# 92MING/Stable-Renderer

Measured on AMD Instinct MI355X. Metric: frames/sec @512^2, SD1.5 20-step img2img, 8-view overlap, higher is better.
Workload: dtype f16

## Files before the change

include/sr_hip.h:

```cpp
#ifndef SR_HIP_H
#define SR_HIP_H
#include <stdint.h>
#ifdef __cplusplus
extern "C" {
#endif

typedef enum {
  SR_OK = 0,
  SR_ERR_INVALID = -1,
  SR_ERR_LAUNCH = -2,
  SR_ERR_UNSUPPORTED = -3
} sr_status;

typedef enum { SR_F16 = 0, SR_F32 = 1 } sr_dtype;

const char* sr_last_error(void);
int sr_version(void);
const char* sr_source_hash(void);
int sr_device_sync(void);

typedef struct {
  const void* a;
  const void* a2;
  const void* w;
  const float* bias;
  const float* rowvec;
  const void* residual;
  void* out;
  const void* zero_page;
  int32_t B, H, W;
  int32_t C1, C2;
  int32_t N;
  int32_t KH;
  int32_t stride;
  int32_t upsample;
  int32_t act;
  int32_t transpose_out;
  int32_t ldt;
  int32_t out_f32;
  int32_t dtype;
  float scale;
  int32_t rowvec_ld;
  void* workspace;
  int64_t workspace_bytes;
  const float* row_stats;
  const float* colsum;
  int32_t tile;
  int32_t split;
  int32_t pad_br;
  const void* prefetch;
  int64_t prefetch_bytes;
  int32_t up_h, up_w;
  int32_t* split_counters;
  int32_t group;
  int32_t ln_inline;
  float ln_eps;
  int32_t tile_order;
} sr_igemm_args;
#define SR_IGEMM_SPLIT_COUNTERS 4096
#define SR_IGEMM_GROUP_MAX 4
int sr_igemm(const sr_igemm_args* args, void* stream);
int sr_igemm_group(const sr_igemm_args* const* args, int32_t n, void* stream);

typedef struct {
  const void* x; const void* x2;
  const float* gamma; const float* beta;
  void* y;
  float* partials;
  int32_t B, HW, C1, C2, groups, silu, dtype;
  float eps;
} sr_groupnorm_args;
int sr_groupnorm(const sr_groupnorm_args* args, void* stream);
int64_t sr_groupnorm_scratch_floats(int32_t B, int32_t HW);

int sr_row_stats(const void* x, float* stats, int32_t rows, int32_t C, float eps, int32_t dtype, void* stream);
int sr_layernorm(const void* x, const float* gamma, const float* beta, void* y, int32_t rows, int32_t C,
                 float eps, int32_t dtype, void* stream);
int sr_layernorm_gather(const void* x, const int32_t* sel, int32_t nsel, int32_t frame_rows, int32_t n_frames, int32_t* err_flag,
                        const float* gamma, const float* beta, void* y, int32_t C, float eps, int32_t dtype, void* stream);

typedef struct {
  const void* q; const void* k; const void* vt; void* o;
  int32_t B, Bk, Tq, Tk, heads, d, ldt, dtype;
  int32_t q_stride, k_stride;
  float scale;
} sr_attention_args;
int sr_attention(const sr_attention_args* args, void* stream);

int sr_nchw_to_nhwc(const float* x, void* y, int32_t B, int32_t C, int32_t HW, int32_t Cpad, float scale_mul,
                    const float* per_batch_scale, int32_t dtype, void* stream);
int sr_nhwc_to_nchw(const void* x, float* y, int32_t B, int32_t C, int32_t HW, int32_t ldc, int32_t dtype,
                    void* stream);
int sr_timestep_embedding(const float* t, void* y, int32_t B, int32_t dim, int32_t dtype, void* stream);
int sr_silu(const void* x, void* y, int64_t n, int32_t dtype, void* stream);
int sr_cast(const void* x, int32_t src_dtype, void* y, int32_t dst_dtype, int64_t n, void* stream);
int sr_cache_touch(const void* p, int64_t bytes, void* stream);
int sr_softmax_rows(void* x, int32_t rows, int32_t cols, int32_t dtype, void* stream);
int sr_gather_rows(const void* x, const int32_t* sel, void* y, int32_t nsel, int32_t n_rows, int64_t row_bytes,
                   int32_t* err_flag, void* stream);
int sr_add_scaled(const void* a, const void* b, void* y, int64_t n, float s, int32_t dtype, void* stream);

typedef enum {
  SR_OP_IGEMM = 1, SR_OP_GROUPNORM = 2, SR_OP_LAYERNORM = 3, SR_OP_ATTENTION = 4, SR_OP_NCHW_TO_NHWC = 5,
  SR_OP_NHWC_TO_NCHW = 6, SR_OP_TIMESTEP_EMBED = 7, SR_OP_SILU = 8, SR_OP_SOFTMAX_ROWS = 9, SR_OP_GATHER_ROWS = 10, SR_OP_ADD_SCALED = 11,
  SR_OP_FORK = 12,
  SR_OP_JOIN = 13,
  SR_OP_ROW_STATS = 14,
  SR_OP_LAYERNORM_GATHER = 15
} sr_op_kind;
typedef struct {
  int32_t kind; int32_t lane;
  union {
    sr_igemm_args igemm;
    sr_groupnorm_args gn;
    sr_attention_args attn;
    struct { const void* x; const float* gamma; const float* beta; void* y; int32_t rows, C, dtype; float eps;
             const int32_t* sel; int32_t* err_flag; int32_t frame_rows, n_frames; } ln;
    struct { const void* x; void* y; const float* per_batch_scale; int32_t B, C, HW, Cpad, dtype, ldc; float scale; } cvt;
    struct { const float* t; void* y; int32_t B, dim, dtype; } temb;
    struct { const void* x; void* y; int64_t n; int32_t dtype; int32_t rows, cols; } ew;
    struct { const void* x; void* y; const int32_t* sel; int64_t row_bytes; int32_t nsel; int32_t n_rows; int32_t* err_flag; } gather;
    struct { const void* a; const void* b; void* y; int64_t n; float s; int32_t dtype; } add;
  } u;
} sr_op;
int sr_plan_run(const sr_op* host_ops, int32_t n_ops, void* stream);
int sr_plan_capture(const sr_op* host_ops, int32_t n_ops, void* stream, void** graph_exec);
int sr_graph_launch(void* graph_exec, void* stream);
int sr_graph_destroy(void* graph_exec);

typedef struct sr_model sr_model;
int sr_model_load(const char* path, sr_model** model);
int sr_model_free(sr_model* model);
int sr_model_io(sr_model* model, const char* name, void** dev_ptr, int64_t* nbytes);
int sr_model_run(sr_model* model, const char* plan, void* stream);
int sr_model_write(sr_model* model, const char* name, const void* src, void* stream);
int sr_model_read(sr_model* model, const char* name, void* dst, void* stream);
int sr_unet_forward(sr_model* unet, const float* x, const float* t, const void* ctx, float* out, void* stream);
int sr_vae_decode(sr_model* vae, const float* z, float* img, void* stream);

int sr_eps_scale_input(const float* x, float* xin, int64_t n_per_copy, int32_t copies, float sigma, void* stream);
int sr_cfg_denoise(const float* x, const float* eps, float* denoised, float* d, int64_t n, int32_t copies,
                   float sigma, float cfg, void* stream);
int sr_cond_crop_scale(const float* x, float* xin, int32_t N, int32_t C, int32_t h, int32_t w, int32_t ah, int32_t aw, int32_t y0,
                       int32_t x0, int32_t chunks, float sigma, void* stream);
int sr_cond_accumulate(const float* x, const float* eps, const float* mult, const int32_t* kinds, float* out_c, float* cnt_c,
                       float* out_u, float* cnt_u, int32_t N, int32_t C, int32_t h, int32_t w, int32_t ah, int32_t aw, int32_t y0,
                       int32_t x0, int32_t chunks, float sigma, void* stream);
int sr_cfg_combine(const float* x, const float* out_c, const float* cnt_c, const float* out_u, const float* cnt_u, float* denoised,
                   float* d, int64_t n, float sigma, float cfg, void* stream);
int sr_euler_step(float* x, const float* d, int64_t n, float dt, void* stream);
int sr_vae_sample(const float* moments, const float* noise, float* z, int32_t B, int32_t zc, int32_t HW, void* stream);
int sr_ddpm_step(float* x, const float* denoised, const float* noise, int64_t n, float sigma, float sigma_next,
                 void* stream);
int sr_lcm_step(float* x, const float* denoised, const float* noise, int64_t n, float sigma_next, void* stream);
int sr_axpby(float* y, const float* x, int64_t n, float a, float b, void* stream);

int sr_idmap_masks(const int32_t* ids, float* masks, int64_t n_pixels, void* stream);

int sr_overlap_build(const int32_t* ids, int32_t N, int32_t H, int32_t W, int32_t lh, int32_t lw,
                     int32_t* pix_cell, int32_t* cell_vid, int32_t* max_vid, void* stream);
int64_t sr_overlap_csr_scratch_ints(int32_t vid_capacity);
int sr_overlap_csr(const int32_t* ids, const int32_t* pix_cell, int32_t N, int32_t H, int32_t W, int32_t vid_capacity,
                   int32_t* vid_off, int32_t* entries, int32_t* scratch, void* stream);
int sr_overlap_step(float* x, const int32_t* cell_vid, const int32_t* vid_off, const int32_t* entries, int32_t N, int32_t C,
                    int32_t lh, int32_t lw, int32_t vid_capacity, float ratio, float* blended, void* stream);

int sr_adain(const float* content, int64_t c_ps, int64_t c_cs, int64_t c_ns, int32_t HWc,
             const void* style, int32_t style_dtype, int64_t s_ps, int64_t s_cs, int64_t s_ns, int32_t HWs,
             float* out, int32_t N, int32_t C, float eps, float* stats, void* stream);

int sr_noise_pool(const void* noise_f16, const void* alpha_f16, const float* bg, float* pooled, float* out,
                  int32_t H, int32_t W, float* stats, void* stream);
int sr_noise_pool_strips(const void* noise_f16, const void* alpha_f16, const float* bg, float* pooled, float* out,
                         int32_t H, int32_t W, int32_t strip, float* stats, void* stream);

int sr_corrmap_update(const float* frame, int32_t Cf, const int32_t* ids, const float* mask,
                      const int32_t* src_index, int32_t n_pixels, int32_t sprite, int32_t material,
                      int32_t check_sprite, int32_t check_material, int32_t mode_first, void* values,
                      uint8_t* writtens, int32_t kk, int32_t V, int32_t* winner, int32_t* err_flag, void* stream);

int sr_legacy_overlap(const float* x, float* y, const int32_t* pix_vert, const int32_t* offsets, const int32_t* tr_f,
                      const int32_t* tr_y, const int32_t* tr_x, const float* view_normal, int32_t T, int32_t C, int32_t h,
                      int32_t w, int32_t H, int32_t W, float alpha, int32_t radius, int32_t algo, int32_t keep_nonzero,
                      void* stream);

int sr_legacy_levels(const int32_t* offsets, const int32_t* tr_f, const int32_t* tr_y, const int32_t* tr_x, const int32_t* order,
                     int32_t n_vertices, int32_t T, int32_t H, int32_t W, int32_t radius, int32_t* level_of, int32_t* n_levels);
int sr_legacy_overlap_seq(float* U, float* newval, const int32_t* lvl_vert, const int32_t* lvl_off_host, int32_t n_levels, int32_t max_len,
                          const int32_t* offsets, const int32_t* tr_f, const int32_t* tr_y, const int32_t* tr_x, const float* view_normal,
                          int32_t C, int32_t H, int32_t W, float alpha, int32_t radius, int32_t algo, void* stream);
int sr_nearest_resize(const float* src, float* dst, int64_t planes, int32_t Hi, int32_t Wi, int32_t Ho, int32_t Wo,
                      const float* keep_if_zero, void* stream);

typedef struct {
  const float* pos; const float* normal; const float* uv;
  const float* color;
  const int32_t* vertex_id;
  const int32_t* tris;
  int32_t nv, nt;
  float MV[16], MV_IT[16], P[16];
  int32_t sprite_id, material_id, corrmap_k, use_texcoord_id, render_mode;
  int32_t has_vertex_color, depth_test, cull_back;
  int32_t id_w, id_h;
  const void* noise_tex; int32_t noise_w, noise_h;
  const void* diffuse_tex; int32_t diffuse_w, diffuse_h;
  const void* corrmap_tex; int32_t corr_w, corr_h;
  const float* tangent; const float* bitangent;
  const void* normal_tex; int32_t normal_w, normal_h;
  int32_t diffuse_levels;
} sr_draw;
typedef struct {
  void* color;
  int32_t* id;
  float* pos;
  void* normal_depth;
  void* noise;
  float* canny;
  float* zbuf;
  int32_t W, H;
} sr_gbuffer;
int sr_gbuffer_clear(const sr_gbuffer* g, void* stream);
int sr_gbuffer_depth_merge(const sr_gbuffer* acc, const sr_gbuffer* src, void* stream);
int sr_defer_post(const void* color_rgba16f, const int32_t* ids, float* out_rgba, int32_t W, int32_t H, int32_t is_baking,
                  int32_t enable_gamma, int32_t enable_hdr, float gamma, float exposure, float saturation, float brightness,
                  float contrast, void* stream);
// ... 8 lines not shown
```

stable-renderer_amd/_lib.py:

```python
import ctypes as C
import os

_HERE = os.path.dirname(os.path.abspath(__file__))
LIB_PATH = os.path.join(_HERE, "csrc", "libsr_hip.so")
_DEV_LIB = os.environ.get("SR_DEV_LIB")

SR_F16, SR_F32 = 0, 1
(OP_IGEMM, OP_GROUPNORM, OP_LAYERNORM, OP_ATTENTION, OP_NCHW_TO_NHWC, OP_NHWC_TO_NCHW, OP_TIMESTEP_EMBED, OP_SILU,
 OP_SOFTMAX_ROWS, OP_GATHER_ROWS, OP_ADD_SCALED, OP_FORK, OP_JOIN, OP_ROW_STATS, OP_LAYERNORM_GATHER) = range(1, 16)

vp = C.c_void_p
i32 = C.c_int32
i64 = C.c_int64
f32 = C.c_float


class IgemmArgs(C.Structure):
    _fields_ = [("a", vp), ("a2", vp), ("w", vp), ("bias", vp), ("rowvec", vp), ("residual", vp), ("out", vp),
                ("zero_page", vp), ("B", i32), ("H", i32), ("W", i32), ("C1", i32), ("C2", i32), ("N", i32),
                ("KH", i32), ("stride", i32), ("upsample", i32), ("act", i32), ("transpose_out", i32), ("ldt", i32),
                ("out_f32", i32), ("dtype", i32), ("scale", f32), ("rowvec_ld", i32), ("workspace", vp),
                ("workspace_bytes", C.c_int64), ("row_stats", vp), ("colsum", vp), ("tile", i32), ("split", i32), ("pad_br", i32),
                ("prefetch", vp), ("prefetch_bytes", C.c_int64), ("up_h", i32), ("up_w", i32), ("split_counters", vp), ("group", i32), ("ln_inline", i32), ("ln_eps", f32), ("tile_order", i32)]


class GroupNormArgs(C.Structure):
    _fields_ = [("x", vp), ("x2", vp), ("gamma", vp), ("beta", vp), ("y", vp), ("partials", vp), ("B", i32),
                ("HW", i32), ("C1", i32), ("C2", i32), ("groups", i32), ("silu", i32), ("dtype", i32), ("eps", f32)]


class AttentionArgs(C.Structure):
    _fields_ = [("q", vp), ("k", vp), ("vt", vp), ("o", vp), ("B", i32), ("Bk", i32), ("Tq", i32), ("Tk", i32),
                ("heads", i32), ("d", i32), ("ldt", i32), ("dtype", i32), ("q_stride", i32), ("k_stride", i32),
                ("scale", f32)]


class _Ln(C.Structure):
    _fields_ = [("x", vp), ("gamma", vp), ("beta", vp), ("y", vp), ("rows", i32), ("C", i32), ("dtype", i32), ("eps", f32),
                ("sel", vp), ("err_flag", vp), ("frame_rows", i32), ("n_frames", i32)]


class _Cvt(C.Structure):
    _fields_ = [("x", vp), ("y", vp), ("per_batch_scale", vp), ("B", i32), ("C", i32), ("HW", i32), ("Cpad", i32),
                ("dtype", i32), ("ldc", i32), ("scale", f32)]


class _Temb(C.Structure):
    _fields_ = [("t", vp), ("y", vp), ("B", i32), ("dim", i32), ("dtype", i32)]


class _Ew(C.Structure):
    _fields_ = [("x", vp), ("y", vp), ("n", i64), ("dtype", i32), ("rows", i32), ("cols", i32)]


class _Gather(C.Structure):
    _fields_ = [("x", vp), ("y", vp), ("sel", vp), ("row_bytes", i64), ("nsel", i32), ("n_rows", i32), ("err_flag", vp)]


class _Add(C.Structure):
    _fields_ = [("a", vp), ("b", vp), ("y", vp), ("n", i64), ("s", f32), ("dtype", i32)]


class _OpU(C.Union):
    _fields_ = [("igemm", IgemmArgs), ("gn", GroupNormArgs), ("attn", AttentionArgs), ("ln", _Ln), ("cvt", _Cvt),
                ("temb", _Temb), ("ew", _Ew), ("gather", _Gather), ("add", _Add)]


class Op(C.Structure):
    _fields_ = [("kind", i32), ("lane", i32), ("u", _OpU)]


class Draw(C.Structure):
    _fields_ = [("pos", vp), ("normal", vp), ("uv", vp), ("color", vp), ("vertex_id", vp), ("tris", vp), ("nv", i32),
                ("nt", i32), ("MV", f32 * 16), ("MV_IT", f32 * 16), ("P", f32 * 16), ("sprite_id", i32),
                ("material_id", i32), ("corrmap_k", i32), ("use_texcoord_id", i32), ("render_mode", i32),
                ("has_vertex_color", i32), ("depth_test", i32), ("cull_back", i32), ("id_w", i32), ("id_h", i32),
                ("noise_tex", vp), ("noise_w", i32), ("noise_h", i32), ("diffuse_tex", vp), ("diffuse_w", i32),
                ("diffuse_h", i32), ("corrmap_tex", vp), ("corr_w", i32), ("corr_h", i32),
                ("tangent", vp), ("bitangent", vp), ("normal_tex", vp), ("normal_w", i32), ("normal_h", i32), ("diffuse_levels", i32)]


class GBuffer(C.Structure):
    _fields_ = [("color", vp), ("id", vp), ("pos", vp), ("normal_depth", vp), ("noise", vp), ("canny", vp), ("zbuf", vp),
                ("W", i32), ("H", i32)]


P = C.POINTER
SYMBOLS = {
    "sr_last_error": (C.c_char_p, []),
    "sr_version": (C.c_int, []),
    "sr_source_hash": (C.c_char_p, []),
    "sr_device_sync": (C.c_int, []),
    "sr_model_load": (C.c_int, [C.c_char_p, P(vp)]),
    "sr_model_free": (C.c_int, [vp]),
    "sr_model_io": (C.c_int, [vp, C.c_char_p, P(vp), P(i64)]),
    "sr_model_run": (C.c_int, [vp, C.c_char_p, vp]),
    "sr_model_write": (C.c_int, [vp, C.c_char_p, vp, vp]),
    "sr_model_read": (C.c_int, [vp, C.c_char_p, vp, vp]),
    "sr_unet_forward": (C.c_int, [vp, vp, vp, vp, vp, vp]),
    "sr_vae_decode": (C.c_int, [vp, vp, vp, vp]),
    "sr_layernorm_gather": (C.c_int, [vp, vp, i32, i32, i32, vp, vp, vp, vp, i32, f32, i32, vp]),
    "sr_igemm": (C.c_int, [P(IgemmArgs), vp]),
    "sr_igemm_group": (C.c_int, [P(P(IgemmArgs)), i32, vp]),
    "sr_groupnorm": (C.c_int, [P(GroupNormArgs), vp]),
    "sr_groupnorm_scratch_floats": (i64, [i32, i32]),
    "sr_layernorm": (C.c_int, [vp, vp, vp, vp, i32, i32, f32, i32, vp]),
    "sr_row_stats": (C.c_int, [vp, vp, i32, i32, f32, i32, vp]),
    "sr_attention": (C.c_int, [P(AttentionArgs), vp]),
    "sr_nchw_to_nhwc": (C.c_int, [vp, vp, i32, i32, i32, i32, f32, vp, i32, vp]),
    "sr_nhwc_to_nchw": (C.c_int, [vp, vp, i32, i32, i32, i32, i32, vp]),
    "sr_timestep_embedding": (C.c_int, [vp, vp, i32, i32, i32, vp]),
    "sr_silu": (C.c_int, [vp, vp, i64, i32, vp]),
    "sr_cast": (C.c_int, [vp, i32, vp, i32, i64, vp]),
    "sr_cache_touch": (C.c_int, [vp, i64, vp]),
    "sr_softmax_rows": (C.c_int, [vp, i32, i32, i32, vp]),
    "sr_gather_rows": (C.c_int, [vp, vp, vp, i32, i32, i64, vp, vp]),
    "sr_add_scaled": (C.c_int, [vp, vp, vp, i64, f32, i32, vp]),
    "sr_plan_run": (C.c_int, [P(Op), i32, vp]),
    "sr_plan_capture": (C.c_int, [P(Op), i32, vp, P(vp)]),
    "sr_graph_launch": (C.c_int, [vp, vp]),
    "sr_graph_destroy": (C.c_int, [vp]),
    "sr_eps_scale_input": (C.c_int, [vp, vp, i64, i32, f32, vp]),
    "sr_cfg_denoise": (C.c_int, [vp, vp, vp, vp, i64, i32, f32, f32, vp]),
    "sr_cond_crop_scale": (C.c_int, [vp, vp, i32, i32, i32, i32, i32, i32, i32, i32, i32, f32, vp]),
    "sr_cond_accumulate": (C.c_int, [vp, vp, vp, vp, vp, vp, vp, vp, i32, i32, i32, i32, i32, i32, i32, i32, i32, f32, vp]),
    "sr_cfg_combine": (C.c_int, [vp, vp, vp, vp, vp, vp, vp, i64, f32, f32, vp]),
    "sr_euler_step": (C.c_int, [vp, vp, i64, f32, vp]),
    "sr_vae_sample": (C.c_int, [vp, vp, vp, i32, i32, i32, vp]),
    "sr_ddpm_step": (C.c_int, [vp, vp, vp, i64, f32, f32, vp]),
    "sr_lcm_step": (C.c_int, [vp, vp, vp, i64, f32, vp]),
    "sr_axpby": (C.c_int, [vp, vp, i64, f32, f32, vp]),
    "sr_idmap_masks": (C.c_int, [vp, vp, i64, vp]),
    "sr_overlap_build": (C.c_int, [vp, i32, i32, i32, i32, i32, vp, vp, vp, vp]),
    "sr_overlap_csr_scratch_ints": (i64, [i32]),
    "sr_overlap_csr": (C.c_int, [vp, vp, i32, i32, i32, i32, vp, vp, vp, vp]),
    "sr_overlap_step": (C.c_int, [vp, vp, vp, vp, i32, i32, i32, i32, i32, f32, vp, vp]),
    "sr_legacy_overlap": (C.c_int, [vp, vp, vp, vp, vp, vp, vp, vp, i32, i32, i32, i32, i32, i32, f32, i32, i32, i32, vp]),
    "sr_legacy_levels": (C.c_int, [vp, vp, vp, vp, vp, i32, i32, i32, i32, i32, vp, vp]),
    "sr_legacy_overlap_seq": (C.c_int, [vp, vp, vp, vp, i32, i32, vp, vp, vp, vp, vp, i32, i32, i32, f32, i32, i32, vp]),
    "sr_nearest_resize": (C.c_int, [vp, vp, i64, i32, i32, i32, i32, vp, vp]),
    "sr_adain": (C.c_int, [vp, i64, i64, i64, i32, vp, i32, i64, i64, i64, i32, vp, i32, i32, f32, vp, vp]),
    "sr_noise_pool": (C.c_int, [vp, vp, vp, vp, vp, i32, i32, vp, vp]),
    "sr_noise_pool_strips": (C.c_int, [vp, vp, vp, vp, vp, i32, i32, i32, vp, vp]),
    "sr_corrmap_update": (C.c_int, [vp, i32, vp, vp, vp, i32, i32, i32, i32, i32, i32, vp, vp, i32, i32, vp, vp, vp]),
    "sr_gbuffer_clear": (C.c_int, [P(GBuffer), vp]),
    "sr_gbuffer_depth_merge": (C.c_int, [P(GBuffer), P(GBuffer), vp]),
    "sr_defer_post": (C.c_int, [vp, vp, vp, i32, i32, i32, i32, i32, f32, f32, f32, f32, f32, vp]),
    "sr_raster_draw": (C.c_int, [P(Draw), P(GBuffer), vp, i64, vp]),
    "sr_raster_scratch_bytes": (i64, [i32, i32, i32]),
}

_lib = None


class SrHipError(RuntimeError):
    pass


def _build_module():
    import importlib.util
    spec = importlib.util.spec_from_file_location("sr_build", os.path.join(_HERE, "csrc", "build.py"))
    mod = importlib.util.module_from_spec(spec)
    spec.loader.exec_module(mod)
    return mod


def _load():
    L = C.CDLL(LIB_PATH)
    for name, (res, args) in SYMBOLS.items():
        fn = getattr(L, name)
        fn.restype = res
        fn.argtypes = args
    return L


def lib():
    global _lib
    if _lib is None and _DEV_LIB:
        L = C.CDLL(_DEV_LIB)
        for name, (res, args) in SYMBOLS.items():
            fn = getattr(L, name)
            fn.restype = res
            fn.argtypes = args
        _lib = L
    if _lib is None:
        bm = _build_module()
        want = bm.source_hash()
        L = None
        if os.path.exists(LIB_PATH) and bm.built_hash() in (None, want):
            try:
                with open(LIB_PATH, "rb") as f:
                    current = want.encode() in f.read()
                if current:
                    L = _load()
            except (OSError, AttributeError):
                L = None
        if L is None:
            import fcntl
            try:
                os.makedirs(os.path.join(_HERE, "csrc", "_obj"), exist_ok=True)
                lock = open(os.path.join(_HERE, "csrc", "_obj", ".build.lock"), "w")
            except OSError as e:
                raise SrHipError(f"libsr_hip.so is stale or missing (sources are {want}) and {os.path.join(_HERE, 'csrc')} is not "
                                 f"writable for a rebuild: {e}; there is no CPU fallback for the product path") from e
            with lock:
                fcntl.flock(lock, fcntl.LOCK_EX)
                try:
                    have = bm.built_hash()
                    if have != want:
                        if os.environ.get("SR_NO_REBUILD") == "1":
                            raise SrHipError(f"libsr_hip.so is stale or missing (built from {have}, sources are {want}) and SR_NO_REBUILD=1; "
                                             "there is no CPU fallback for the product path")
                        try:
                            bm.build()
                        except Exception as e:
                            raise SrHipError(f"libsr_hip.so is stale or missing (built from {have}, sources are {want}) and the rebuild "
                                             f"failed: {e}\nrun `python stable-renderer_amd/csrc/build.py`; there is no CPU fallback for the "
                                             "product path") from e
                    if not os.path.exists(LIB_PATH):
                        raise SrHipError(f"{LIB_PATH} not built; there is no CPU fallback for the product path")
                    L = _load()
                finally:
                    fcntl.flock(lock, fcntl.LOCK_UN)
        if L.sr_source_hash().decode() != want:
            raise SrHipError(f"libsr_hip.so (built from {L.sr_source_hash().decode()}) does not match its sources ({want}): "
                             "remove stable-renderer_amd/csrc/_obj and rebuild")
        _lib = L
    return _lib


def check(rc):
    if rc != 0:
        raise SrHipError("libsr_hip: %s (code %d)" % (lib().sr_last_error().decode(errors="replace"), rc))
```

stable-renderer_amd/csrc/igemm.hip:

```cpp
#include "sr_common.h"
#ifndef SR_IGEMM_TRACE
#define SR_IGEMM_TRACE 0
#endif
#if SR_IGEMM_TRACE
#define SR_TS(k) do { if (threadIdx.x == 0) ts_[k] = wall_clock64(); } while (0)
#else
#define SR_TS(k) do { } while (0)
#endif
#include <stdlib.h>
#include <type_traits>

namespace {

#define SR_FOLD(p) ((p).row_stats != nullptr || (p).ln_inline != 0)
__device__ __forceinline__ float2 sr_fold_stat(const sr_igemm_args& p, const int m, const int m0) {
  extern __shared__ __attribute__((aligned(16))) char sr_lds_front[];
  if (p.ln_inline) return *(const float2*)(sr_lds_front + 8 * (m - m0));
  return *(const float2*)(p.row_stats + 2 * (int64_t)m);
}

template <typename T, int BM, int BN, int WAVES_M, int WAVES_N, int LDS_AVAIL, bool GEGLU, int VCAP, bool VECPRE>
__device__ __forceinline__ void epilogue_rows_h(const sr_igemm_args& p, f32x4 (&acc)[BN / WAVES_N / 16][BM / WAVES_M / 16], char* smem, const int M,
                                                const int rpb, const int m0, const int n0, const int pm0, const int qn0, const int wv,
                                                const int lane) {
  constexpr int NW = WAVES_M * WAVES_N, TM = BM / WAVES_M / 16, TN = BN / WAVES_N / 16;
  constexpr int WCOLS = BN / WAVES_N, OCOLS = GEGLU ? WCOLS / 2 : WCOLS;
  constexpr int ROWB = OCOLS * 2 + 16;
  constexpr int CPR = OCOLS * 2 / 16, RPI = 64 / CPR;
  constexpr int VEC_B = 2 * BN * 4;
  constexpr int LDS_ROWS = VECPRE ? LDS_AVAIL : LDS_AVAIL - VEC_B;
  constexpr int ACC = TM * TN * 4;
  constexpr auto iters = [](int tmp) { return (tmp * 16 + RPI - 1) / RPI; };
  constexpr auto fits = [](int tmp) { return tmp >= 1 && TM % tmp == 0 && NW * tmp * 16 * ROWB <= LDS_ROWS; };
  constexpr auto pre_ok = [](int tmp) { return ACC + (TM / tmp) * ((tmp * 16 + RPI - 1) / RPI) * 4 + 48 <= VCAP; };
  constexpr auto roll_ok = [](int tmp) { return TM / tmp > 1 && ACC + 2 * ((tmp * 16 + RPI - 1) / RPI) * 4 + 40 <= VCAP; };
  constexpr int T_LDS = fits(TM) ? TM : (fits(TM / 2) ? TM / 2 : 1);
  constexpr int TMP = pre_ok(T_LDS) ? T_LDS : (roll_ok(T_LDS) ? T_LDS : ((T_LDS > 1 && roll_ok(T_LDS / 2) && fits(T_LDS / 2)) ? T_LDS / 2 : ((T_LDS > 1 && roll_ok(1)) ? 1 : T_LDS)));
  constexpr int ROWS = TMP * 16, ITER = iters(TMP), NPASS = TM / TMP;
  constexpr bool PRE = pre_ok(TMP);
  constexpr bool ROLL = !PRE && roll_ok(TMP);
  static_assert(OCOLS % 8 == 0 && NW * 16 * ROWB <= LDS_ROWS, "epilogue staging");
  const int c16 = lane & 15, g4 = lane >> 4;
  const float scale = p.scale;
  const int N = p.N;
  const int ldr = p.rowvec_ld ? p.rowvec_ld : N;
  const int ldo = GEGLU ? (N >> 1) : N;
  float* lvec = (float*)(VECPRE ? smem - VEC_B : smem);
  char* wl = smem + (VECPRE ? 0 : VEC_B) + wv * (ROWS * ROWB);
  const int lr = lane / CPR, lc = lane - lr * CPR;
  const int ncol = (GEGLU ? ((n0 + qn0) >> 1) : (n0 + qn0)) + lc * 8;
  const bool lane_on = lr < RPI && ncol < ldo;
  const int tid = wv * 64 + lane;

  float4 vb = make_float4(0.f, 0.f, 0.f, 0.f), vc = make_float4(0.f, 0.f, 0.f, 0.f);
  if constexpr (!VECPRE) {
    const bool vec_lane = tid < BN / 4 && n0 + tid * 4 < N;
    if (vec_lane) {
      if (p.bias) vb = *(const float4*)(p.bias + n0 + tid * 4);
      if (SR_FOLD(p)) vc = *(const float4*)(p.colsum + n0 + tid * 4);
    }
  }
  uint4 resid[PRE ? NPASS * ITER : 1];
  if constexpr (PRE) {
    if (p.residual) {
#pragma unroll
      for (int ps = 0; ps < NPASS; ++ps)
#pragma unroll
        for (int it = 0; it < ITER; ++it) {
          const int row = it * RPI + lr, m = m0 + pm0 + ps * ROWS + row;
          resid[ps * ITER + it] = make_uint4(0, 0, 0, 0);
          if (lane_on && row < ROWS && m < M) resid[ps * ITER + it] = *(const uint4*)((const _Float16*)p.residual + (int64_t)m * ldo + ncol);
        }
    }
  }
  uint4 rcur[ROLL ? ITER : 1], rnext[ROLL ? ITER : 1];
  auto roll_load = [&](uint4 (&dst)[ROLL ? ITER : 1], int ps) {
#pragma unroll
    for (int it = 0; it < (ROLL ? ITER : 1); ++it) {
      const int row = it * RPI + lr, m = m0 + pm0 + ps * ROWS + row;
      dst[it] = make_uint4(0, 0, 0, 0);
      if (lane_on && row < ROWS && m < M) dst[it] = *(const uint4*)((const _Float16*)p.residual + (int64_t)m * ldo + ncol);
    }
  };
  if constexpr (ROLL) { if (p.residual) roll_load(rcur, 0); }
  __syncthreads();
  if constexpr (!VECPRE) {
    if (tid < BN / 4) { *(float4*)(lvec + tid * 4) = vb; *(float4*)(lvec + BN + tid * 4) = vc; }
    __syncthreads();
  }
#pragma unroll
  for (int ps = 0; ps < NPASS; ++ps) {
#pragma unroll
    for (int t = 0; t < TMP; ++t) {
      const int tm = ps * TMP + t;
      const int m = m0 + pm0 + tm * 16 + c16;
      const int b = (p.rowvec && m < M) ? m / rpb : 0;
      float2 rs = make_float2(1.f, 0.f);
      if (SR_FOLD(p) && m < M) rs = sr_fold_stat(p, m, m0);
#pragma unroll
      for (int tn = 0; tn < TN; ++tn) {
        const int nl = qn0 + tn * 16 + 4 * g4, n = n0 + nl;
        float v[4] = {acc[tn][tm][0] * scale, acc[tn][tm][1] * scale, acc[tn][tm][2] * scale, acc[tn][tm][3] * scale};
        if (n < N) {
          if (SR_FOLD(p)) {
            const float4 cs = *(const float4*)(lvec + BN + nl);
            v[0] = fmaf(rs.x, v[0], rs.y * cs.x); v[1] = fmaf(rs.x, v[1], rs.y * cs.y);
            v[2] = fmaf(rs.x, v[2], rs.y * cs.z); v[3] = fmaf(rs.x, v[3], rs.y * cs.w);
          }
          if (p.bias) { const float4 bv = *(const float4*)(lvec + nl); v[0] += bv.x; v[1] += bv.y; v[2] += bv.z; v[3] += bv.w; }
          if (p.rowvec) { const float4 rv = *(const float4*)(p.rowvec + (int64_t)b * ldr + n); v[0] += rv.x; v[1] += rv.y; v[2] += rv.z; v[3] += rv.w; }
        }
        if (p.act == 1) { for (int r = 0; r < 4; ++r) v[r] = sr_silu_f(v[r]); }
        else if (p.act == 3) { for (int r = 0; r < 4; ++r) v[r] = sr_gelu_f(v[r]); }
        else if (p.act == 4) { for (int r = 0; r < 4; ++r) v[r] = fminf(fmaxf((v[r] + 1.0f) * 0.5f, 0.0f), 1.0f); }
        char* dst = wl + (t * 16 + c16) * ROWB;
        if constexpr (GEGLU) {
          const float o0 = v[0] * sr_gelu_f(v[1]), o1 = v[2] * sr_gelu_f(v[3]);
          h16x2 hv = {(_Float16)o0, (_Float16)o1};
          *(h16x2*)(dst + (tn * 8 + 2 * g4) * 2) = hv;
        } else {
          h16x4 hv = {(_Float16)v[0], (_Float16)v[1], (_Float16)v[2], (_Float16)v[3]};
          *(h16x4*)(dst + (tn * 16 + 4 * g4) * 2) = hv;
        }
      }
    }
    __builtin_amdgcn_s_waitcnt(0xC07F);
    __builtin_amdgcn_wave_barrier();
    if constexpr (ROLL) { if (p.residual && ps + 1 < NPASS) roll_load(rnext, ps + 1); }
#pragma unroll
    for (int it = 0; it < ITER; ++it) {
      const int row = it * RPI + lr, m = m0 + pm0 + ps * ROWS + row;
      if (!(lane_on && row < ROWS && m < M)) continue;
      uint4 raw = *(const uint4*)(wl + row * ROWB + lc * 16);
      const int64_t oi = (int64_t)m * ldo + ncol;
      if (p.residual) {
        const h16x8 rr = PRE ? __builtin_bit_cast(h16x8, resid[PRE ? ps * ITER + it : 0])
                       : ROLL ? __builtin_bit_cast(h16x8, rcur[ROLL ? it : 0]) : *(const h16x8*)((const _Float16*)p.residual + oi);
        h16x8 hv = __builtin_bit_cast(h16x8, raw);
#pragma unroll
        for (int e = 0; e < 8; ++e) hv[e] = (_Float16)((float)hv[e] + (float)rr[e]);
        raw = __builtin_bit_cast(uint4, hv);
      }
      *(uint4*)((_Float16*)p.out + oi) = raw;
    }
    if constexpr (ROLL) {
#pragma unroll
      for (int it = 0; it < ITER; ++it) rcur[it] = rnext[it];
    }
    __builtin_amdgcn_wave_barrier();
  }
}

template <typename T, int BM, int BN, int WAVES_M, int WAVES_N, int LDS_AVAIL, bool BLOCK_SYNC = true, int VCAP = 256, bool VECPRE = false>
__device__ __forceinline__ void epilogue_rows(const sr_igemm_args& p, f32x4 (&acc)[BN / WAVES_N / 16][BM / WAVES_M / 16], char* smem, const int M,
                                              const int rpb, const int m0, const int n0, const int pm0, const int qn0, const int wv,
                                              const int lane) {
  constexpr int NW = WAVES_M * WAVES_N, TM = BM / WAVES_M / 16, TN = BN / WAVES_N / 16;
  const int c16 = lane & 15, g4 = lane >> 4;
  const float scale = p.scale;
  const int N = p.N;
  const int ldr = p.rowvec_ld ? p.rowvec_ld : N;
  {
    const int ldo = (p.act == 2) ? (N >> 1) : N;
    const bool o32 = p.out_f32 || sizeof(T) == 4;
    const int oes = o32 ? 4 : 2;
    if constexpr (sizeof(T) == 2) {
      if (!o32 && (ldo * 2) % 16 == 0) {
        static_assert(BLOCK_SYNC, "the fp16 epilogue synchronises the workgroup itself");
        if (p.act == 2) epilogue_rows_h<T, BM, BN, WAVES_M, WAVES_N, LDS_AVAIL, true, VCAP, VECPRE>(p, acc, smem, M, rpb, m0, n0, pm0, qn0, wv, lane);
        else            epilogue_rows_h<T, BM, BN, WAVES_M, WAVES_N, LDS_AVAIL, false, VCAP, VECPRE>(p, acc, smem, M, rpb, m0, n0, pm0, qn0, wv, lane);
        return;
      }
    }
    if ((ldo * oes) % 16 == 0) {
      constexpr int WCOLS = BN / WAVES_N;
      constexpr int TMP = (NW * (BM / WAVES_M) * (WCOLS * 4 + 16) <= LDS_AVAIL) ? TM : 1;
      const int ocols = (p.act == 2) ? WCOLS / 2 : WCOLS;
      const int rowb = ocols * oes + 16;
      if constexpr (BLOCK_SYNC) __syncthreads();
      char* wl = smem + wv * ((TMP * 16) * rowb);
      const int cpr = ocols * oes / 16;
      const int rpi = 64 / cpr;
      const int lr = lane / cpr, lc = lane - lr * cpr;
      const int ncol0 = (p.act == 2) ? ((n0 + qn0) >> 1) : (n0 + qn0);
      const int epc_o = 16 / oes;
#pragma unroll
     for (int tm0 = 0; tm0 < TM; tm0 += TMP) {
#pragma unroll
      for (int tm = tm0; tm < tm0 + TMP; ++tm) {
        const int m = m0 + pm0 + tm * 16 + c16;
        const int b = (m < M) ? m / rpb : 0;
        float2 rs = make_float2(1.f, 0.f);
        if (SR_FOLD(p) && m < M) rs = sr_fold_stat(p, m, m0);
#pragma unroll
        for (int tn = 0; tn < TN; ++tn) {
          const int n = n0 + qn0 + tn * 16 + 4 * g4;
          float v[4] = {acc[tn][tm][0] * scale, acc[tn][tm][1] * scale, acc[tn][tm][2] * scale, acc[tn][tm][3] * scale};
          if (n < N) {
            if (SR_FOLD(p)) {
              const float4 cs = *(const float4*)(p.colsum + n);
              v[0] = fmaf(rs.x, v[0], rs.y * cs.x); v[1] = fmaf(rs.x, v[1], rs.y * cs.y);
              v[2] = fmaf(rs.x, v[2], rs.y * cs.z); v[3] = fmaf(rs.x, v[3], rs.y * cs.w);
            }
            if (p.bias) { const float4 bv = *(const float4*)(p.bias + n); v[0] += bv.x; v[1] += bv.y; v[2] += bv.z; v[3] += bv.w; }
            if (p.rowvec) { const float4 rv = *(const float4*)(p.rowvec + (int64_t)b * ldr + n); v[0] += rv.x; v[1] += rv.y; v[2] += rv.z; v[3] += rv.w; }
          }
          if (p.act == 1) { for (int r = 0; r < 4; ++r) v[r] = sr_silu_f(v[r]); }
          else if (p.act == 3) { for (int r = 0; r < 4; ++r) v[r] = sr_gelu_f(v[r]); }
          else if (p.act == 4) { for (int r = 0; r < 4; ++r) v[r] = fminf(fmaxf((v[r] + 1.0f) * 0.5f, 0.0f), 1.0f); }
          char* dst = wl + ((tm - tm0) * 16 + c16) * rowb;
          if (p.act == 2) {
            const float o0 = v[0] * sr_gelu_f(v[1]), o1 = v[2] * sr_gelu_f(v[3]);
            const int col = tn * 8 + 2 * g4;
            if (o32) *(float2*)(dst + col * 4) = make_float2(o0, o1);
            else { h16x2 hv = {(_Float16)o0, (_Float16)o1}; *(h16x2*)(dst + col * 2) = hv; }
          } else {
            const int col = tn * 16 + 4 * g4;
            if (o32) *(float4*)(dst + col * 4) = make_float4(v[0], v[1], v[2], v[3]);
            else { h16x4 hv = {(_Float16)v[0], (_Float16)v[1], (_Float16)v[2], (_Float16)v[3]}; *(h16x4*)(dst + col * 2) = hv; }
          }
        }
      }
      __builtin_amdgcn_s_waitcnt(0xC07F);
      __builtin_amdgcn_wave_barrier();
      for (int r0 = 0; r0 < TMP * 16; r0 += rpi) {
        const int row = r0 + lr;
        if (lr >= rpi || row >= TMP * 16) continue;
        const int m = m0 + pm0 + tm0 * 16 + row, ncol = ncol0 + lc * epc_o;
        if (m >= M || ncol >= ldo) continue;
        uint4 raw = *(const uint4*)(wl + row * rowb + lc * 16);
        const int64_t oi = (int64_t)m * ldo + ncol;
        if (p.residual) {
          if constexpr (sizeof(T) == 2) {
            if (o32) {
              float4 f = __builtin_bit_cast(float4, raw);
              const h16x4 r4 = *(const h16x4*)((const _Float16*)p.residual + oi);
              f.x += (float)r4[0]; f.y += (float)r4[1]; f.z += (float)r4[2]; f.w += (float)r4[3];
              raw = __builtin_bit_cast(uint4, f);
            } else {
              const h16x8 rr = *(const h16x8*)((const _Float16*)p.residual + oi);
              h16x8 hv = __builtin_bit_cast(h16x8, raw);
#pragma unroll
              for (int e = 0; e < 8; ++e) hv[e] = (_Float16)((float)hv[e] + (float)rr[e]);
              raw = __builtin_bit_cast(uint4, hv);
            }
          } else {
            float4 f = __builtin_bit_cast(float4, raw);
            const float4 rr = *(const float4*)((const float*)p.residual + oi);
            f.x += rr.x; f.y += rr.y; f.z += rr.z; f.w += rr.w;
            raw = __builtin_bit_cast(uint4, f);
          }
        }
        *(uint4*)((char*)p.out + oi * oes) = raw;
      }
      __builtin_amdgcn_wave_barrier();
     }
      return;
    }
#pragma unroll
    for (int tm = 0; tm < TM; ++tm) {
      const int m = m0 + pm0 + tm * 16 + c16;
      if (m >= M) continue;
      const int b = m / rpb;
#pragma unroll
      for (int tn = 0; tn < TN; ++tn) {
        const int n = n0 + qn0 + tn * 16 + 4 * g4;
        if (n >= N) continue;
        float v[4] = {acc[tn][tm][0] * scale, acc[tn][tm][1] * scale, acc[tn][tm][2] * scale, acc[tn][tm][3] * scale};
        const int nv = (N - n) < 4 ? (N - n) : 4;
        if (SR_FOLD(p)) {
          const float2 rs = sr_fold_stat(p, m, m0);
          for (int r = 0; r < nv; ++r) v[r] = fmaf(rs.x, v[r], rs.y * p.colsum[n + r]);
        }
        if (p.bias) { for (int r = 0; r < nv; ++r) v[r] += p.bias[n + r]; }
        if (p.rowvec) { for (int r = 0; r < nv; ++r) v[r] += p.rowvec[(int64_t)b * ldr + n + r]; }
        if (p.act == 1) { for (int r = 0; r < 4; ++r) v[r] = sr_silu_f(v[r]); }
        else if (p.act == 3) { for (int r = 0; r < 4; ++r) v[r] = sr_gelu_f(v[r]); }
        else if (p.act == 4) { for (int r = 0; r < 4; ++r) v[r] = fminf(fmaxf((v[r] + 1.0f) * 0.5f, 0.0f), 1.0f); }
        if (p.act == 2) {
          float o0 = v[0] * sr_gelu_f(v[1]), o1 = v[2] * sr_gelu_f(v[3]);
          const int64_t oi = (int64_t)m * ldo + (n >> 1);
          if (p.residual) { o0 += sr_load_f((const T*)p.residual + oi); o1 += sr_load_f((const T*)p.residual + oi + 1); }
          if (p.out_f32) { float* o = (float*)p.out + oi; o[0] = o0; o[1] = o1; }
          else { T* o = (T*)p.out + oi; sr_store_f(o, o0); sr_store_f(o + 1, o1); }
          continue;
        }
        const int64_t oi = (int64_t)m * ldo + n;
        if (nv == 4) {
          if (p.residual) {
            if constexpr (sizeof(T) == 2) {
              const h16x4 rr = *(const h16x4*)((const T*)p.residual + oi);
              v[0] += (float)rr[0]; v[1] += (float)rr[1]; v[2] += (float)rr[2]; v[3] += (float)rr[3];
            } else {
              const float4 rr = *(const float4*)((const float*)p.residual + oi);
              v[0] += rr.x; v[1] += rr.y; v[2] += rr.z; v[3] += rr.w;
            }
          }
          if (p.out_f32 || sizeof(T) == 4) {
            *(float4*)((float*)p.out + oi) = make_float4(v[0], v[1], v[2], v[3]);
          } else {
            h16x4 hv = {(_Float16)v[0], (_Float16)v[1], (_Float16)v[2], (_Float16)v[3]};
            *(h16x4*)((_Float16*)p.out + oi) = hv;
          }
        } else {
          for (int r = 0; r < nv; ++r) {
            float o = v[r];
            if (p.residual) o += sr_load_f((const T*)p.residual + oi + r);
            if (p.out_f32) ((float*)p.out)[oi + r] = o; else sr_store_f((T*)p.out + oi + r, o);
          }
        }
      }
    }
  }
}

template <int PS, int D>
__device__ __forceinline__ void wait_leaving(int y) {
#define SR_WL(k) if constexpr (D - 1 > k) { if (y == k) { asm volatile("s_waitcnt vmcnt(%0)" ::"n"(PS * k) : "memory"); return; } }
  SR_WL(1) SR_WL(2) SR_WL(3) SR_WL(4) SR_WL(5) SR_WL(6)
#undef SR_WL
  asm volatile("s_waitcnt vmcnt(0)" ::: "memory");
}

template <typename T, int BM, int BN, int WAVES_M, int WAVES_N, int STAGES, bool TRANS, bool SPLIT = false, int BKB = 128, int SPREAD = 0, int MINB = 1, bool LNI = false>
__device__ __forceinline__ void igemm_body(const sr_igemm_args& p, const int M, const int Ho, const int Wo,
                                           const int NT, const int nwg, const int tile0, const int bid, const int nblk) {
  extern __shared__ __attribute__((aligned(16))) char smem_all[];
  constexpr int PF_B = WAVES_M * WAVES_N * 256;
  char* const smem_raw = smem_all + PF_B;
  constexpr bool VECPRE = sizeof(T) == 2 && !SPLIT;
  constexpr int VEC_B = VECPRE ? 2 * BN * 4 : 0;
  char* const smem = smem_raw + VEC_B;
  constexpr int KE = BKB / (int)sizeof(T);
  constexpr int NW = WAVES_M * WAVES_N;
  constexpr int RPI = 1024 / BKB;
  constexpr int GP = BM / RPI, GQ = BN / RPI;
  constexpr int NIP = (GP + NW - 1) / NW, NIQ = (GQ + NW - 1) / NW;
  constexpr int TM = BM / WAVES_M / 16, TN = BN / WAVES_N / 16;
  constexpr int STAGE_BYTES = (BM + BN) * BKB;
  constexpr int FBLK = 16 * BKB;
  static_assert(NW == 4 || NW == 8, "4 or 8 waves");
  static_assert(BKB == 128 || BKB == 64, "K bytes per stage");
  static_assert(BM % RPI == 0 && BN % RPI == 0, "tile rows must be whole LDS-DMA groups");

  const int tid = threadIdx.x, lane = tid & 63;
  const int wv = __builtin_amdgcn_readfirstlane(tid >> 6);
#if SR_IGEMM_TRACE
  unsigned long long ts_[6] = {0, 0, 0, 0, 0, 0};
#endif
  SR_TS(0);
  if (p.prefetch) {
    const int64_t nthr = (int64_t)nblk * gridDim.y * (NW * 64);
    sr_prefetch_touch(p.prefetch, p.prefetch_bytes, ((int64_t)blockIdx.y * nblk + bid) * (NW * 64) + tid, nthr,
                      __builtin_amdgcn_readfirstlane(sr_lds_addr(smem_all) + wv * 256));
  }
  const int wg = tile0 + sr_xcd_remap(bid, nwg);
  int mt, nt;
  sr_tile_of(wg, NT, (M + BM - 1) / BM, p.tile_order, mt, nt);
  const int m0 = mt * BM, n0 = nt * BN;
  if constexpr (VECPRE) {
    constexpr int CH = BN / 2;
    const int c = wv * 64 + lane;
    if (wv * 64 < CH) {
      const bool second = c >= BN / 4;
      const int n = n0 + 4 * (second ? c - BN / 4 : c);
      const float* base = second ? (SR_FOLD(p) ? p.colsum : nullptr) : p.bias;
      const char* src = (base && n < p.N) ? (const char*)(base + n) : (const char*)p.zero_page;
      if (c < CH) sr_glds16_asm(src, __builtin_amdgcn_readfirstlane(sr_lds_addr(smem_raw) + wv * 1024));
    }
  }
  const int lrow = BKB == 128 ? lane >> 3 : lane >> 2;
  int lchunk;
  if constexpr (BKB == 128) lchunk = (lane & 7) ^ lrow;
  else { const int q = (lane & 3) ^ ((lrow >> 2) & 3); lchunk = (0x1320 >> (4 * q)) & 3; }

  const int C1 = p.C1, C2 = p.C2, Ctot = C1 + C2;
  const int K1 = C1 / KE, KPT = Ctot / KE;
  const int ntaps = p.KH * p.KH;
  const int KT = ntaps * KPT;
  const int H = p.H, W = p.W, pad = p.pad_br ? 0 : (p.KH >> 1);
  const int rpb = Ho * Wo;

  int pb[NIP], py[NIP], px[NIP];
#pragma unroll
  for (int i = 0; i < NIP; ++i) {
    const int gi = (i * NW + wv) < GP ? (i * NW + wv) : GP - 1;
    const int m = m0 + gi * RPI + lrow;
    if (m < M) {
      if (rpb == 1) { pb[i] = m; py[i] = -pad; px[i] = -pad; }
      else {
        const int b = m / rpb, rem = m - b * rpb, oy = rem / Wo;
        pb[i] = b; py[i] = oy * p.stride - pad; px[i] = (rem - oy * Wo) * p.stride - pad;
      }
    } else { pb[i] = -1; py[i] = 0; px[i] = 0; }
  }
  const char* zp = (const char*)p.zero_page + lchunk * 16;
  const char* rowA[NIP];
  const char* rowB[NIP];
  auto set_tap = [&](int tap) {
    const int ky = tap / p.KH, kx = tap - ky * p.KH;
#pragma unroll
    for (int i = 0; i < NIP; ++i) {
      int iy = py[i] + ky, ix = px[i] + kx;
      bool ok = pb[i] >= 0;
      if (p.upsample) {
        if (p.up_h > 0) {
          ok = ok && iy >= 0 && ix >= 0 && iy < p.up_h && ix < p.up_w;
          iy = min((int)floorf((float)iy * ((float)H / (float)p.up_h)), H - 1);
          ix = min((int)floorf((float)ix * ((float)W / (float)p.up_w)), W - 1);
          if (!ok) { iy = 0; ix = 0; }
        } else { ok = ok && iy >= 0 && ix >= 0 && iy < 2 * H && ix < 2 * W; iy >>= 1; ix >>= 1; }
      }
      else            { ok = ok && iy >= 0 && ix >= 0 && iy < H && ix < W; }
      const int64_t pix = ((int64_t)pb[i] * H + iy) * W + ix;
      rowA[i] = ok ? (const char*)p.a + (pix * C1) * (int64_t)sizeof(T) + lchunk * 16 : zp;
      rowB[i] = (ok && C2 > 0) ? (const char*)p.a2 + (pix * C2) * (int64_t)sizeof(T) + lchunk * 16 : zp;
    }
  };
  const char* wrow[NIQ];
#pragma unroll
  for (int i = 0; i < NIQ; ++i) {
    const int gi = (i * NW + wv) < GQ ? (i * NW + wv) : GQ - 1;
    const int n = n0 + gi * RPI + lrow;
    wrow[i] = (const char*)p.w + ((int64_t)n * KT * KE) * (int64_t)sizeof(T) + lchunk * 16;
  }

  int kt0 = 0, kt1 = KT;
  if constexpr (SPLIT) {
    kt0 = (int)((int64_t)KT * blockIdx.y / gridDim.y);
    kt1 = (int)((int64_t)KT * (blockIdx.y + 1) / gridDim.y);
#pragma unroll
    for (int i = 0; i < NIQ; ++i) wrow[i] += (int64_t)kt0 * BKB;
  }
  int s_tap = kt0 / KPT, s_kk = kt0 - s_tap * KPT;
  auto advance = [&]() { if (++s_kk == KPT) { s_kk = 0; if (++s_tap < ntaps) set_tap(s_tap); } };
  set_tap(s_tap);
  auto stage = [&](int buf) {
    char* tP = smem + buf * STAGE_BYTES;
    char* tQ = tP + BM * BKB;
    const bool fromA = s_kk < K1;
    const int off = (fromA ? s_kk : s_kk - K1) * BKB;
    auto gp = [&](int i) { return ((i * NW + wv) < GP ? (i * NW + wv) : GP - 1) * 1024; };
    auto gq = [&](int i) { return ((i * NW + wv) < GQ ? (i * NW + wv) : GQ - 1) * 1024; };
    {
      const unsigned lP = __builtin_amdgcn_readfirstlane(sr_lds_addr(tP)), lQ = __builtin_amdgcn_readfirstlane(sr_lds_addr(tQ));
      const unsigned m0 = sr_m0_save();
#pragma unroll
      for (int i = 0; i < NIP; ++i) sr_glds16_asm_nosave((fromA ? rowA[i] : rowB[i]) + off, lP + gp(i));
#pragma unroll
      for (int i = 0; i < NIQ; ++i) { sr_glds16_asm_nosave(wrow[i], lQ + gq(i)); wrow[i] += BKB; }
      sr_m0_restore(m0);
    }
    advance();
  };

  const int c16 = lane & 15, g4 = lane >> 4;
  const int wm = wv / WAVES_N, wn = wv - wm * WAVES_N;
  const int pm0 = wm * (BM / WAVES_M), qn0 = wn * (BN / WAVES_N);
  int foff[2];
  if constexpr (BKB == 128) {
    foff[0] = c16 * 128 + (((0 + g4) ^ (c16 & 7)) << 4);
    foff[1] = c16 * 128 + (((4 + g4) ^ (c16 & 7)) << 4);
  } else {
    foff[0] = foff[1] = c16 * 64 + ((((c16 >> 2) & 3) ^ ((0x2130 >> (4 * g4)) & 3)) << 4);
  }

  constexpr int TA = TRANS ? TM : TN, TB = TRANS ? TN : TM;
  f32x4 acc[TA][TB];
#pragma unroll
  for (int a = 0; a < TA; ++a)
#pragma unroll
    for (int b = 0; b < TB; ++b) acc[a][b] = f32x4{0.f, 0.f, 0.f, 0.f};

  constexpr int TMS = LNI ? TM / WAVES_N : 1;
  static_assert(!LNI || (TM % WAVES_N == 0 && !SPLIT), "in-launch LayerNorm statistics: fragments split evenly over the waves of a row block");
  float lsum[TMS], lsq[TMS], lpiv[TMS];
#pragma unroll
// ... 28 lines not shown

  auto compute = [&](int buf, int j0 = 0, int j1 = BKB / 64) {
    const char* tP = smem + buf * STAGE_BYTES + pm0 * BKB;
    const char* tQ = smem + buf * STAGE_BYTES + BM * BKB + qn0 * BKB;
#pragma unroll
    for (int j = j0; j < j1; ++j) {
      uint4 xf[TM], wf[TN];
#pragma unroll
      for (int t = 0; t < TM; ++t) xf[t] = *(const uint4*)(tP + t * FBLK + foff[j]);
#pragma unroll
      for (int t = 0; t < TN; ++t) wf[t] = *(const uint4*)(tQ + t * FBLK + foff[j]);
      if constexpr (LNI) ln_acc(tP, foff[j]);
#pragma unroll
      for (int tn = 0; tn < TN; ++tn)
#pragma unroll
        for (int tm = 0; tm < TM; ++tm) {
          if constexpr (TRANS) sr_mma(acc[tm][tn], xf[tm], wf[tn], T());
          else                 sr_mma(acc[tn][tm], wf[tn], xf[tm], T());
        }
    }
  };
  auto compute_staging = [&](int buf, int nbuf) {
    const char* tP = smem + buf * STAGE_BYTES + pm0 * BKB;
    const char* tQ = smem + buf * STAGE_BYTES + BM * BKB + qn0 * BKB;
    char* nP = smem + nbuf * STAGE_BYTES;
    const unsigned lP = __builtin_amdgcn_readfirstlane(sr_lds_addr(nP)), lQ = __builtin_amdgcn_readfirstlane(sr_lds_addr(nP + BM * BKB));
    const bool fromA = s_kk < K1;
    const int off = (fromA ? s_kk : s_kk - K1) * BKB;
    constexpr int PIECES = NIP + NIQ, PPS = (PIECES + TN - 1) / TN;
    auto piece = [&](int i) {
      if (i < NIP) {
        const int g = ((i * NW + wv) < GP ? (i * NW + wv) : GP - 1) * 1024;
        sr_glds16_asm_nosave((fromA ? rowA[i] : rowB[i]) + off, lP + g);
      } else if (i < PIECES) {
        const int q = i - NIP;
        const int g = ((q * NW + wv) < GQ ? (q * NW + wv) : GQ - 1) * 1024;
        sr_glds16_asm_nosave(wrow[q], lQ + g);
        wrow[q] += BKB;
      }
    };
    const unsigned m0_keep = sr_m0_save();
#pragma unroll
    for (int j = 0; j < BKB / 64; ++j) {
      uint4 xf[TM], wf[TN];
#pragma unroll
      for (int t = 0; t < TM; ++t) xf[t] = *(const uint4*)(tP + t * FBLK + foff[j]);
#pragma unroll
      for (int t = 0; t < TN; ++t) wf[t] = *(const uint4*)(tQ + t * FBLK + foff[j]);
      if constexpr (LNI) ln_acc(tP, foff[j]);
#pragma unroll
      for (int tn = 0; tn < TN; ++tn) {
#pragma unroll
        for (int tm = 0; tm < TM; ++tm) {
          if constexpr (TRANS) sr_mma(acc[tm][tn], xf[tm], wf[tn], T());
          else                 sr_mma(acc[tn][tm], wf[tn], xf[tm], T());
        }
        if (j == 0) {
#pragma unroll
          for (int q = 0; q < PPS; ++q) piece(tn * PPS + q);
        }
      }
    }
    sr_m0_restore(m0_keep);
    advance();
  };
  {
    constexpr int PER_STAGE = NIP + NIQ;
    constexpr int D = STAGES - 1;
    static_assert(STAGES >= 2 && STAGES <= 8, "ring depth");
    static_assert(PER_STAGE * (D - 1) < 64, "vmcnt immediate");
    const int nk = kt1 - kt0;
    SR_TS(1);
#pragma unroll
    for (int i = 0; i < D; ++i) if (i < nk) stage(i);
    int cur = 0;
    for (int kt = 0; kt < nk; ++kt) {
      const int younger = nk - 1 - kt;
      if (younger >= D - 1) asm volatile("s_waitcnt vmcnt(%0)" ::"n"(PER_STAGE * (D - 1)) : "memory");
      else                  wait_leaving<PER_STAGE, D>(younger);
      __builtin_amdgcn_s_barrier();
      if (kt == 0) SR_TS(2);
      if constexpr (SPREAD == 1) {
        if (kt + D < nk) { int nb = cur + D; if (nb >= STAGES) nb -= STAGES; compute_staging(cur, nb); }
        else compute(cur);
      } else if constexpr (SPREAD == 2 && BKB == 128) {
        compute(cur, 0, 1);
        if (kt + D < nk) { int nb = cur + D; if (nb >= STAGES) nb -= STAGES; stage(nb); }
        compute(cur, 1, 2);
      } else {
        if (kt + D < nk) { int nb = cur + D; if (nb >= STAGES) nb -= STAGES; stage(nb); }
        compute(cur);
      }
      if (++cur == STAGES) cur = 0;
    }
  }

  SR_TS(3);
  if constexpr (LNI) {
    const float invk = 1.0f / (float)p.C1;
#pragma unroll
    for (int i = 0; i < TMS; ++i) {
      float su = lsum[i], sq = lsq[i];
      su += __shfl_xor(su, 16); sq += __shfl_xor(sq, 16);
      su += __shfl_xor(su, 32); sq += __shfl_xor(sq, 32);
      const int tm = wn + i * WAVES_N;
      if (g4 == 0) {
        const float dm = su * invk, var = fmaxf(fmaf(-dm, dm, sq * invk), 0.f);
        const float mean = sizeof(T) == 4 ? lpiv[i] + dm : dm;
        const float rstd = rsqrtf(var + p.ln_eps);
        *(float2*)(smem_all + 8 * (pm0 + tm * 16 + c16)) = make_float2(rstd, -rstd * mean);
      }
    }
    __syncthreads();
  }
  const float scale = p.scale;
  const int N = p.N;
  const int ldr = p.rowvec_ld ? p.rowvec_ld : N;
  if constexpr (SPLIT) {
    f32x4* ws = (f32x4*)p.workspace + (((int64_t)blockIdx.y * nwg + (wg - tile0)) * NW + wv) * (TN * TM * 64) + lane;
#pragma unroll
    for (int tn = 0; tn < TN; ++tn)
#pragma unroll
      for (int tm = 0; tm < TM; ++tm) ws[(tn * TM + tm) * 64] = acc[tn][tm];
    if (p.split_counters == nullptr) return;
    __threadfence();
    __syncthreads();
    int* const flag = (int*)smem_all;
    if (tid == 0) {
      const int prev = __hip_atomic_fetch_add(p.split_counters + (wg - tile0), 1, __ATOMIC_RELAXED, __HIP_MEMORY_SCOPE_AGENT);
      *flag = prev == (int)gridDim.y - 1;
    }
    __syncthreads();
    if (!*flag) return;
    __threadfence();
    {
      const f32x4* wr = (const f32x4*)p.workspace + ((int64_t)(wg - tile0) * NW + wv) * (TN * TM * 64) + lane;
      const int64_t zs = (int64_t)nwg * NW * (TN * TM * 64);
      const int S = gridDim.y;
#pragma unroll
      for (int tn = 0; tn < TN; ++tn)
#pragma unroll
        for (int tm = 0; tm < TM; ++tm) acc[tn][tm] = wr[(tn * TM + tm) * 64];
      for (int z = 1; z < S; ++z) {
#pragma unroll
        for (int tn = 0; tn < TN; ++tn)
#pragma unroll
          for (int tm = 0; tm < TM; ++tm) acc[tn][tm] += wr[z * zs + (tn * TM + tm) * 64];
      }
      if (tid == 0) p.split_counters[wg - tile0] = 0;
    }
    epilogue_rows<T, BM, BN, WAVES_M, WAVES_N, STAGES * STAGE_BYTES, true, (MINB >= 4 ? 128 : 256), VECPRE>(p, acc, smem, M, rpb, m0, n0, pm0, qn0, wv, lane);
    return;
  } else if constexpr (!TRANS) {
    epilogue_rows<T, BM, BN, WAVES_M, WAVES_N, STAGES * STAGE_BYTES, true, (MINB >= 4 ? 128 : 256), VECPRE>(p, acc, smem, M, rpb, m0, n0, pm0, qn0, wv, lane);
#if SR_IGEMM_TRACE
    SR_TS(4);
    asm volatile("s_waitcnt vmcnt(0)" ::: "memory");
    SR_TS(5);
    if (threadIdx.x == 0 && p.workspace && !SPLIT) { unsigned long long* w_ = (unsigned long long*)p.workspace + (size_t)bid * 8; for (int k_ = 0; k_ < 6; ++k_) w_[k_] = ts_[k_]; w_[6] = __smid(); }
#endif
  } else {
    const bool vec = (rpb % 4 == 0) && (p.ldt % 4 == 0);
#pragma unroll
    for (int tm = 0; tm < TM; ++tm) {
      const int m = m0 + pm0 + tm * 16 + 4 * g4;
      if (m >= M) continue;
#pragma unroll
      for (int tn = 0; tn < TN; ++tn) {
        const int n = n0 + qn0 + tn * 16 + c16;
        if (n >= N) continue;
        const float bz = p.bias ? p.bias[n] : 0.f;
        float v[4] = {acc[tm][tn][0] * scale, acc[tm][tn][1] * scale, acc[tm][tn][2] * scale, acc[tm][tn][3] * scale};
        if (SR_FOLD(p)) {
          const float cs = p.colsum[n];
          for (int r = 0; r < 4; ++r)
            if (m + r < M) { const float2 rs = sr_fold_stat(p, m + r, m0); v[r] = fmaf(rs.x, v[r], rs.y * cs); }
        }
        for (int r = 0; r < 4; ++r) v[r] += bz;
        if (vec) {
          const int b = m / rpb, t = m - b * rpb;
          const int64_t oi = ((int64_t)b * N + n) * p.ldt + t;
          if (p.out_f32 || sizeof(T) == 4) *(float4*)((float*)p.out + oi) = make_float4(v[0], v[1], v[2], v[3]);
          else { h16x4 hv = {(_Float16)v[0], (_Float16)v[1], (_Float16)v[2], (_Float16)v[3]}; *(h16x4*)((_Float16*)p.out + oi) = hv; }
        } else {
          for (int r = 0; r < 4; ++r) {
            const int mm = m + r;
            if (mm >= M) break;
            const int b = mm / rpb, t = mm - b * rpb;
            const int64_t oi = ((int64_t)b * N + n) * p.ldt + t;
            if (p.out_f32) ((float*)p.out)[oi] = v[r]; else sr_store_f((T*)p.out + oi, v[r]);
          }
        }
      }
    }
  }
}

template <typename T, int BM, int BN, int WAVES_M, int WAVES_N, int STAGES, bool TRANS, bool SPLIT = false, int BKB = 128, int SPREAD = 0, int MINB = 1, bool LNI = false>
__global__ __launch_bounds__(WAVES_M * WAVES_N * 64, MINB) void igemm_kernel(const sr_igemm_args p, const int M, const int Ho, const int Wo,
                                                                        const int NT, const int nwg, const int tile0) {
  igemm_body<T, BM, BN, WAVES_M, WAVES_N, STAGES, TRANS, SPLIT, BKB, SPREAD, MINB, LNI>(p, M, Ho, Wo, NT, nwg, tile0, blockIdx.x, gridDim.x);
}

struct igemm_group_k {
  sr_igemm_args p[SR_IGEMM_GROUP_MAX];
  int M[SR_IGEMM_GROUP_MAX], Ho[SR_IGEMM_GROUP_MAX], Wo[SR_IGEMM_GROUP_MAX], NT[SR_IGEMM_GROUP_MAX], nwg[SR_IGEMM_GROUP_MAX];
  int start[SR_IGEMM_GROUP_MAX + 1];
  int n;
};
template <typename T, int BM, int BN, int WAVES_M, int WAVES_N, int STAGES, int BKB = 128, int SPREAD = 0, int MINB = 1, bool LNI = false>
__global__ __launch_bounds__(WAVES_M * WAVES_N * 64, MINB) void igemm_group_kernel(const igemm_group_k g) {
  int i = 0;
#pragma unroll
  for (int j = 1; j < SR_IGEMM_GROUP_MAX; ++j) if (j < g.n && (int)blockIdx.x >= g.start[j]) i = j;
  igemm_body<T, BM, BN, WAVES_M, WAVES_N, STAGES, false, false, BKB, SPREAD, MINB, LNI>(g.p[i], g.M[i], g.Ho[i], g.Wo[i], g.NT[i], g.nwg[i], 0,
                                                                                          (int)blockIdx.x - g.start[i], g.nwg[i]);
}

template <typename T, int BM, int BN, int WAVES_M, int WAVES_N, int STAGES, int BKB = 128, int SPREAD = 0, int MINB = 1, bool LNI = false>
int launch_group_impl(const sr_igemm_args* const* as, const int* Ms, const int* Hos, const int* Wos, int n, hipStream_t st) {
  igemm_group_k g;
  g.n = n;
  int tot = 0;
  for (int i = 0; i < SR_IGEMM_GROUP_MAX; ++i) {
    const int k = i < n ? i : n - 1;
    g.p[i] = *as[k];
    g.p[i].prefetch = nullptr;
    g.M[i] = Ms[k]; g.Ho[i] = Hos[k]; g.Wo[i] = Wos[k];
    g.NT[i] = (as[k]->N + BN - 1) / BN;
    g.nwg[i] = ((Ms[k] + BM - 1) / BM) * g.NT[i];
    g.start[i] = tot;
    if (i < n) tot += g.nwg[i];
  }
  g.start[SR_IGEMM_GROUP_MAX] = tot;
  constexpr int lds_stage = STAGES * (BM + BN) * BKB;
  constexpr int lds_epi_all = WAVES_M * WAVES_N * (BM / WAVES_M) * ((BN / WAVES_N) * 4 + 16);
  constexpr int lds_epi = lds_epi_all <= lds_stage ? lds_epi_all : WAVES_M * WAVES_N * 16 * ((BN / WAVES_N) * 4 + 16);
  constexpr int lds = (lds_stage > lds_epi ? lds_stage : lds_epi) + (sizeof(T) == 2 ? 2 * BN * 4 : 0) + WAVES_M * WAVES_N * 256;
  auto k = igemm_group_kernel<T, BM, BN, WAVES_M, WAVES_N, STAGES, BKB, SPREAD, MINB, LNI>;
  static bool attr_set = false;
  if (!attr_set) { (void)hipFuncSetAttribute((const void*)k, hipFuncAttributeMaxDynamicSharedMemorySize, lds); attr_set = true; }
  hipLaunchKernelGGL(k, dim3(tot), dim3(WAVES_M * WAVES_N * 64), lds, st, g);
  SR_CHECK_LAUNCH("sr_igemm_group");
  return SR_OK;
}
template <typename T, int BM, int BN, int WAVES_M, int WAVES_N, int STAGES, int BKB = 128, int SPREAD = 0, int MINB = 1>
int launch_group(const sr_igemm_args* const* as, const int* Ms, const int* Hos, const int* Wos, int n, hipStream_t st) {
  bool lni = false;
  for (int i = 0; i < n; ++i) lni = lni || as[i]->ln_inline;
  if (lni) return launch_group_impl<T, BM, BN, WAVES_M, WAVES_N, STAGES, BKB, SPREAD, MINB, true>(as, Ms, Hos, Wos, n, st);
  return launch_group_impl<T, BM, BN, WAVES_M, WAVES_N, STAGES, BKB, SPREAD, MINB, false>(as, Ms, Hos, Wos, n, st);
}

template <typename T, int BM, int BN, int WAVES_M, int WAVES_N, int STAGES, bool TRANS, int BKB, int SPREAD, int MINB, bool LNI>
int launch_impl(const sr_igemm_args& a, int M, int Ho, int Wo, hipStream_t st) {
  const int Npad = (a.N + 127) / 128 * 128;
  const int MT = (M + BM - 1) / BM, NT = Npad / BN;
  const int NTv = (a.N + BN - 1) / BN;
  const int nwg = MT * NTv;
  constexpr int lds_stage = STAGES * (BM + BN) * BKB;
  constexpr int lds_epi_all = WAVES_M * WAVES_N * (BM / WAVES_M) * ((BN / WAVES_N) * 4 + 16);
  constexpr int lds_epi = lds_epi_all <= lds_stage ? lds_epi_all : WAVES_M * WAVES_N * 16 * ((BN / WAVES_N) * 4 + 16);
  constexpr int lds = (lds_stage > lds_epi ? lds_stage : lds_epi) + (sizeof(T) == 2 ? 2 * BN * 4 : 0)
                      + WAVES_M * WAVES_N * 256;
  auto k = igemm_kernel<T, BM, BN, WAVES_M, WAVES_N, STAGES, TRANS, false, BKB, SPREAD, MINB, LNI>;
  static bool attr_set = false;
  if (!attr_set) { (void)hipFuncSetAttribute((const void*)k, hipFuncAttributeMaxDynamicSharedMemorySize, lds); attr_set = true; }
  (void)NT;
  hipLaunchKernelGGL(k, dim3(nwg), dim3(WAVES_M * WAVES_N * 64), lds, st, a, M, Ho, Wo, NTv, nwg, 0);
  SR_CHECK_LAUNCH("sr_igemm");
  return SR_OK;
}
template <typename T, int BM, int BN, int WAVES_M, int WAVES_N, int STAGES, bool TRANS, int BKB = 128, int SPREAD = 0, int MINB = 1>
int launch(const sr_igemm_args& a, int M, int Ho, int Wo, hipStream_t st) {
  if (a.ln_inline) SR_FAIL(SR_ERR_INVALID, "sr_igemm: ln_inline is not built for this tile (%d x %d, %d stages)", BM, BN, STAGES);
  return launch_impl<T, BM, BN, WAVES_M, WAVES_N, STAGES, TRANS, BKB, SPREAD, MINB, false>(a, M, Ho, Wo, st);
}
template <typename T, int BM, int BN, int WAVES_M, int WAVES_N, int STAGES, bool TRANS, int BKB = 128, int SPREAD = 0, int MINB = 1>
int launch_ln(const sr_igemm_args& a, int M, int Ho, int Wo, hipStream_t st) {
  if (a.ln_inline) return launch_impl<T, BM, BN, WAVES_M, WAVES_N, STAGES, TRANS, BKB, SPREAD, MINB, true>(a, M, Ho, Wo, st);
  return launch_impl<T, BM, BN, WAVES_M, WAVES_N, STAGES, TRANS, BKB, SPREAD, MINB, false>(a, M, Ho, Wo, st);
}

template <typename T, int BM, int BN>
__global__ __launch_bounds__(256) void splitk_reduce_kernel(const sr_igemm_args p, const int M, const int rpb, const int S,
                                                            const int NT, const int nwg, const int tile0) {
  constexpr int TM = BM / 2 / 16, TN = BN / 2 / 16, FR = TN * TM;
  const int tile_l = blockIdx.x / FR, fr = blockIdx.x - tile_l * FR;
  const int tn = fr / TM, tm = fr - tn * TM;
  const int wv = threadIdx.x >> 6, lane = threadIdx.x & 63, c16 = lane & 15, g4 = lane >> 4;
  const int wg = tile0 + tile_l;
  int mt, nt;
  sr_tile_of(wg, NT, (M + BM - 1) / BM, p.tile_order, mt, nt);
  const int m = mt * BM + (wv >> 1) * (BM / 2) + tm * 16 + c16;
  const int n = nt * BN + (wv & 1) * (BN / 2) + tn * 16 + 4 * g4;
  const int N = p.N;
  if (m >= M || n >= N) return;
  const f32x4* ws = (const f32x4*)p.workspace + ((int64_t)tile_l * 4 + wv) * (FR * 64) + fr * 64 + lane;
  const int64_t zs = (int64_t)nwg * 4 * FR * 64;
  f32x4 acc = ws[0];
  for (int z = 1; z < S; ++z) acc += ws[z * zs];
  float v[4] = {acc[0] * p.scale, acc[1] * p.scale, acc[2] * p.scale, acc[3] * p.scale};
  if (p.row_stats) {
    const float2 rs = *(const float2*)(p.row_stats + 2 * (int64_t)m);
    const float4 cs = *(const float4*)(p.colsum + n);
    v[0] = fmaf(rs.x, v[0], rs.y * cs.x); v[1] = fmaf(rs.x, v[1], rs.y * cs.y);
    v[2] = fmaf(rs.x, v[2], rs.y * cs.z); v[3] = fmaf(rs.x, v[3], rs.y * cs.w);
  }
  if (p.bias) { const float4 bv = *(const float4*)(p.bias + n); v[0] += bv.x; v[1] += bv.y; v[2] += bv.z; v[3] += bv.w; }
  if (p.rowvec) {
    const int ldr = p.rowvec_ld ? p.rowvec_ld : N;
    const float4 rv = *(const float4*)(p.rowvec + (int64_t)(m / rpb) * ldr + n);
    v[0] += rv.x; v[1] += rv.y; v[2] += rv.z; v[3] += rv.w;
  }
  if (p.act == 1) { for (int r = 0; r < 4; ++r) v[r] = sr_silu_f(v[r]); }
  else if (p.act == 3) { for (int r = 0; r < 4; ++r) v[r] = sr_gelu_f(v[r]); }
  else if (p.act == 4) { for (int r = 0; r < 4; ++r) v[r] = fminf(fmaxf((v[r] + 1.0f) * 0.5f, 0.0f), 1.0f); }
  const int64_t oi = (int64_t)m * N + n;
  if (p.residual) {
    if constexpr (sizeof(T) == 2) {
      const h16x4 rr = *(const h16x4*)((const _Float16*)p.residual + oi);
      v[0] += (float)rr[0]; v[1] += (float)rr[1]; v[2] += (float)rr[2]; v[3] += (float)rr[3];
    } else {
      const float4 rr = *(const float4*)((const float*)p.residual + oi);
      v[0] += rr.x; v[1] += rr.y; v[2] += rr.z; v[3] += rr.w;
    }
  }
  if (p.out_f32 || sizeof(T) == 4) *(float4*)((float*)p.out + oi) = make_float4(v[0], v[1], v[2], v[3]);
  else { h16x4 hv = {(_Float16)v[0], (_Float16)v[1], (_Float16)v[2], (_Float16)v[3]}; *(h16x4*)((_Float16*)p.out + oi) = hv; }
}

template <typename T, int BM, int BN, int STAGES = 2>
int launch_split(const sr_igemm_args& a, int M, int Ho, int Wo, int tile0, int S, hipStream_t st) {
  const int MT = (M + BM - 1) / BM, NTv = (a.N + BN - 1) / BN, ntiles = MT * NTv, ntail = ntiles - tile0;
  constexpr int lds_stage = STAGES * (BM + BN) * 128;
  constexpr int lds_epi = 4 * (BM / 2) * ((BN / 2) * 4 + 16);
  constexpr int lds = (lds_stage > lds_epi ? lds_stage : lds_epi) + (sizeof(T) == 2 ? 2 * BN * 4 : 0) + 4 * 256;
  auto kf = igemm_kernel<T, BM, BN, 2, 2, STAGES, false, false>;
  auto ks = igemm_kernel<T, BM, BN, 2, 2, STAGES, false, true>;
  static bool attr_set = false;
  if (!attr_set) {
    (void)hipFuncSetAttribute((const void*)kf, hipFuncAttributeMaxDynamicSharedMemorySize, lds);
    (void)hipFuncSetAttribute((const void*)ks, hipFuncAttributeMaxDynamicSharedMemorySize, lds);
    attr_set = true;
  }
  if (tile0 > 0) hipLaunchKernelGGL(kf, dim3(tile0), dim3(256), lds, st, a, M, Ho, Wo, NTv, tile0, 0);
  sr_igemm_args as = a;
  if (ntail > SR_IGEMM_SPLIT_COUNTERS) as.split_counters = nullptr;
  hipLaunchKernelGGL(ks, dim3(ntail, S), dim3(256), lds, st, as, M, Ho, Wo, NTv, ntail, tile0);
  if (!as.split_counters) {
    constexpr int FR = (BM / 32) * (BN / 32);
    hipLaunchKernelGGL((splitk_reduce_kernel<T, BM, BN>), dim3(ntail * FR), dim3(256), 0, st, a, M, Ho * Wo, S, NTv, ntail, tile0);
  }
  SR_CHECK_LAUNCH("sr_igemm(split-K)");
  return SR_OK;
}

__global__ __launch_bounds__(512, 1) void conv3p_kernel(const sr_igemm_args p, const int M, const int NT, const int nwg) {
  using T = _Float16;
  extern __shared__ __attribute__((aligned(16))) char smem_all[];
  char* const smem = smem_all + 8 * 256;
  constexpr int BM = 256, BN = 320, WAVES_M = 4, WAVES_N = 2, TM = 4, TN = 10;
  constexpr int APITCH = 80, ABYTES = 32768, BBYTES = BN * 64, BOFF = 2 * ABYTES, LDS_TOTAL = BOFF + 4 * BBYTES;
  const int tid = threadIdx.x, lane = tid & 63;
  const int wv = __builtin_amdgcn_readfirstlane(tid >> 6);
  if (p.prefetch)
    sr_prefetch_touch(p.prefetch, p.prefetch_bytes, (int64_t)blockIdx.x * 512 + tid, (int64_t)gridDim.x * 512,
                      __builtin_amdgcn_readfirstlane(sr_lds_addr(smem_all) + wv * 256));
  const int wg = sr_xcd_remap(blockIdx.x, nwg);
  const int mt = wg / NT, nt = wg - mt * NT;
  const int m0 = mt * BM, n0 = nt * BN;
  const int H = p.H, W = p.W, C1 = p.C1, rpb = H * W;
  const int ipt = rpb >= 256 ? 1 : 256 / rpb;
  const int Ri = rpb >= 256 ? 256 / W : H;
  const int PW = W + 2, HPI = (Ri + 2) * PW, HR = ipt * HPI;
  const int b0 = m0 / rpb, y0 = (m0 - b0 * rpb) / W;

  unsigned aoffg[4];
#pragma unroll
  for (int i = 0; i < 4; ++i) {
    const int u = (wv * 4 + i) * 64 + lane;
    const int hrow = u / 5, ch = u - hrow * 5;
    const int img = hrow / HPI, rem = hrow - img * HPI, hr = rem / PW, hc = rem - hr * PW;
    const int y = y0 + hr - 1, x = hc - 1, b = b0 + img;
    const bool ok = ch < 4 && hrow < HR && y >= 0 && y < H && x >= 0 && x < W && b < p.B;
    aoffg[i] = ok ? (unsigned)(((((int64_t)b * H + y) * W + x) * C1) * 2 + ch * 16) : 0xFFFFFFFFu;
    if (!ok) {
      *(uint4*)(smem + (wv * 4 + i) * 1024 + lane * 16) = make_uint4(0, 0, 0, 0);
      *(uint4*)(smem + ABYTES + (wv * 4 + i) * 1024 + lane * 16) = make_uint4(0, 0, 0, 0);
    }
  }
  asm volatile("s_waitcnt lgkmcnt(0)" ::: "memory");
  const int lrow = lane >> 2;
  const int lchunk = (0x1320 >> (4 * ((lane & 3) ^ ((lrow >> 2) & 3)))) & 3;
  const unsigned wlane = (unsigned)(lrow * 9 * C1 * 2 + lchunk * 16);
  const unsigned ldsA = __builtin_amdgcn_readfirstlane(sr_lds_addr(smem)), ldsB = ldsA + BOFF;
  int ac = 0;
  auto issueA = [&](int buf, int i) {
    if (aoffg[i] != 0xFFFFFFFFu) sr_glds16_asm_saddr(aoffg[i], (const char*)p.a + (int64_t)ac * 64, ldsA + buf * ABYTES + (wv * 4 + i) * 1024);
  };
  int lc = 0, lt = 0;
  auto issueB = [&](int slot) {
    const char* wb = (const char*)p.w + ((int64_t)n0 * 9 * C1 + lt * C1 + lc * 32) * 2;
#pragma unroll
    for (int i = 0; i < 3; ++i) {
      const int gi = (i * 8 + wv) < 20 ? (i * 8 + wv) : 19;
      sr_glds16_asm_saddr(wlane, wb + (int64_t)gi * 16 * 9 * C1 * 2, ldsB + slot * BBYTES + gi * 1024);
    }
    if (++lt == 9) { lt = 0; ++lc; }
  };

  const int c16 = lane & 15, g4 = lane >> 4;
  const int wm = wv >> 1, wn = wv & 1;
  const int pm0 = wm * 64, qn0 = wn * 160;
  int aoff0, adel[TM];
  {
    const int riw = Ri * W;
    auto hrow_of = [&](int pi) { const int img = pi / riw, q = pi - img * riw, r = q / W, cx = q - r * W; return img * HPI + r * PW + cx; };
    aoff0 = hrow_of(pm0 + c16) * APITCH + g4 * 16;
#pragma unroll
    for (int j = 0; j < TM; ++j) adel[j] = __builtin_amdgcn_readfirstlane((hrow_of(pm0 + j * 16) - hrow_of(pm0)) * APITCH);
  }
  const int foffB = qn0 * 64 + c16 * 64 + ((((c16 >> 2) & 3) ^ ((0x2130 >> (4 * g4)) & 3)) << 4);
  const int pw80 = PW * APITCH;

  f32x4 acc[TN][TM];
#pragma unroll
  for (int a = 0; a < TN; ++a)
#pragma unroll
    for (int b = 0; b < TM; ++b) acc[a][b] = f32x4{0.f, 0.f, 0.f, 0.f};

  const int NC = C1 / 32;
  {
    const unsigned m0k = sr_m0_save();
#pragma unroll
    for (int i = 0; i < 4; ++i) issueA(0, i);
    ac = 1;
    issueB(0); issueB(1); issueB(2);
    sr_m0_restore(m0k);
  }
  int s = 0;
  auto chunk = [&](auto lastc, const int c) {
    constexpr bool LASTC = decltype(lastc)::value;
    auto step = [&](auto tc) {
      constexpr int t = decltype(tc)::value;
      constexpr int nx = LASTC ? (t <= 6 ? 6 : (t == 7 ? 3 : 0))
                               : 6 + (t >= 1 && t <= 4) + (t >= 2 && t <= 5) + (t >= 3 && t <= 6);
      asm volatile("s_waitcnt vmcnt(%0)" ::"n"(nx) : "memory");
      __builtin_amdgcn_s_barrier();
      const char* Bq = smem + BOFF + (s & 3) * BBYTES + foffB;
      int to = (t / 3) * pw80 + (t % 3) * APITCH + (c & 1) * ABYTES;
      asm volatile("" : "+s"(to));
      uint4 xf[TM], wf[TN];
#pragma unroll
      for (int j = 0; j < TM; ++j) xf[j] = *(const uint4*)(smem + aoff0 + (adel[j] + to));
#pragma unroll
      for (int tn = 0; tn < TN; ++tn) wf[tn] = *(const uint4*)(Bq + tn * 1024);
      if (!LASTC || t < 6) {
        const unsigned m0k = sr_m0_save();
        issueB((s + 3) & 3);
        if constexpr (!LASTC) { if (t < 4) issueA((c + 1) & 1, t); if (t == 3) ++ac; }
        sr_m0_restore(m0k);
      }
#pragma unroll
      for (int tn = 0; tn < TN; ++tn)
#pragma unroll
        for (int tm = 0; tm < TM; ++tm) sr_mma(acc[tn][tm], wf[tn], xf[tm], T());
      ++s;
    };
    step(std::integral_constant<int, 0>{}); step(std::integral_constant<int, 1>{}); step(std::integral_constant<int, 2>{});
    step(std::integral_constant<int, 3>{}); step(std::integral_constant<int, 4>{}); step(std::integral_constant<int, 5>{});
    step(std::integral_constant<int, 6>{}); step(std::integral_constant<int, 7>{}); step(std::integral_constant<int, 8>{});
  };
  for (int c = 0; c < NC - 1; ++c) chunk(std::false_type{}, c);
  chunk(std::true_type{}, NC - 1);

  epilogue_rows<T, BM, BN, WAVES_M, WAVES_N, LDS_TOTAL>(p, acc, smem, M, rpb, m0, n0, pm0, qn0, wv, lane);
}

static bool conv3p_ok(const sr_igemm_args& a, int M) {
  if (a.dtype != SR_F16 || a.KH != 3 || a.stride != 1 || a.upsample || a.C2 || a.transpose_out || a.row_stats || a.ln_inline || a.pad_br) return false;
  if (a.C1 % 64 || a.N % 320 || M % 256 || a.act == 2) return false;
  const int rpb = a.H * a.W;
  if (a.W < 8 || 256 % a.W) { if (!(rpb < 256 && 256 % rpb == 0)) return false; }
  if (rpb >= 256 ? (rpb % 256 != 0 || 256 % a.W != 0) : (256 % rpb != 0)) return false;
  const int ipt = rpb >= 256 ? 1 : 256 / rpb, Ri = rpb >= 256 ? 256 / a.W : a.H;
  if ((int64_t)a.B * rpb * a.C1 * 2 >= 0xFFFFFFFFLL) return false;
  return ipt * (Ri + 2) * (a.W + 2) * 80 <= 32768;
}

static int launch_conv3p(const sr_igemm_args& a, int M, hipStream_t st) {
  constexpr int lds = 2 * 32768 + 4 * 320 * 64 + 8 * 256;
  const int NT = a.N / 320, nwg = (M / 256) * NT;
  static bool attr_set = false;
  if (!attr_set) { (void)hipFuncSetAttribute((const void*)conv3p_kernel, hipFuncAttributeMaxDynamicSharedMemorySize, lds); attr_set = true; }
  hipLaunchKernelGGL(conv3p_kernel, dim3(nwg), dim3(512), lds, st, a, M, NT, nwg);
  SR_CHECK_LAUNCH("sr_igemm(conv3p)");
  return SR_OK;
}

static inline int plan_split(int64_t tiles, int KT, int slots, double t_k, int64_t tile_ws_bytes, int64_t ws_bytes, int* tile0, int forceS = 0) {
  const int64_t full = tiles / slots, tail = tiles - full * slots;
  *tile0 = (int)(full * slots);
  if (tail == 0) return 1;
  if (forceS > 0)
    return (KT / forceS >= 4 && (int64_t)forceS * tail * tile_ws_bytes <= ws_bytes) ? forceS : -1;
  if (const char* fs = getenv("SR_SPLIT_S")) {
    const int S = atoi(fs);
    if (S >= 1 && KT / S >= 4 && (int64_t)S * tail * tile_ws_bytes <= ws_bytes) return S;
  }
  double best = (double)KT * t_k;
  int bestS = 1;
  for (int S = 2; S <= 16; ++S) {
    if (KT / S < 8 || (int64_t)S * tail * tile_ws_bytes > ws_bytes) break;
    const int64_t rounds = (tail * S + slots - 1) / slots;
    const double t = (double)rounds * ((KT + S - 1) / S) * t_k + (double)(2 * S * tail * tile_ws_bytes) / 4.0e6 + 14.0;
    if (t < best * 0.9) { best = t; bestS = S; }
  }
  return bestS;
}

template <typename T, bool TRANS>
int dispatch(const sr_igemm_args& a, int M, int Ho, int Wo, hipStream_t st) {
  const int n128 = (a.N + 127) / 128, n64 = (a.N + 63) / 64;
  const int64_t wg_128x128 = (int64_t)((M + 127) / 128) * n128;
  const bool waste128 = (n128 * 128 - a.N) * 8 > a.N;
  const char* fenv = getenv("SR_IGEMM_TILE");
  const int force = fenv ? atoi(fenv) : a.tile;
  static const bool split_off = getenv("SR_SPLITK") && atoi(getenv("SR_SPLITK")) == 0;
  const int KT = a.KH * a.KH * ((a.C1 + a.C2) / (int)(128 / sizeof(T)));
  const int forceS = a.split > 1 ? a.split : 0;
  const bool can_split = !TRANS && !split_off && a.split >= 0 && a.workspace && a.act != 2 && a.N % 4 == 0 && !a.ln_inline;
  const bool may_split = can_split && KT >= 32;
  const bool deep_split = can_split && KT >= 8 && (force == 14 || force == 15);
  if (forceS && !((may_split && (force == 2 || force == 3)) || deep_split))
    SR_FAIL(SR_ERR_INVALID, "sr_igemm: split = %d needs tile 2 / 3 (K >= 32 steps) or 14 / 15 (K >= 8 steps), a workspace, no GEGLU / transposed output", a.split);
  if constexpr (!TRANS) {
    if (deep_split && forceS) {
      int tile0 = 0;
      const int64_t tiles = force == 15 ? wg_128x128 : (int64_t)((M + 127) / 128) * n64;
      const int S = plan_split(tiles, KT, 256, 1.0, 128 * (force == 15 ? 128 : 64) * 4, a.workspace_bytes, &tile0, forceS);
      if (S < 0) SR_FAIL(SR_ERR_INVALID, "sr_igemm: split = %d does not fit this shape (K steps %d, workspace %lld B)", a.split, KT, (long long)a.workspace_bytes);
      if (S > 1) return force == 15 ? launch_split<T, 128, 128, 4>(a, M, Ho, Wo, tile0, S, st) : launch_split<T, 128, 64, 6>(a, M, Ho, Wo, tile0, S, st);
      SR_FAIL(SR_ERR_INVALID, "sr_igemm: split = %d: nothing to split (whole rounds of workgroups only)", a.split);
    }
    if (may_split && (force == 2 || force == 3)) {
      int tile0 = 0;
      if (force == 2) {
        const int S = plan_split(wg_128x128, KT, 512, 1.2, 128 * 128 * 4, a.workspace_bytes, &tile0, forceS);
        if (S < 0) SR_FAIL(SR_ERR_INVALID, "sr_igemm: split = %d does not fit this shape (K steps %d, workspace %lld B)", a.split, KT, (long long)a.workspace_bytes);
        if (S > 1) return launch_split<T, 128, 128>(a, M, Ho, Wo, tile0, S, st);
      } else {
        const int S = plan_split((int64_t)((M + 127) / 128) * n64, KT, 768, 0.93, 128 * 64 * 4, a.workspace_bytes, &tile0, forceS);
        if (S < 0) SR_FAIL(SR_ERR_INVALID, "sr_igemm: split = %d does not fit this shape (K steps %d, workspace %lld B)", a.split, KT, (long long)a.workspace_bytes);
        if (S > 1) return launch_split<T, 128, 64>(a, M, Ho, Wo, tile0, S, st);
      }
      if (forceS) SR_FAIL(SR_ERR_INVALID, "sr_igemm: split = %d: nothing to split (whole rounds of workgroups only)", a.split);
    }
  }
  if (force == 2) return launch_ln<T, 128, 128, 2, 2, 2, TRANS>(a, M, Ho, Wo, st);
  if (force == 3) return launch_ln<T, 128, 64, 2, 2, 2, TRANS>(a, M, Ho, Wo, st);
  if (force == 4) return launch_ln<T, 64, 64, 2, 2, 2, TRANS>(a, M, Ho, Wo, st);
  if (force == 13) return launch_ln<T, 64, 64, 2, 2, 8, TRANS>(a, M, Ho, Wo, st);
  if (force == 14) return launch_ln<T, 128, 64, 2, 2, 6, TRANS>(a, M, Ho, Wo, st);
  if (force == 15) return launch_ln<T, 128, 128, 2, 2, 4, TRANS>(a, M, Ho, Wo, st);
  if (force == 8) {
    if constexpr (!TRANS && sizeof(T) == 2) { if (conv3p_ok(a, M)) return launch_conv3p(a, M, st); }
    SR_FAIL(SR_ERR_INVALID, "sr_igemm: tile 8 (patch-stationary 3x3) needs fp16, KH=3, stride 1, one source, N %% 320 == 0, "
                            "256-pixel tiles of whole rows / images (H=%d W=%d M=%d N=%d)", a.H, a.W, M, a.N);
  }
  if constexpr (!TRANS && sizeof(T) == 2) {
    if ((force >= 5 && force <= 7) && a.N % 320) SR_FAIL(SR_ERR_INVALID, "sr_igemm: tile %d (256x320) needs N %% 320 == 0, N=%d", force, a.N);
    if (force == 6) return launch<T, 256, 320, 4, 2, 4, TRANS, 64>(a, M, Ho, Wo, st);
    if (force == 9) {
      if (a.N % 160) SR_FAIL(SR_ERR_INVALID, "sr_igemm: tile 9 (128x160) needs N %% 160 == 0, N=%d", a.N);
      return launch_ln<T, 128, 160, 4, 2, 2, TRANS, 128, 0, 4>(a, M, Ho, Wo, st);
    }
    if (force == 10) {
      if (a.N % 320) SR_FAIL(SR_ERR_INVALID, "sr_igemm: tile 10 (128x320) needs N %% 320 == 0, N=%d", a.N);
      return launch_ln<T, 128, 320, 2, 4, 2, TRANS, 64, 0, 4>(a, M, Ho, Wo, st);
    }
    if (force == 11) return launch_ln<T, 128, 128, 4, 2, 2, TRANS, 128, 0, 4>(a, M, Ho, Wo, st);
    if (force == 12) return launch_ln<T, 256, 128, 4, 2, 2, TRANS, 64, 0, 4>(a, M, Ho, Wo, st);
    if (force == 7 || (force == 0 && a.N % 320 == 0 && (int64_t)((M + 255) / 256) * (a.N / 320) < 256 &&
                       (int64_t)((M + 127) / 128) * (a.N / 320) >= 256))
      return launch_ln<T, 128, 320, 2, 4, 2, TRANS>(a, M, Ho, Wo, st);

    if (force == 5 || (force == 0 && a.N % 320 == 0 && (int64_t)((M + 255) / 256) * (a.N / 320) >= 256))
      return launch_ln<T, 256, 320, 4, 2, 2, TRANS, 128, 2>(a, M, Ho, Wo, st);
  } else {
    if (force >= 5 && force <= 12) SR_FAIL(SR_ERR_INVALID, "sr_igemm: tile %d is fp16, non-transposed only", force);
  }
  const int64_t wg_256x128 = (int64_t)((M + 255) / 256) * n128;
  const bool big = !waste128 && wg_256x128 >= 512;
  if constexpr (!TRANS) {
    if (force == 0 && may_split && !big) {
      int tile0 = 0;
      if (!waste128) {
        const int S = plan_split(wg_128x128, KT, 512, 1.2, 128 * 128 * 4, a.workspace_bytes, &tile0);
        if (S > 1) return launch_split<T, 128, 128>(a, M, Ho, Wo, tile0, S, st);
      } else {
        const int S = plan_split((int64_t)((M + 127) / 128) * n64, KT, 768, 0.93, 128 * 64 * 4, a.workspace_bytes, &tile0);
        if (S > 1) return launch_split<T, 128, 64>(a, M, Ho, Wo, tile0, S, st);
      }
    }
  }
  if (force == 1 || (force == 0 && big && !a.ln_inline))
    return launch<T, 256, 128, 4, 2, 3, TRANS, 128, 1>(a, M, Ho, Wo, st);
  if (!waste128 && wg_128x128 >= 192 && !(a.KH == 1 && wg_128x128 <= 768)) return launch_ln<T, 128, 128, 2, 2, 2, TRANS>(a, M, Ho, Wo, st);
  const int64_t wg_128x64 = (int64_t)((M + 127) / 128) * n64;
  if (wg_128x64 >= 192) return launch_ln<T, 128, 64, 2, 2, 2, TRANS>(a, M, Ho, Wo, st);
  if ((int64_t)((M + 63) / 64) * n64 <= 256 && KT >= 4) return launch_ln<T, 64, 64, 2, 2, 8, TRANS>(a, M, Ho, Wo, st);
  return launch_ln<T, 64, 64, 2, 2, 2, TRANS>(a, M, Ho, Wo, st);
}

}

static int igemm_check(const sr_igemm_args* a, int* M_, int* Ho_, int* Wo_) {
  if (!a || !a->a || !a->w || !a->out || !a->zero_page) SR_FAIL(SR_ERR_INVALID, "sr_igemm: null pointer");
  const int ke = a->dtype == SR_F16 ? 64 : 32;
  if (a->dtype != SR_F16 && a->dtype != SR_F32) SR_FAIL(SR_ERR_INVALID, "sr_igemm: bad dtype %d", a->dtype);
  if (a->C1 <= 0 || a->C1 % ke || a->C2 % ke || a->C2 < 0) SR_FAIL(SR_ERR_INVALID, "sr_igemm: C1=%d C2=%d must be multiples of %d", a->C1, a->C2, ke);
  if (a->C2 > 0 && !a->a2) SR_FAIL(SR_ERR_INVALID, "sr_igemm: C2>0 without a2");
  if (a->KH != 1 && a->KH != 3) SR_FAIL(SR_ERR_INVALID, "sr_igemm: KH=%d", a->KH);
  if (a->stride != 1 && a->stride != 2) SR_FAIL(SR_ERR_INVALID, "sr_igemm: stride=%d", a->stride);
  if (a->upsample && a->stride != 1) SR_FAIL(SR_ERR_INVALID, "sr_igemm: upsample with stride");
  if (a->pad_br && (a->KH != 3 || a->upsample)) SR_FAIL(SR_ERR_INVALID, "sr_igemm: pad_br is for 3x3 convs without upsample");
  if (a->N <= 0 || a->B <= 0 || a->H <= 0 || a->W <= 0) SR_FAIL(SR_ERR_INVALID, "sr_igemm: bad sizes");
  if (a->act == 2 && (a->N % 4 || a->transpose_out)) SR_FAIL(SR_ERR_INVALID, "sr_igemm: GEGLU needs N%%4==0");
  if (a->row_stats && !a->colsum) SR_FAIL(SR_ERR_INVALID, "sr_igemm: row_stats without colsum");
  if (a->ln_inline && (a->row_stats || !a->colsum)) SR_FAIL(SR_ERR_INVALID, "sr_igemm: ln_inline takes colsum and no row_stats");
  if ((a->row_stats || a->ln_inline) && (a->KH != 1 || a->stride != 1 || a->upsample || a->C2)) SR_FAIL(SR_ERR_INVALID, "sr_igemm: folded LayerNorm is for 1x1 single-source layers");
  if (a->tile < 0 || a->tile > 15 || a->split < -1 || a->split == 1 || a->split > 16) SR_FAIL(SR_ERR_INVALID, "sr_igemm: tile=%d split=%d", a->tile, a->split);
  if (a->tile_order != 0 && a->tile_order != 1) SR_FAIL(SR_ERR_INVALID, "sr_igemm: tile_order=%d (0 rows first, 1 columns first)", a->tile_order);
  int Ho, Wo;
  if (a->upsample && ((a->up_h > 0) != (a->up_w > 0))) SR_FAIL(SR_ERR_INVALID, "sr_igemm: up_h / up_w go together");
  if (!a->upsample && (a->up_h || a->up_w)) SR_FAIL(SR_ERR_INVALID, "sr_igemm: up_h / up_w without upsample");
  if (a->upsample) { Ho = a->up_h > 0 ? a->up_h : 2 * a->H; Wo = a->up_w > 0 ? a->up_w : 2 * a->W; }
  else if (a->stride == 2) {
    const int ptot = a->pad_br ? a->KH / 2 : 2 * (a->KH / 2);
    Ho = (a->H + ptot - a->KH) / 2 + 1; Wo = (a->W + ptot - a->KH) / 2 + 1;
  }
  else { Ho = a->H; Wo = a->W; }
  const int64_t M64 = (int64_t)a->B * Ho * Wo;
  if (M64 > 0x7fffffffLL / 2) SR_FAIL(SR_ERR_INVALID, "sr_igemm: M too large");
  if (a->transpose_out && a->ldt < Ho * Wo) SR_FAIL(SR_ERR_INVALID, "sr_igemm: ldt < pixels per batch");
  *M_ = (int)M64; *Ho_ = Ho; *Wo_ = Wo;
  return SR_OK;
}

extern "C" int sr_igemm(const sr_igemm_args* a, void* stream) {
  int M, Ho, Wo;
  const int rc = igemm_check(a, &M, &Ho, &Wo);
  if (rc != SR_OK) return rc;
  hipStream_t st = sr_stream(stream);
  if (a->dtype == SR_F16) {
    return a->transpose_out ? dispatch<_Float16, true>(*a, M, Ho, Wo, st) : dispatch<_Float16, false>(*a, M, Ho, Wo, st);
  }
  return a->transpose_out ? dispatch<float, true>(*a, M, Ho, Wo, st) : dispatch<float, false>(*a, M, Ho, Wo, st);
}

template <typename T>
static int group_launch(int tile, const sr_igemm_args* const* as, const int* Ms, const int* Hos, const int* Wos, int n, hipStream_t st) {
  switch (tile) {
    case 2: return launch_group<T, 128, 128, 2, 2, 2>(as, Ms, Hos, Wos, n, st);
    case 3: return launch_group<T, 128, 64, 2, 2, 2>(as, Ms, Hos, Wos, n, st);
    case 4: return launch_group<T, 64, 64, 2, 2, 2>(as, Ms, Hos, Wos, n, st);
    case 13: return launch_group<T, 64, 64, 2, 2, 8>(as, Ms, Hos, Wos, n, st);
    case 14: return launch_group<T, 128, 64, 2, 2, 6>(as, Ms, Hos, Wos, n, st);
    case 15: return launch_group<T, 128, 128, 2, 2, 4>(as, Ms, Hos, Wos, n, st);
    default: break;
  }
  if constexpr (sizeof(T) == 2) {
    if (tile == 9) return launch_group<T, 128, 160, 4, 2, 2, 128, 0, 4>(as, Ms, Hos, Wos, n, st);
    if (tile == 10) return launch_group<T, 128, 320, 2, 4, 2, 64, 0, 4>(as, Ms, Hos, Wos, n, st);
  }
  return -100;
}

extern "C" int sr_igemm_group(const sr_igemm_args* const* args, int32_t n, void* stream) {
  if (!args || n < 1 || n > SR_IGEMM_GROUP_MAX) SR_FAIL(SR_ERR_INVALID, "sr_igemm_group: 1..%d problems", SR_IGEMM_GROUP_MAX);
  int M[SR_IGEMM_GROUP_MAX], Ho[SR_IGEMM_GROUP_MAX], Wo[SR_IGEMM_GROUP_MAX];
  bool one = n > 1;
  for (int i = 0; i < n; ++i) {
    const int rc = igemm_check(args[i], &M[i], &Ho[i], &Wo[i]);
    if (rc != SR_OK) return rc;
    const sr_igemm_args* a = args[i];
    one = one && a->dtype == args[0]->dtype && a->tile == args[0]->tile && a->tile != 0 && !a->transpose_out && a->split == -1;
    if (a->tile == 9) one = one && a->N % 160 == 0;
    if (a->tile == 10) one = one && a->N % 320 == 0;
  }
  hipStream_t st = sr_stream(stream);
  if (one) {
    const int rc = args[0]->dtype == SR_F16 ? group_launch<_Float16>(args[0]->tile, args, M, Ho, Wo, n, st)
                                            : group_launch<float>(args[0]->tile, args, M, Ho, Wo, n, st);
    if (rc != -100) return rc;
  }
  for (int i = 0; i < n; ++i) {
    const int rc = sr_igemm(args[i], stream);
    if (rc != SR_OK) return rc;
  }
  return SR_OK;
}
```

stable-renderer_amd/csrc/norm.hip:

```cpp
#include "sr_common.h"
#include <stdlib.h>
#include <type_traits>

namespace {

__host__ __device__ inline int gn_ppc(int HW, int B) {
  const int chunks = B >= 8 ? 64 : B >= 4 ? 128 : 256;
  const int p = (HW + chunks - 1) / chunks;
  return p < 64 ? 64 : p;
}

template <typename T>
__device__ __forceinline__ void load_chunk(const T* p, float (&v)[sr_traits<T>::EPC]) {
  if constexpr (sizeof(T) == 2) {
    const h16x8 h = *(const h16x8*)p;
#pragma unroll
    for (int e = 0; e < 8; ++e) v[e] = (float)h[e];
  } else {
    const float4 f = *(const float4*)p;
    v[0] = f.x; v[1] = f.y; v[2] = f.z; v[3] = f.w;
  }
}
template <typename T>
__device__ __forceinline__ void store_chunk(T* p, const float (&v)[sr_traits<T>::EPC]) {
  if constexpr (sizeof(T) == 2) {
    h16x8 h;
#pragma unroll
    for (int e = 0; e < 8; ++e) h[e] = (_Float16)v[e];
    *(h16x8*)p = h;
  } else {
    *(float4*)p = make_float4(v[0], v[1], v[2], v[3]);
  }
}

template <typename T>
__device__ __forceinline__ float gn_pivot(const T* x1, const T* x2, int b, int HW, int C1, int C2, int c0) {
  return c0 < C1 ? (float)x1[(int64_t)b * HW * C1 + c0] : (float)x2[(int64_t)b * HW * C2 + (c0 - C1)];
}

template <typename T>
__global__ __launch_bounds__(256) void gn_stats_kernel(const T* __restrict__ x1, const T* __restrict__ x2, float* __restrict__ partials,
                                                       int HW, int C1, int C2, int groups, int nchunk) {
  constexpr int EPC = sr_traits<T>::EPC;
  extern __shared__ __attribute__((aligned(16))) char smem_raw[];
  const int C = C1 + C2, cpt = C / EPC, cpg = C / groups;
  const int b = blockIdx.y, chunk = blockIdx.x, tid = threadIdx.x;
  const int pp_ = 256 / cpt;
  const int nps = pp_ >= 1 ? pp_ : 1;
  float* chs = (float*)smem_raw;
  float* chq = chs + nps * C;
  const int ppc = gn_ppc(HW, gridDim.y);
  const int p0 = chunk * ppc;
  const int p1 = min(HW, p0 + ppc);
  const int pp = 256 / cpt;
  if (pp >= 1) {
    const int cc = tid % cpt, ps = tid / cpt;
    if (ps < pp) {
      float s[EPC], q[EPC];
#pragma unroll
      for (int e = 0; e < EPC; ++e) { s[e] = 0.f; q[e] = 0.f; }
      const int c0 = cc * EPC;
      const T* src = c0 < C1 ? x1 + (int64_t)b * HW * C1 + c0 : x2 + (int64_t)b * HW * C2 + (c0 - C1);
      const int cs = c0 < C1 ? C1 : C2;
      float piv[EPC];
#pragma unroll
      for (int e = 0; e < EPC; ++e) piv[e] = gn_pivot<T>(x1, x2, b, HW, C1, C2, (c0 + e) / cpg * cpg);
      int p = p0 + ps;
      for (; p + 3 * pp < p1; p += 4 * pp) {
        float v0[EPC], v1[EPC], v2[EPC], v3[EPC];
        load_chunk<T>(src + (int64_t)p * cs, v0);
        load_chunk<T>(src + (int64_t)(p + pp) * cs, v1);
        load_chunk<T>(src + (int64_t)(p + 2 * pp) * cs, v2);
        load_chunk<T>(src + (int64_t)(p + 3 * pp) * cs, v3);
#pragma unroll
        for (int e = 0; e < EPC; ++e) {
          const float d0 = v0[e] - piv[e], d1 = v1[e] - piv[e], d2 = v2[e] - piv[e], d3 = v3[e] - piv[e];
          s[e] += d0; q[e] += d0 * d0;
          s[e] += d1; q[e] += d1 * d1;
          s[e] += d2; q[e] += d2 * d2;
          s[e] += d3; q[e] += d3 * d3;
        }
      }
      for (; p < p1; p += pp) {
        float v[EPC];
        load_chunk<T>(src + (int64_t)p * cs, v);
#pragma unroll
        for (int e = 0; e < EPC; ++e) { const float d = v[e] - piv[e]; s[e] += d; q[e] += d * d; }
      }
#pragma unroll
      for (int e = 0; e < EPC; ++e) { chs[ps * C + c0 + e] = s[e]; chq[ps * C + c0 + e] = q[e]; }
    }
  } else {
    for (int cc = tid; cc < cpt; cc += 256) {
      float s[EPC], q[EPC];
#pragma unroll
      for (int e = 0; e < EPC; ++e) { s[e] = 0.f; q[e] = 0.f; }
      const int c0 = cc * EPC;
      const T* src = c0 < C1 ? x1 + (int64_t)b * HW * C1 + c0 : x2 + (int64_t)b * HW * C2 + (c0 - C1);
      const int cs = c0 < C1 ? C1 : C2;
      float piv[EPC];
#pragma unroll
      for (int e = 0; e < EPC; ++e) piv[e] = gn_pivot<T>(x1, x2, b, HW, C1, C2, (c0 + e) / cpg * cpg);
      for (int p = p0; p < p1; ++p) {
        float v[EPC];
        load_chunk<T>(src + (int64_t)p * cs, v);
#pragma unroll
        for (int e = 0; e < EPC; ++e) { const float d = v[e] - piv[e]; s[e] += d; q[e] += d * d; }
      }
#pragma unroll
      for (int e = 0; e < EPC; ++e) { chs[c0 + e] = s[e]; chq[c0 + e] = q[e]; }
    }
  }
  __syncthreads();
  if (tid < groups) {
    float gs = 0.f, gq = 0.f;
    for (int ps = 0; ps < nps; ++ps)
      for (int c = tid * cpg; c < (tid + 1) * cpg; ++c) { gs += chs[ps * C + c]; gq += chq[ps * C + c]; }
    float* o = partials + (((int64_t)b * nchunk + chunk) * groups + tid) * 2;
    o[0] = gs; o[1] = gq;
  }
}

template <typename T>
__global__ __launch_bounds__(256) void gn_apply_kernel(const T* __restrict__ x1, const T* __restrict__ x2, const float* __restrict__ partials,
                                                       const float* __restrict__ gamma, const float* __restrict__ beta, T* __restrict__ y,
                                                       int HW, int C1, int C2, int groups, int nchunk, float eps, int silu) {
  constexpr int EPC = sr_traits<T>::EPC;
  extern __shared__ __attribute__((aligned(16))) char smem_raw[];
  float* sc = (float*)smem_raw;
  const int C = C1 + C2, cpt = C / EPC, cpg = C / groups;
  float* sh = sc + C;
  float* gm = sh + C;
  const int b = blockIdx.y, chunk = blockIdx.x, tid = threadIdx.x;
  const int ppc = gn_ppc(HW, gridDim.y);
  const int p0 = chunk * ppc;
  const int p1 = min(HW, p0 + ppc);
  const int total = (p1 - p0) * cpt;
  auto src_of = [&](int idx, int& c0, int& p) -> const T* {
    p = p0 + idx / cpt;
    c0 = (idx - (idx / cpt) * cpt) * EPC;
    return c0 < C1 ? x1 + ((int64_t)b * HW + p) * C1 + c0 : x2 + ((int64_t)b * HW + p) * C2 + (c0 - C1);
  };
  auto finish = [&](float (&v)[EPC], int c0, int p) {
#pragma unroll
    for (int e = 0; e < EPC; ++e) {
      float t = v[e] * sc[c0 + e] + sh[c0 + e];
      v[e] = silu ? sr_silu_f(t) : t;
    }
    store_chunk<T>(y + ((int64_t)b * HW + p) * C + c0, v);
  };
  using VEC = typename std::conditional<sizeof(T) == 2, h16x8, f32x4>::type;
  VEC pr[4];
  int pc0[4], pq0[4];
  int pre_n = 0;
#pragma unroll
  for (int i = 0; i < 4; ++i) {
    pr[i] = VEC{};
    if (tid + i * 256 < total) { pr[i] = *(const VEC*)src_of(tid + i * 256, pc0[i], pq0[i]); pre_n = i + 1; }
  }
  {
    float* red = gm + 2 * groups;
    const int g = tid & 31, part = tid >> 5;
    if (g < groups) {
      float s = 0.f, q = 0.f;
      const float* pp = partials + ((int64_t)b * nchunk * groups + g) * 2;
      for (int i = part; i < nchunk; i += 8) { s += pp[(int64_t)i * groups * 2]; q += pp[(int64_t)i * groups * 2 + 1]; }
      red[(part * groups + g) * 2] = s; red[(part * groups + g) * 2 + 1] = q;
    }
    __syncthreads();
    if (tid < groups) {
      double s = 0.0, q = 0.0;
      for (int p8 = 0; p8 < 8; ++p8) { s += red[(p8 * groups + tid) * 2]; q += red[(p8 * groups + tid) * 2 + 1]; }
      const double cnt = (double)HW * cpg;
      const double dm = s / cnt;
      double var = q / cnt - dm * dm;
      if (var < 0.0) var = 0.0;
      gm[tid] = (float)((double)gn_pivot<T>(x1, x2, b, HW, C1, C2, tid * cpg) + dm);
      gm[groups + tid] = (float)(1.0 / sqrt(var + (double)eps));
    }
  }
  __syncthreads();
  for (int c = tid; c < C; c += 256) {
    const int g = c / cpg;
    const float a = gm[groups + g] * gamma[c];
    sc[c] = a; sh[c] = beta[c] - gm[g] * a;
  }
  __syncthreads();
  int idx = tid;
#pragma unroll
  for (int i = 0; i < 4; ++i) {
    VEC r = pr[i];
    asm volatile("" : "+v"(r));
    if (i < pre_n) {
      float v[EPC];
      load_chunk<T>((const T*)&r, v);
      finish(v, pc0[i], pq0[i]);
    }
  }
  idx += pre_n * 256;
  for (; idx + 3 * 256 < total; idx += 4 * 256) {
    int c0[4], pq[4];
    float v0[EPC], v1[EPC], v2[EPC], v3[EPC];
    load_chunk<T>(src_of(idx, c0[0], pq[0]), v0);
    load_chunk<T>(src_of(idx + 256, c0[1], pq[1]), v1);
    load_chunk<T>(src_of(idx + 512, c0[2], pq[2]), v2);
    load_chunk<T>(src_of(idx + 768, c0[3], pq[3]), v3);
    finish(v0, c0[0], pq[0]); finish(v1, c0[1], pq[1]); finish(v2, c0[2], pq[2]); finish(v3, c0[3], pq[3]);
  }
  for (; idx < total; idx += 256) {
    int c0, pq;
    float v[EPC];
    load_chunk<T>(src_of(idx, c0, pq), v);
    finish(v, c0, pq);
  }
}

template <typename T, int NV, int BLOCK>
__global__ __launch_bounds__(BLOCK) void gn_fused_kernel(const T* __restrict__ x1, const T* __restrict__ x2, const float* __restrict__ gamma,
                                                         const float* __restrict__ beta, T* __restrict__ y, int HW, int C1, int C2,
                                                         int groups, int GB, float eps, int silu) {
  constexpr int EPC = sr_traits<T>::EPC;
  using VEC = typename std::conditional<sizeof(T) == 2, h16x8, f32x4>::type;
  extern __shared__ __attribute__((aligned(16))) char smem_raw[];
  const int C = C1 + C2, cpg = C / groups, span = GB * cpg, vpp = span / EPC, pp = BLOCK / vpp;
  float* chs = (float*)smem_raw;
  float* chsum = chs + pp * span;
  float* gstat = chsum + span;
  float* strip = gstat + GB;
  const int NS = BLOCK / span;
  const int nb = groups / GB, wg = sr_xcd_remap(blockIdx.x, gridDim.x);
  const int b = wg / nb, bundle = wg - b * nb, tid = threadIdx.x;
  const int cc = tid % vpp, ps = tid / vpp;
  const bool active = ps < pp;
  const int cl = cc * EPC, c0 = bundle * span + cl;
  const T* src = c0 < C1 ? x1 + (int64_t)b * HW * C1 + c0 : x2 + (int64_t)b * HW * C2 + (c0 - C1);
  const int cs = c0 < C1 ? C1 : C2;
  VEC raw[NV];
  float acc[EPC], piv[EPC];
#pragma unroll
  for (int e = 0; e < EPC; ++e) { acc[e] = 0.f; piv[e] = gn_pivot<T>(x1, x2, b, HW, C1, C2, (c0 + e) / cpg * cpg); }
#pragma unroll
  for (int i = 0; i < NV; ++i) {
    const int p = ps + i * pp;
    if (active && p < HW) {
      raw[i] = *(const VEC*)(src + (int64_t)p * cs);
      float v[EPC];
      load_chunk<T>((const T*)&raw[i], v);
#pragma unroll
      for (int e = 0; e < EPC; ++e) acc[e] += v[e] - piv[e];
    }
  }
  const float inv_cnt = 1.0f / ((float)HW * (float)cpg);
  float mean_e[EPC], rstd_e[EPC];
  for (int round = 0; round < 2; ++round) {
    if (active) {
#pragma unroll
      for (int e = 0; e < EPC; ++e) chs[ps * span + cl + e] = acc[e];
    }
    __syncthreads();
    if (tid < NS * span) {
      const int c = tid % span, s0 = tid / span;
      float t = 0.f;
      for (int q = s0; q < pp; q += NS) t += chs[q * span + c];
      strip[s0 * span + c] = t;
    }
    __syncthreads();
    if (tid < span) {
      float t = 0.f;
      for (int q = 0; q < NS; ++q) t += strip[q * span + tid];
      chsum[tid] = t;
    }
    __syncthreads();
    if (tid < GB) {
      float t = 0.f;
      for (int c = tid * cpg; c < (tid + 1) * cpg; ++c) t += chsum[c];
      gstat[tid] = round == 0 ? t * inv_cnt : rsqrtf(t * inv_cnt + eps);
    }
    __syncthreads();
    if (round == 0) {
#pragma unroll
      for (int e = 0; e < EPC; ++e) { mean_e[e] = gstat[(cl + e) / cpg]; acc[e] = 0.f; }
#pragma unroll
      for (int i = 0; i < NV; ++i) {
        const int p = ps + i * pp;
        if (active && p < HW) {
          float v[EPC];
          VEC r = raw[i];
          asm volatile("" : "+v"(r));
          load_chunk<T>((const T*)&r, v);
#pragma unroll
          for (int e = 0; e < EPC; ++e) { const float d = (v[e] - piv[e]) - mean_e[e]; acc[e] += d * d; }
        }
      }
      __syncthreads();
    } else {
#pragma unroll
      for (int e = 0; e < EPC; ++e) rstd_e[e] = gstat[(cl + e) / cpg];
    }
  }
  if (!active) return;
  float sc[EPC], sh[EPC];
#pragma unroll
  for (int e = 0; e < EPC; ++e) {
    sc[e] = rstd_e[e] * gamma[c0 + e];
    sh[e] = beta[c0 + e] - mean_e[e] * sc[e];
  }
  T* dst = y + (int64_t)b * HW * C + c0;
#pragma unroll
  for (int i = 0; i < NV; ++i) {
    const int p = ps + i * pp;
    if (p < HW) {
      float v[EPC];
      VEC r = raw[i];
// ... 295 lines not shown
  for (int i = 0; i < MAXC; ++i) {
    const int cc = lane + i * 64;
    if (cc < cpt) {
      load_chunk<T>(x + (int64_t)row * C + cc * EPC, v[i]);
#pragma unroll
      for (int e = 0; e < EPC; ++e) s += v[i][e];
    }
  }
#pragma unroll
  for (int o = 32; o > 0; o >>= 1) s += __shfl_xor(s, o);
  const float mean = s / (float)C;
  float q = 0.f;
#pragma unroll
  for (int i = 0; i < MAXC; ++i) {
    const int cc = lane + i * 64;
    if (cc < cpt) {
#pragma unroll
      for (int e = 0; e < EPC; ++e) { const float d = v[i][e] - mean; q += d * d; }
    }
  }
#pragma unroll
  for (int o = 32; o > 0; o >>= 1) q += __shfl_xor(q, o);
  if (lane == 0) {
    const float rstd = rsqrtf(q / (float)C + eps);
    *(float2*)(stats + 2 * (int64_t)row) = make_float2(rstd, -rstd * mean);
  }
}

}

extern "C" int sr_row_stats(const void* x, float* stats, int32_t rows, int32_t C, float eps, int32_t dtype, void* stream) {
  if (!x || !stats) SR_FAIL(SR_ERR_INVALID, "sr_row_stats: null pointer");
  const int epc = dtype == SR_F16 ? 8 : 4;
  if (C % epc || C / epc > 64 * 5) SR_FAIL(SR_ERR_INVALID, "sr_row_stats: C=%d unsupported", C);
  hipStream_t st = sr_stream(stream);
  dim3 grid(sr_cdiv(rows, 4));
  if (dtype == SR_F16) hipLaunchKernelGGL(row_stats_kernel<_Float16>, grid, dim3(256), 0, st, (const _Float16*)x, stats, rows, C, eps);
  else if (dtype == SR_F32) hipLaunchKernelGGL(row_stats_kernel<float>, grid, dim3(256), 0, st, (const float*)x, stats, rows, C, eps);
  else SR_FAIL(SR_ERR_INVALID, "sr_row_stats: dtype");
  SR_CHECK_LAUNCH("sr_row_stats");
  return SR_OK;
}

extern "C" int64_t sr_groupnorm_scratch_floats(int32_t B, int32_t HW) {
  int64_t need = 0;
  for (int b = 1; b <= B; ++b) {
    const int64_t n = (int64_t)b * sr_cdiv(HW, gn_ppc(HW, b)) * 64 * 2;
    need = n > need ? n : need;
  }
  return need;
}

extern "C" int sr_groupnorm(const sr_groupnorm_args* a, void* stream) {
  if (!a || !a->x || !a->y || !a->gamma || !a->beta || !a->partials) SR_FAIL(SR_ERR_INVALID, "sr_groupnorm: null pointer");
  const int epc = a->dtype == SR_F16 ? 8 : 4;
  const int C = a->C1 + a->C2;
  if (a->groups <= 0 || a->groups > 64 || C % a->groups) SR_FAIL(SR_ERR_INVALID, "sr_groupnorm: C=%d groups=%d", C, a->groups);
  if (a->C1 % epc || a->C2 % epc) SR_FAIL(SR_ERR_INVALID, "sr_groupnorm: channels must be multiples of %d", epc);
  if (a->C2 > 0 && !a->x2) SR_FAIL(SR_ERR_INVALID, "sr_groupnorm: C2>0 without x2");
  const int nchunk = sr_cdiv(a->HW, gn_ppc(a->HW, a->B));
  if (a->groups > 32) SR_FAIL(SR_ERR_INVALID, "sr_groupnorm: at most 32 groups");
  const size_t lds = (size_t)(2 * C + 2 * a->groups + 16 * a->groups) * sizeof(float);
  if (lds > 64 * 1024) SR_FAIL(SR_ERR_INVALID, "sr_groupnorm: C too large");
  hipStream_t st = sr_stream(stream);
  static const bool no_fused = getenv("SR_GN_TWO_PASS") != nullptr;
  if (!no_fused && (a->dtype == SR_F16 ? try_gn_wave<_Float16>(a, st) : a->dtype == SR_F32 ? try_gn_wave<float>(a, st) : false)) {
    SR_CHECK_LAUNCH("sr_groupnorm");
    return SR_OK;
  }
  if (!no_fused && (a->dtype == SR_F16 ? try_gn_fused<_Float16>(a, st) : a->dtype == SR_F32 ? try_gn_fused<float>(a, st) : false)) {
    SR_CHECK_LAUNCH("sr_groupnorm");
    return SR_OK;
  }
  dim3 grid(nchunk, a->B);
  const int cpt = C / epc, nps = 256 / cpt >= 1 ? 256 / cpt : 1;
  const size_t lds_stats = (size_t)2 * nps * C * sizeof(float);
  if (a->dtype == SR_F16) {
    hipLaunchKernelGGL(gn_stats_kernel<_Float16>, grid, dim3(256), lds_stats, st, (const _Float16*)a->x, (const _Float16*)a->x2, a->partials, a->HW, a->C1, a->C2, a->groups, nchunk);
    hipLaunchKernelGGL(gn_apply_kernel<_Float16>, grid, dim3(256), lds, st, (const _Float16*)a->x, (const _Float16*)a->x2, a->partials, a->gamma, a->beta,
                       (_Float16*)a->y, a->HW, a->C1, a->C2, a->groups, nchunk, a->eps, a->silu);
  } else if (a->dtype == SR_F32) {
    hipLaunchKernelGGL(gn_stats_kernel<float>, grid, dim3(256), lds_stats, st, (const float*)a->x, (const float*)a->x2, a->partials, a->HW, a->C1, a->C2, a->groups, nchunk);
    hipLaunchKernelGGL(gn_apply_kernel<float>, grid, dim3(256), lds, st, (const float*)a->x, (const float*)a->x2, a->partials, a->gamma, a->beta,
                       (float*)a->y, a->HW, a->C1, a->C2, a->groups, nchunk, a->eps, a->silu);
  } else SR_FAIL(SR_ERR_INVALID, "sr_groupnorm: dtype");
  SR_CHECK_LAUNCH("sr_groupnorm");
  return SR_OK;
}

static int layernorm_impl(const void* x, const float* gamma, const float* beta, void* y, int32_t rows, int32_t C,
                          float eps, int32_t dtype, void* stream, const ln_gather g) {
  if (!x || !y || !gamma || !beta) SR_FAIL(SR_ERR_INVALID, "sr_layernorm: null pointer");
  const int epc = dtype == SR_F16 ? 8 : 4;
  if (C % epc || C / epc > 64 * 5) SR_FAIL(SR_ERR_INVALID, "sr_layernorm: C=%d unsupported", C);
  hipStream_t st = sr_stream(stream);
  const int cpt = C / epc;
  auto go = [&](auto t, auto maxc, auto nrows) {
    using T = decltype(t);
    constexpr int MAXC = decltype(maxc)::value, ROWS = decltype(nrows)::value;
    hipLaunchKernelGGL((layernorm_kernel<T, MAXC, ROWS>), dim3(sr_cdiv(rows, 4 * ROWS)), dim3(256), 0, st, (const T*)x, gamma, beta, (T*)y, rows, C, eps, g);
  };
  using I1 = std::integral_constant<int, 1>; using I2 = std::integral_constant<int, 2>; using I3 = std::integral_constant<int, 3>;
  using I4 = std::integral_constant<int, 4>; using I5 = std::integral_constant<int, 5>;
  static const bool no_sub = getenv("SR_LN_WAVE_ROWS") != nullptr;
  auto sub = [&](auto t) -> bool {
    using T = decltype(t);
    if (no_sub) return false;
    for (int nch = 5; nch >= 1; --nch) {
      if (cpt % nch) continue;
      const int lpr = cpt / nch;
      if (lpr > 32 || (lpr & (lpr - 1))) continue;
      const dim3 grid(sr_cdiv(rows, 4 * (64 / lpr)));
#define SR_LN_SUB(L, N) hipLaunchKernelGGL((layernorm_sub_kernel<T, L, N>), grid, dim3(256), 0, st, (const T*)x, gamma, beta, (T*)y, rows, C, eps, g); return true
#define SR_LN_SUBN(L) switch (nch) { case 1: SR_LN_SUB(L, 1); case 2: SR_LN_SUB(L, 2); case 3: SR_LN_SUB(L, 3); case 4: SR_LN_SUB(L, 4); default: SR_LN_SUB(L, 5); }
      switch (lpr) {
        case 1: SR_LN_SUBN(1)
        case 2: SR_LN_SUBN(2)
        case 4: SR_LN_SUBN(4)
        case 8: SR_LN_SUBN(8)
        case 16: SR_LN_SUBN(16)
        default: SR_LN_SUBN(32)
      }
#undef SR_LN_SUBN
#undef SR_LN_SUB
    }
    return false;
  };
  if ((dtype == SR_F16 && sub(_Float16())) || (dtype == SR_F32 && sub(float()))) {
    SR_CHECK_LAUNCH("sr_layernorm");
    return SR_OK;
  }
  if (dtype == SR_F16) {
    if (cpt <= 64) go(_Float16(), I1{}, I4{}); else if (cpt <= 128) go(_Float16(), I2{}, I2{});
    else if (cpt <= 192) go(_Float16(), I3{}, I2{}); else go(_Float16(), I5{}, I1{});
  } else if (dtype == SR_F32) {
    if (cpt <= 64) go(float(), I1{}, I4{}); else if (cpt <= 128) go(float(), I2{}, I2{});
    else if (cpt <= 192) go(float(), I3{}, I2{}); else go(float(), I5{}, I1{});
  }
  else SR_FAIL(SR_ERR_INVALID, "sr_layernorm: dtype");
  SR_CHECK_LAUNCH("sr_layernorm");
  return SR_OK;
}

extern "C" int sr_layernorm(const void* x, const float* gamma, const float* beta, void* y, int32_t rows, int32_t C,
                            float eps, int32_t dtype, void* stream) {
  return layernorm_impl(x, gamma, beta, y, rows, C, eps, dtype, stream, ln_gather{nullptr, nullptr, 1, 0});
}

extern "C" int sr_layernorm_gather(const void* x, const int32_t* sel, int32_t nsel, int32_t frame_rows, int32_t n_frames, int32_t* err_flag,
                                   const float* gamma, const float* beta, void* y, int32_t C, float eps, int32_t dtype, void* stream) {
  if (!sel || nsel < 1 || frame_rows < 1 || n_frames < 1) SR_FAIL(SR_ERR_INVALID, "sr_layernorm_gather: bad selection");
  return layernorm_impl(x, gamma, beta, y, nsel * frame_rows, C, eps, dtype, stream, ln_gather{sel, err_flag, frame_rows, n_frames});
}
```

stable-renderer_amd/csrc/plan.hip:

```cpp
#include "sr_common.h"

static int run_op(const sr_op& op, void* stream) {
  switch (op.kind) {
    case SR_OP_IGEMM: return sr_igemm(&op.u.igemm, stream);
    case SR_OP_GROUPNORM: return sr_groupnorm(&op.u.gn, stream);
    case SR_OP_ATTENTION: return sr_attention(&op.u.attn, stream);
    case SR_OP_LAYERNORM:
      return sr_layernorm(op.u.ln.x, op.u.ln.gamma, op.u.ln.beta, op.u.ln.y, op.u.ln.rows, op.u.ln.C, op.u.ln.eps, op.u.ln.dtype, stream);
    case SR_OP_LAYERNORM_GATHER:
      if (op.u.ln.frame_rows < 1 || op.u.ln.rows % op.u.ln.frame_rows) { sr_set_error("sr_plan_run: layernorm_gather: rows %% frame_rows"); return SR_ERR_INVALID; }
      return sr_layernorm_gather(op.u.ln.x, op.u.ln.sel, op.u.ln.rows / op.u.ln.frame_rows, op.u.ln.frame_rows, op.u.ln.n_frames, op.u.ln.err_flag,
                                 op.u.ln.gamma, op.u.ln.beta, op.u.ln.y, op.u.ln.C, op.u.ln.eps, op.u.ln.dtype, stream);
    case SR_OP_ROW_STATS:
      return sr_row_stats(op.u.ln.x, (float*)op.u.ln.y, op.u.ln.rows, op.u.ln.C, op.u.ln.eps, op.u.ln.dtype, stream);
    case SR_OP_NCHW_TO_NHWC:
      return sr_nchw_to_nhwc((const float*)op.u.cvt.x, op.u.cvt.y, op.u.cvt.B, op.u.cvt.C, op.u.cvt.HW, op.u.cvt.Cpad, op.u.cvt.scale,
                             op.u.cvt.per_batch_scale, op.u.cvt.dtype, stream);
    case SR_OP_NHWC_TO_NCHW:
      return sr_nhwc_to_nchw(op.u.cvt.x, (float*)op.u.cvt.y, op.u.cvt.B, op.u.cvt.C, op.u.cvt.HW, op.u.cvt.ldc, op.u.cvt.dtype, stream);
    case SR_OP_TIMESTEP_EMBED:
      return sr_timestep_embedding(op.u.temb.t, op.u.temb.y, op.u.temb.B, op.u.temb.dim, op.u.temb.dtype, stream);
    case SR_OP_SILU: return sr_silu(op.u.ew.x, op.u.ew.y, op.u.ew.n, op.u.ew.dtype, stream);
    case SR_OP_SOFTMAX_ROWS: return sr_softmax_rows(op.u.ew.y, op.u.ew.rows, op.u.ew.cols, op.u.ew.dtype, stream);
    case SR_OP_ADD_SCALED: return sr_add_scaled(op.u.add.a, op.u.add.b, op.u.add.y, op.u.add.n, op.u.add.s, op.u.add.dtype, stream);
    case SR_OP_GATHER_ROWS: return sr_gather_rows(op.u.gather.x, op.u.gather.sel, op.u.gather.y, op.u.gather.nsel, op.u.gather.n_rows, op.u.gather.row_bytes,
                                                   op.u.gather.err_flag, stream);
    default: sr_set_error("sr_plan_run: unknown op kind %d", op.kind); return SR_ERR_INVALID;
  }
}

#include <map>
#include <mutex>
#include <utility>
struct sr_side { hipStream_t s = nullptr; hipEvent_t fork = nullptr, join = nullptr; };
static std::mutex g_side_mu;
static std::map<std::pair<int, void*>, sr_side> g_sides;
static int side_get(void* main_stream, sr_side* out) {
  int dev = -1;
  if (hipGetDevice(&dev) != hipSuccess) SR_FAIL(SR_ERR_LAUNCH, "side lane: hipGetDevice");
  std::lock_guard<std::mutex> lk(g_side_mu);
  const auto key = std::make_pair(dev, main_stream);
  auto it = g_sides.find(key);
  if (it == g_sides.end()) {
    sr_side sd;
    if (hipStreamCreateWithFlags(&sd.s, hipStreamNonBlocking) != hipSuccess) SR_FAIL(SR_ERR_LAUNCH, "side stream");
    if (hipEventCreateWithFlags(&sd.fork, hipEventDisableTiming) != hipSuccess || hipEventCreateWithFlags(&sd.join, hipEventDisableTiming) != hipSuccess)
      SR_FAIL(SR_ERR_LAUNCH, "side events");
    it = g_sides.emplace(key, sd).first;
  }
  *out = it->second;
  return SR_OK;
}

extern "C" int sr_plan_run(const sr_op* ops, int32_t n, void* stream) {
  if (!ops || n < 0) SR_FAIL(SR_ERR_INVALID, "sr_plan_run: bad args");
  bool side_open = false;
  sr_side sd;
  for (int i = 0; i < n; ++i) {
    if (ops[i].kind == SR_OP_FORK || ops[i].kind == SR_OP_JOIN || ops[i].lane == 1) {
      if (!sd.s && side_get(stream, &sd) != SR_OK) return SR_ERR_LAUNCH;
    }
    if (ops[i].kind == SR_OP_FORK) {
      if (hipEventRecord(sd.fork, sr_stream(stream)) != hipSuccess || hipStreamWaitEvent(sd.s, sd.fork, 0) != hipSuccess)
        SR_FAIL(SR_ERR_LAUNCH, "sr_plan_run: fork at op %d", i);
      side_open = true;
      continue;
    }
    if (ops[i].kind == SR_OP_JOIN) {
      if (side_open && (hipEventRecord(sd.join, sd.s) != hipSuccess || hipStreamWaitEvent(sr_stream(stream), sd.join, 0) != hipSuccess))
        SR_FAIL(SR_ERR_LAUNCH, "sr_plan_run: join at op %d", i);
      side_open = false;
      continue;
    }
    if (ops[i].lane == 1 && !side_open) SR_FAIL(SR_ERR_INVALID, "sr_plan_run: side-lane op %d outside FORK..JOIN", i);
    int rc;
    const int grp = ops[i].kind == SR_OP_IGEMM ? ops[i].u.igemm.group : 0;
    if (grp > 1) {
      if (grp > SR_IGEMM_GROUP_MAX || i + grp > n) SR_FAIL(SR_ERR_INVALID, "sr_plan_run: op %d: group of %d", i, grp);
      const sr_igemm_args* ptr[SR_IGEMM_GROUP_MAX];
      for (int j = 0; j < grp; ++j) {
        if (ops[i + j].kind != SR_OP_IGEMM || ops[i + j].lane != ops[i].lane) SR_FAIL(SR_ERR_INVALID, "sr_plan_run: op %d: group member %d is not an igemm op of the same lane", i, j);
        ptr[j] = &ops[i + j].u.igemm;
      }
      rc = sr_igemm_group(ptr, grp, ops[i].lane == 1 ? (void*)sd.s : stream);
      if (rc == SR_OK) { i += grp - 1; continue; }
    } else
      rc = run_op(ops[i], ops[i].lane == 1 ? (void*)sd.s : stream);
    if (rc != SR_OK) {
      char buf[400];
      snprintf(buf, sizeof(buf), "%s", sr_last_error());
      sr_set_error("plan op %d (kind %d): %s", i, ops[i].kind, buf);
      return rc;
    }
  }
  if (side_open) {
    if (hipEventRecord(sd.join, sd.s) != hipSuccess || hipStreamWaitEvent(sr_stream(stream), sd.join, 0) != hipSuccess)
      SR_FAIL(SR_ERR_LAUNCH, "sr_plan_run: final join");
  }
  return SR_OK;
}

extern "C" int sr_plan_capture(const sr_op* ops, int32_t n, void* stream, void** graph_exec) {
  if (!ops || !graph_exec || !stream) SR_FAIL(SR_ERR_INVALID, "sr_plan_capture: needs a non-default stream");
  hipStream_t st = sr_stream(stream);
  int rc = sr_plan_run(ops, n, stream);
  if (rc != SR_OK) return rc;
  if (hipStreamSynchronize(st) != hipSuccess) SR_FAIL(SR_ERR_LAUNCH, "sr_plan_capture: warm-up failed: %s", hipGetErrorString(hipGetLastError()));
  if (hipStreamBeginCapture(st, hipStreamCaptureModeThreadLocal) != hipSuccess) SR_FAIL(SR_ERR_LAUNCH, "sr_plan_capture: begin capture failed");
  rc = sr_plan_run(ops, n, stream);
  hipGraph_t graph = nullptr;
  const hipError_t e = hipStreamEndCapture(st, &graph);
  if (rc != SR_OK) { if (graph) (void)hipGraphDestroy(graph); return rc; }
  if (e != hipSuccess || !graph) SR_FAIL(SR_ERR_LAUNCH, "sr_plan_capture: end capture: %s", hipGetErrorString(e));
  hipGraphExec_t ex = nullptr;
  const hipError_t e2 = hipGraphInstantiate(&ex, graph, nullptr, nullptr, 0);
  (void)hipGraphDestroy(graph);
  if (e2 != hipSuccess) SR_FAIL(SR_ERR_LAUNCH, "sr_plan_capture: instantiate: %s", hipGetErrorString(e2));
  *graph_exec = (void*)ex;
  return SR_OK;
}

extern "C" int sr_graph_launch(void* graph_exec, void* stream) {
  if (!graph_exec) SR_FAIL(SR_ERR_INVALID, "sr_graph_launch: null");
  const hipError_t e = hipGraphLaunch((hipGraphExec_t)graph_exec, sr_stream(stream));
  if (e != hipSuccess) SR_FAIL(SR_ERR_LAUNCH, "sr_graph_launch: %s", hipGetErrorString(e));
  return SR_OK;
}

extern "C" int sr_graph_destroy(void* graph_exec) {
  if (graph_exec) (void)hipGraphExecDestroy((hipGraphExec_t)graph_exec);
  return SR_OK;
}
```

stable-renderer_amd/ops.py:

```python
import contextlib
import ctypes as C
import os
import threading

import torch

from . import _lib as L
from . import _lib_tiled as LT

DT = {torch.float16: L.SR_F16, torch.float32: L.SR_F32}
TDT = {L.SR_F16: torch.float16, L.SR_F32: torch.float32}


def _p(t):
    return None if t is None else C.c_void_p(t.data_ptr())


_raw_stream = getattr(torch._C, "_cuda_getCurrentRawStream", None)
_raw_device = getattr(torch._C, "_cuda_getDevice", None)


def stream_ptr():
    if _raw_stream is not None and _raw_device is not None:
        return C.c_void_p(_raw_stream(_raw_device()))
    return C.c_void_p(torch.cuda.current_stream().cuda_stream)


_zero_pages = {}


def zero_page(device):
    key = str(device)
    if key not in _zero_pages:
        _zero_pages[key] = torch.zeros(65536, dtype=torch.uint8, device=device)
    return _zero_pages[key]


def kelems(dtype):
    return 64 if dtype == torch.float16 else 32


def pack_conv_weight(w, dtype, cin_pad=None, geglu=False):
    if w.dim() == 2:
        w = w[:, :, None, None]
    n, cin, kh, kw = w.shape
    ke = kelems(dtype)
    cp = cin_pad if cin_pad is not None else (cin + ke - 1) // ke * ke
    if geglu:
        half = n // 2
        w = torch.stack([w[:half], w[half:]], dim=1).reshape(n, cin, kh, kw)
    wp = torch.zeros((n + 127) // 128 * 128, kh, kw, cp, dtype=torch.float32)
    wp[:n, :, :, :cin] = w.permute(0, 2, 3, 1).float()
    return wp.reshape(wp.shape[0], kh * kw * cp).to(dtype).contiguous()


def pack_bias(b, geglu=False):
    b = b.float()
    if geglu:
        half = b.shape[0] // 2
        b = torch.stack([b[:half], b[half:]], dim=1).reshape(-1)
    return b.contiguous()


_WS = {}
_tls = threading.local()


@contextlib.contextmanager
def workspace_slot(slot):
    prev = getattr(_tls, "slot", 0)
    _tls.slot = slot
    try:
        yield
    finally:
        _tls.slot = prev


def workspace(device, nbytes=64 << 20):
    key = (str(device), getattr(_tls, "slot", 0))
    if key not in _WS:
        _WS[key] = torch.empty(nbytes, dtype=torch.uint8, device=device)
    return _WS[key]


SPLIT_COUNTERS = 4096
_WSC = {}


def split_counters(device):
    key = (str(device), getattr(_tls, "slot", 0))
    if key not in _WSC:
        _WSC[key] = torch.zeros(SPLIT_COUNTERS, dtype=torch.int32, device=device)
    return _WSC[key]


def igemm_args(a, w, out, B, H, W, C1, N, KH=1, stride=1, upsample=0, a2=None, C2=0, bias=None, rowvec=None,
               residual=None, act=0, transpose_out=0, ldt=0, out_f32=0, scale=1.0, dtype=None, rowvec_ld=0, tile=0, split=0, row_stats=None, colsum=None,
               pad_br=0, up_hw=None, ln_inline=False, ln_eps=1e-5, tile_order=0):
    ar = L.IgemmArgs()
    ar.a, ar.a2, ar.w, ar.bias, ar.rowvec, ar.residual, ar.out = _p(a), _p(a2), _p(w), _p(bias), _p(rowvec), _p(residual), _p(out)
    ar.zero_page = _p(zero_page(a.device))
    ar.B, ar.H, ar.W, ar.C1, ar.C2, ar.N, ar.KH, ar.stride, ar.upsample = B, H, W, C1, C2, N, KH, stride, upsample
    ar.act, ar.transpose_out, ar.ldt, ar.out_f32 = act, transpose_out, ldt, out_f32
    ar.dtype = DT[a.dtype if dtype is None else dtype]
    ar.scale = scale
    ar.rowvec_ld = rowvec_ld
    ar.tile, ar.split, ar.pad_br, ar.tile_order = tile, split, pad_br, tile_order
    ar.up_h, ar.up_w = (0, 0) if (up_hw is None or tuple(up_hw) == (2 * H, 2 * W)) else (int(up_hw[0]), int(up_hw[1]))
    ar.row_stats, ar.colsum = _p(row_stats), _p(colsum)
    ar.ln_inline, ar.ln_eps = int(bool(ln_inline)), ln_eps
    ws = workspace(a.device)
    ar.workspace, ar.workspace_bytes = _p(ws), ws.numel()
    if os.environ.get("SR_SPLIT_FIXUP", "0") == "1":
        ar.split_counters = _p(split_counters(a.device))
    return ar


def igemm(*a, **k):
    ar = igemm_args(*a, **k)
    L.check(L.lib().sr_igemm(C.byref(ar), stream_ptr()))


_TUNED = {}
_TUNE_CACHE = os.environ.get("SR_AUTOTUNE_CACHE")
if _TUNE_CACHE and os.path.exists(_TUNE_CACHE):
    import json as _json
    with open(_TUNE_CACHE) as _f:
        _TUNED.update({tuple(_json.loads(k)): tuple(v) for k, v in _json.load(_f).items()})


def load_tune_table(path):
    import json as _json
    with open(path) as f:
        _TUNED.update({tuple(_json.loads(k)): tuple(v) for k, v in _json.load(f).items()})


def save_tune_table(path):
    import json as _json
    with open(path, "w") as f:
        _json.dump({_json.dumps([int(x) for x in k]): list(v) for k, v in sorted(_TUNED.items())}, f, indent=0)


for _tbl in filter(None, os.environ.get("SR_AUTOTUNE_TABLES", "").split(os.pathsep)):
    if os.path.exists(_tbl):
        load_tune_table(_tbl)
if os.environ.get("SR_AUTOTUNE_DUMP"):
    import atexit as _atexit
    _atexit.register(lambda: save_tune_table("%s.%d.json" % (os.environ["SR_AUTOTUNE_DUMP"], os.getpid())))


_CANDIDATES = ((0, 0), (0, -1), (1, -1), (2, 0), (2, -1), (2, 2), (2, 3), (2, 4), (2, 6), (2, 8), (3, 0), (3, -1), (3, 2), (3, 3), (3, 4), (3, 6), (3, 8), (4, -1), (5, -1), (6, -1), (7, -1), (8, -1), (9, -1), (10, -1), (11, -1), (12, -1),
               (13, -1), (14, -1), (14, 2), (14, 3), (14, 4), (14, 5), (15, -1), (15, 2), (15, 3), (15, 4), (15, 5))


def autotune_enabled():
    return os.environ.get("SR_AUTOTUNE", "1") != "0" and torch.cuda.is_available()


_TUNE_COLD = os.environ.get("SR_TUNE_COLD", "1") == "1"
_FLUSH = {}


def _tune_cold(ar, sig, allow_split, reps):
    lib, st = L.lib(), stream_ptr()
    dev = torch.cuda.current_device()
    if dev not in _FLUSH:
        _FLUSH[dev] = torch.empty(320 << 20, dtype=torch.uint8, device="cuda")
    flush = _FLUSH[dev]

    es = 2 if ar.dtype == L.SR_F16 else 4
    Ho, Wo = ((ar.up_h or 2 * ar.H), (ar.up_w or 2 * ar.W)) if ar.upsample else ((ar.H + ar.stride - 1) // ar.stride, (ar.W + ar.stride - 1) // ar.stride)
    warm = [(ar.a, ar.B * ar.H * ar.W * ar.C1 * es)]
    if ar.a2 and ar.C2:
        warm.append((ar.a2, ar.B * ar.H * ar.W * ar.C2 * es))
    if ar.residual:
        warm.append((ar.residual, ar.B * Ho * Wo * (ar.N // 2 if ar.act == 2 else ar.N) * es))

    def timed(n):
        tot = 0.0
        for _ in range(n):
            flush.add_(1)
            for ptr, nbytes in warm:
                lib.sr_cache_touch(ptr, nbytes, st)
            e0, e1 = torch.cuda.Event(enable_timing=True), torch.cuda.Event(enable_timing=True)
            e0.record()
            lib.sr_igemm(C.byref(ar), st)
            e1.record()
            e1.synchronize()
            tot += e0.elapsed_time(e1)
        return tot / n
    times = {}
    for tile, split in _CANDIDATES:
        if ((ar.act == 2 or ar.transpose_out) and split >= 0 and tile != 0) or (not allow_split and split >= 0):
            continue
        ar.tile, ar.split = tile, split
        if lib.sr_igemm(C.byref(ar), st) != 0:
            continue
        times[(tile, split)] = timed(reps)
    for c in sorted(times, key=times.get)[:4]:
        ar.tile, ar.split = c
        times[c] = min(times[c], timed(3 * reps))
    best, best_t = (0, 0 if allow_split else -1), None
    for c in _CANDIDATES:
        if c in times and (best_t is None or times[c] < best_t * 0.97):
            best, best_t = c, times[c]
    order = 0
    w_bytes = ar.N * ar.KH * ar.KH * (ar.C1 + ar.C2) * es
    a_bytes = ar.B * ar.H * ar.W * (ar.C1 + ar.C2) * es
    if best_t is not None and w_bytes > 2 * a_bytes and os.environ.get("SR_TUNE_ORDER", "1") == "1":
        ar.tile, ar.split = best
        t0 = min(best_t, timed(3 * reps))
        ar.tile_order = 1
        if lib.sr_igemm(C.byref(ar), st) == 0 and timed(3 * reps) < float(os.environ.get("SR_TUNE_ORDER_MARGIN", "0.97")) * t0:
            order = 1
        ar.tile_order = 0
    _TUNED[sig] = best + ((1,) if order else ())
    if _TUNE_CACHE:
        import json as _json
        with open(_TUNE_CACHE, "w") as _f:
            _json.dump({_json.dumps([int(x) for x in k]): list(v) for k, v in _TUNED.items()}, _f)
    if os.environ.get("SR_AUTOTUNE_LOG"):
        print(f"[tune cold] B{ar.B} {ar.H}x{ar.W} C{ar.C1}+{ar.C2} N{ar.N} k{ar.KH} s{ar.stride} u{ar.upsample} act{ar.act} "
              f"t{ar.transpose_out} -> tile {best[0]} split {best[1]} order {order}  {best_t * 1e3:.1f} us", flush=True)


def tune_igemm(ar, min_flops=2.0e8, reps=4, allow_split=True):
    Ho, Wo = ((ar.up_h or 2 * ar.H), (ar.up_w or 2 * ar.W)) if ar.upsample else ((ar.H + ar.stride - 1) // ar.stride, (ar.W + ar.stride - 1) // ar.stride)
    flops = 2.0 * ar.B * Ho * Wo * ar.N * ar.KH * ar.KH * (ar.C1 + ar.C2)
    if flops < min_flops:
        return
    sig = _sig(ar, allow_split)
    if sig not in _TUNED and _TUNE_COLD:
        _tune_cold(ar, sig, allow_split, reps)
    if sig not in _TUNED:
        lib, st = L.lib(), stream_ptr()
        times = {}
        for rnd in range(2):
            for tile, split in _CANDIDATES:
                if (ar.act == 2 or ar.transpose_out) and split >= 0 and tile != 0:
                    continue
                if not allow_split and split >= 0:
                    continue
                if rnd == 1 and (tile, split) not in times:
                    continue
                ar.tile, ar.split = tile, split
                if lib.sr_igemm(C.byref(ar), st) != 0:
                    continue
                n = reps if rnd == 0 else max(reps, min(40, int(1.0 / max(times[(tile, split)], 1e-3))))
                e0, e1 = torch.cuda.Event(enable_timing=True), torch.cuda.Event(enable_timing=True)
                e0.record()
                for _ in range(n):
                    lib.sr_igemm(C.byref(ar), st)
                e1.record()
                e1.synchronize()
                t = e0.elapsed_time(e1) / n
                times[(tile, split)] = min(t, times.get((tile, split), t)) if rnd == 1 else t
        for tile, split in sorted(times, key=times.get)[:3]:
            ar.tile, ar.split = tile, split
            n = max(2 * reps, min(80, int(2.0 / max(times[(tile, split)], 1e-3))))
            e0, e1 = torch.cuda.Event(enable_timing=True), torch.cuda.Event(enable_timing=True)
            e0.record()
            for _ in range(n):
                lib.sr_igemm(C.byref(ar), st)
            e1.record()
            e1.synchronize()
            times[(tile, split)] = min(times[(tile, split)], e0.elapsed_time(e1) / n)
        best, best_t = (0, 0 if allow_split else -1), None
        for c in _CANDIDATES:
            if c in times and (best_t is None or times[c] < best_t * 0.97):
                best, best_t = c, times[c]
        _TUNED[sig] = best
        if _TUNE_CACHE:
            import json as _json
            with open(_TUNE_CACHE, "w") as _f:
                _json.dump({_json.dumps([int(x) for x in k]): list(v) for k, v in _TUNED.items()}, _f)
        if os.environ.get("SR_AUTOTUNE_LOG"):
            print(f"[tune] B{ar.B} {ar.H}x{ar.W} C{ar.C1}+{ar.C2} N{ar.N} k{ar.KH} s{ar.stride} u{ar.upsample} act{ar.act} "
                  f"t{ar.transpose_out} -> tile {best[0]} split {best[1]}  {best_t * 1e3:.1f} us", flush=True)
    v = _TUNED[sig]
    ar.tile, ar.split, ar.tile_order = v[0], v[1], (v[2] if len(v) > 2 else 0)


GROUP_TILES = (4, 13, 3, 14, 2, 15, 9, 10)
GROUP_MAX = 4


def _sig(ar, allow_split=True):
    return (ar.dtype, ar.B, ar.H, ar.W, ar.C1, ar.C2, ar.N, ar.KH, ar.stride, ar.upsample, ar.act, ar.transpose_out, ar.out_f32,
            bool(ar.residual), bool(ar.rowvec), bool(allow_split), bool(ar.row_stats) + 2 * ar.ln_inline, ar.pad_br, ar.up_h, ar.up_w)


def igemm_group(ars, stream=None):
    arr = (C.POINTER(L.IgemmArgs) * len(ars))(*[C.pointer(a) for a in ars])
    L.check(L.lib().sr_igemm_group(arr, len(ars), stream_ptr() if stream is None else stream))


def tune_group(ars, reps=4):
    n = len(ars)
    if n < 2 or n > GROUP_MAX or not autotune_enabled() or os.environ.get("SR_IGEMM_GROUPS", "1") == "0":
        return False
    if any(a.transpose_out for a in ars) or len({a.dtype for a in ars}) != 1:
        return False
    key = (-7, n) + tuple(x for a in ars for x in _sig(a))
    if key not in _TUNED:
        lib, st = L.lib(), stream_ptr()
        dev = torch.cuda.current_device()
        if dev not in _FLUSH:
            _FLUSH[dev] = torch.empty(320 << 20, dtype=torch.uint8, device="cuda")
        flush = _FLUSH[dev]
        warm = []
        for ar in ars:
            es = 2 if ar.dtype == L.SR_F16 else 4
            warm.append((ar.a, ar.B * ar.H * ar.W * ar.C1 * es))
            if ar.a2 and ar.C2:
                warm.append((ar.a2, ar.B * ar.H * ar.W * ar.C2 * es))
        arr = (C.POINTER(L.IgemmArgs) * n)(*[C.pointer(a) for a in ars])

        def timed(fn, k):
            tot = 0.0
            for _ in range(k):
                flush.add_(1)
                for ptr, nbytes in warm:
                    lib.sr_cache_touch(ptr, nbytes, st)
                e0, e1 = torch.cuda.Event(enable_timing=True), torch.cuda.Event(enable_timing=True)
                e0.record()
                fn()
                e1.record()
                e1.synchronize()
                tot += e0.elapsed_time(e1)
            return tot / k
        own = [(a.tile, a.split) for a in ars]

        def seq():
            for a in ars:
                lib.sr_igemm(C.byref(a), st)
        seq()
        t_seq = min(timed(seq, reps), timed(seq, reps))
        times = {}
        for t in GROUP_TILES:
            if (t == 9 and any(a.N % 160 for a in ars)) or (t == 10 and any(a.N % 320 for a in ars)) or (t in (9, 10) and ars[0].dtype != L.SR_F16):
                continue
            for a in ars:
                a.tile, a.split = t, -1
            if lib.sr_igemm_group(arr, n, st) != 0:
                continue
            times[t] = timed(lambda: lib.sr_igemm_group(arr, n, st), reps)
        for t in sorted(times, key=times.get)[:2]:
            for a in ars:
                a.tile, a.split = t, -1
            times[t] = min(times[t], timed(lambda: lib.sr_igemm_group(arr, n, st), 2 * reps))
        for a, (t, sp) in zip(ars, own):
            a.tile, a.split = t, sp
        best = min(times, key=times.get) if times else 0
        _TUNED[key] = (best, -1) if (times and times[best] < 0.97 * t_seq) else (0, -1)
        if _TUNE_CACHE:
            import json as _json
            with open(_TUNE_CACHE, "w") as _f:
                _json.dump({_json.dumps([int(x) for x in k]): list(v) for k, v in _TUNED.items()}, _f)
        if os.environ.get("SR_AUTOTUNE_LOG"):
            print("[tune group] " + " | ".join(f"B{a.B} {a.H}x{a.W} C{a.C1}+{a.C2} N{a.N} k{a.KH}" for a in ars)
                  + f" -> seq {t_seq * 1e3:.1f} us, grouped " + " ".join(f"{t}:{v * 1e3:.1f}" for t, v in sorted(times.items()))
                  + f" -> {_TUNED[key][0]}", flush=True)
    tile = _TUNED[key][0]
    if tile == 0:
        return False
    for a in ars:
        a.tile, a.split, a.group = tile, -1, 0
    ars[0].group = n
    return True


def groupnorm_args(x, gamma, beta, y, B, HW, C1, partials, x2=None, C2=0, groups=32, eps=1e-5, silu=False):
    ar = L.GroupNormArgs()
    ar.x, ar.x2, ar.gamma, ar.beta, ar.y, ar.partials = _p(x), _p(x2), _p(gamma), _p(beta), _p(y), _p(partials)
    ar.B, ar.HW, ar.C1, ar.C2, ar.groups, ar.silu, ar.dtype, ar.eps = B, HW, C1, C2, groups, int(silu), DT[x.dtype], eps
    return ar


def groupnorm(x, gamma, beta, B, HW, C1, x2=None, C2=0, groups=32, eps=1e-5, silu=False):
    y = torch.empty(B, HW, C1 + C2, dtype=x.dtype, device=x.device)
    partials = torch.empty(L.lib().sr_groupnorm_scratch_floats(B, HW), dtype=torch.float32, device=x.device)
    ar = groupnorm_args(x, gamma, beta, y, B, HW, C1, partials, x2, C2, groups, eps, silu)
    L.check(L.lib().sr_groupnorm(C.byref(ar), stream_ptr()))
    return y


def row_stats(x, eps=1e-5):
    rows, Cc = x.numel() // x.shape[-1], x.shape[-1]
    st = torch.empty(rows, 2, dtype=torch.float32, device=x.device)
    L.check(L.lib().sr_row_stats(_p(x), _p(st), rows, Cc, eps, DT[x.dtype], stream_ptr()))
    return st


def fold_layernorm(w, bias, gamma, beta, dtype, geglu=False):
    w32 = w.float() * gamma.float()[None, :]
    wq = w32.to(dtype).float()
    colsum = wq.sum(1)
    b2 = w.float() @ beta.float()
    if bias is not None:
        b2 = b2 + bias.float()
    return pack_conv_weight(w32, dtype, geglu=geglu), pack_bias(colsum, geglu=geglu), pack_bias(b2, geglu=geglu)


def layernorm(x, gamma, beta, eps=1e-5):
    rows, Cc = x.numel() // x.shape[-1], x.shape[-1]
    y = torch.empty_like(x)
    L.check(L.lib().sr_layernorm(_p(x), _p(gamma), _p(beta), _p(y), rows, Cc, eps, DT[x.dtype], stream_ptr()))
    return y


def attention_args(q, k, vt, o, B, Bk, Tq, Tk, heads, d, ldt, q_stride=None, k_stride=None, scale=None):
    ar = L.AttentionArgs()
    ar.q, ar.k, ar.vt, ar.o = _p(q), _p(k), _p(vt), _p(o)
    ar.B, ar.Bk, ar.Tq, ar.Tk, ar.heads, ar.d, ar.ldt, ar.dtype = B, Bk, Tq, Tk, heads, d, ldt, DT[q.dtype]
    ar.q_stride = heads * d if q_stride is None else q_stride
    ar.k_stride = heads * d if k_stride is None else k_stride
    ar.scale = d ** -0.5 if scale is None else scale
    return ar


def attention(q, k, vt, heads, Tk=None):
    B, Tq, Cc = q.shape
    Bk = k.shape[0]
    Tk = k.shape[1] if Tk is None else Tk
    d = Cc // heads
    o = torch.empty_like(q)
    ar = attention_args(q, k, vt, o, B, Bk, Tq, Tk, heads, d, vt.shape[-1])
    L.check(L.lib().sr_attention(C.byref(ar), stream_ptr()))
    return o


def nchw_to_nhwc(x, dtype, cpad=None, scale=1.0, per_batch_scale=None):
    B, Cc, H, W = x.shape
    cpad = Cc if cpad is None else cpad
    y = torch.empty(B, H * W, cpad, dtype=dtype, device=x.device)
    L.check(L.lib().sr_nchw_to_nhwc(_p(x), _p(y), B, Cc, H * W, cpad, scale, _p(per_batch_scale), DT[dtype], stream_ptr()))
    return y


def nhwc_to_nchw(x, B, Cc, H, W, ldc=None):
    y = torch.empty(B, Cc, H, W, dtype=torch.float32, device=x.device)
    L.check(L.lib().sr_nhwc_to_nchw(_p(x), _p(y), B, Cc, H * W, Cc if ldc is None else ldc, DT[x.dtype], stream_ptr()))
    return y


def timestep_embedding(t, dim, dtype):
    y = torch.empty(t.shape[0], dim, dtype=dtype, device=t.device)
    L.check(L.lib().sr_timestep_embedding(_p(t), _p(y), t.shape[0], dim, DT[dtype], stream_ptr()))
    return y


def idmap_masks(ids):
    m = torch.empty(ids.shape[:-1], dtype=torch.float32, device=ids.device)
    L.check(L.lib().sr_idmap_masks(_p(ids), _p(m), m.numel(), stream_ptr()))
    return m


class OverlapIndex:

    def __init__(self, ids, lh, lw):
        assert ids.dtype == torch.int32 and ids.is_contiguous() and ids.dim() == 4 and ids.shape[-1] == 4
        self.ids = ids
        self.N, self.H, self.W = ids.shape[:3]
        self.lh, self.lw = lh, lw
        dev = ids.device
        self.pix_cell = torch.empty(self.N * self.H * self.W, dtype=torch.int32, device=dev)
        self.cell_vid = torch.empty(self.N * lh * lw, dtype=torch.int32, device=dev)
        info = torch.zeros(4, dtype=torch.int32, device=dev)
        L.check(L.lib().sr_overlap_build(_p(ids), self.N, self.H, self.W, lh, lw, _p(self.pix_cell), _p(self.cell_vid),
                                         _p(info), stream_ptr()))
        max_vid, oob, nvalid, _ = info.tolist()
        if oob:
            raise IndexError("id-map pixel maps outside the latent (non-square frame?): index out of bounds")
        self.n_valid = nvalid
        self.cap = max_vid + 1
        lib = L.lib()
        self.vid_off = torch.empty(self.cap + 1, dtype=torch.int32, device=dev)
        self.entries = torch.empty(max(nvalid, 1), dtype=torch.int32, device=dev)
        scratch = torch.empty(lib.sr_overlap_csr_scratch_ints(self.cap), dtype=torch.int32, device=dev)
        L.check(lib.sr_overlap_csr(_p(ids), _p(self.pix_cell), self.N, self.H, self.W, self.cap, _p(self.vid_off), _p(self.entries),
                                   _p(scratch), stream_ptr()))
        self.blended = None

    def step(self, x, ratio, blended_out=None):
        assert x.dtype == torch.float32 and x.is_contiguous() and tuple(x.shape[2:]) == (self.lh, self.lw) and x.shape[0] == self.N
        Cc = x.shape[1]
        bl = blended_out
        if bl is None:
            if self.blended is None or self.blended.shape != x.shape:
                self.blended = torch.empty_like(x)
            bl = self.blended
        assert bl.dtype == torch.float32 and bl.is_contiguous() and bl.shape == x.shape
        L.check(L.lib().sr_overlap_step(_p(x), _p(self.cell_vid), _p(self.vid_off), _p(self.entries), self.N, Cc, self.lh, self.lw,
                                        self.cap, float(ratio), _p(bl), stream_ptr()))
        return x


def adain_nchw(content, style, eps=1e-5):
    N, Cc = content.shape[:2]
    hwc, hws = content[0, 0].numel(), style[0, 0].numel()
    content, style = content.contiguous(), style.contiguous()
    out = torch.empty_like(content, dtype=torch.float32)
    L.check(L.lib().sr_adain(_p(content), 1, hwc, Cc * hwc, hwc, _p(style), DT[style.dtype], 1, hws, Cc * hws, hws,
                             _p(out), N, Cc, eps, None, stream_ptr()))
    return out


def noise_pool(noise_f16, alpha_f16, bg_f32, magnitude=8):
    H, W = noise_f16.shape[1:3]
    m = int(magnitude)
    pooled = torch.empty(H // m, W // m, 4, dtype=torch.float32, device=noise_f16.device)
    out = torch.empty(1, 4, H // m, W // m, dtype=torch.float32, device=noise_f16.device)
    key = ("np", str(noise_f16.device), getattr(_tls, "slot", 0))
    if key not in _WS:
        _WS[key] = torch.empty(2048, dtype=torch.float32, device=noise_f16.device)
    if m == 8:
        L.check(L.lib().sr_noise_pool(_p(noise_f16), _p(alpha_f16), _p(bg_f32), _p(pooled), _p(out), H, W, _p(_WS[key]), stream_ptr()))
    else:
        L.check(L.lib().sr_noise_pool_strips(_p(noise_f16), _p(alpha_f16), _p(bg_f32), _p(pooled), _p(out), H, W, m * m, _p(_WS[key]), stream_ptr()))
    return pooled, out


def eps_scale_input(x, xin, copies, sigma):
    L.check(L.lib().sr_eps_scale_input(_p(x), _p(xin), x.numel(), copies, float(sigma), stream_ptr()))


def cfg_denoise(x, eps, den, d, copies, sigma, cfg):
    L.check(L.lib().sr_cfg_denoise(_p(x), _p(eps), _p(den), _p(d), x.numel(), copies, float(sigma), float(cfg), stream_ptr()))


def cond_crop_scale(x, xin, area, chunks, sigma):
# ... 67 lines not shown
```

stable-renderer_amd/plan.py:

```python
import ctypes as C
import os

import torch

from . import _lib as L
from . import ops as O


def igemm_algorithmic_bytes(ar):
    es = 2 if ar.dtype == L.SR_F16 else 4
    st, up = max(ar.stride, 1), ar.upsample
    Ho, Wo = ((ar.up_h, ar.up_w) if ar.up_h else (2 * ar.H, 2 * ar.W)) if up else ((ar.H + st - 1) // st, (ar.W + st - 1) // st)
    M, C = ar.B * Ho * Wo, ar.C1 + ar.C2
    n_out = ar.N // 2 if ar.act == 2 else ar.N
    return (ar.B * ar.H * ar.W * C * es + ar.N * ar.KH * ar.KH * C * es + M * n_out * (4 if ar.out_f32 else es)
            + (M * n_out * es if ar.residual else 0))


class Plan:
    def __init__(self, op_list, keep, op_flops=None):
        self.op_flops = list(op_flops) if op_flops is not None else [0] * len(op_list)
        self.n = len(op_list)
        self.ops = (L.Op * max(self.n, 1))(*op_list)
        self._keep = keep
        self._graph = None
        self._graph_stream = None

    def run(self):
        L.check(L.lib().sr_plan_run(self.ops, self.n, O.stream_ptr()))

    def igemm_bytes(self):
        return sum(igemm_algorithmic_bytes(self.ops[i].u.igemm) for i in range(self.n) if self.ops[i].kind == L.OP_IGEMM)

    def subset(self, kind):
        idx = [i for i in range(self.n) if self.ops[i].kind == kind]
        sel = []
        for i in idx:
            op = L.Op()
            C.memmove(C.byref(op), C.byref(self.ops[i]), C.sizeof(L.Op))
            op.lane = 0
            sel.append(op)
        return Plan(sel, self._keep, [self.op_flops[i] for i in idx])

    def capture(self, stream):
        ge = C.c_void_p()
        L.check(L.lib().sr_plan_capture(self.ops, self.n, C.c_void_p(stream.cuda_stream), C.byref(ge)))
        self._graph, self._graph_stream = ge, stream

    def launch(self):
        if self._graph is None:
            return self.run()
        L.check(L.lib().sr_graph_launch(self._graph, O.stream_ptr()))

    def __del__(self):
        try:
            if self._graph is not None:
                L.lib().sr_graph_destroy(self._graph)
        except Exception:
            pass


class PlanBuilder:

    def __init__(self, device, dtype):
        self.device, self.dtype = device, dtype
        self.ops = []
        self.op_flops = []
        self.keep = []
        self._gn_scratch = None
        self.flops = 0
        self._lane = 0
        self.two_lanes = os.environ.get("SR_TWO_LANES", "0") == "1"
        self.prefetch = os.environ.get("SR_PREFETCH", "0") == "1"
        self._prev_igemm = None

    def fork(self):
        if self.two_lanes:
            self._emit(L.OP_FORK, None, None)

    def join(self):
        if self.two_lanes:
            self._emit(L.OP_JOIN, None, None)

    def side(self):
        pb = self

        class _Side:
            def __enter__(self_inner):
                pb._lane = 1 if pb.two_lanes else 0

            def __exit__(self_inner, *a):
                pb._lane = 0
        return _Side()

    def buf(self, *shape, dtype=None, zero=False):
        t = (torch.zeros if zero else torch.empty)(*shape, dtype=dtype or self.dtype, device=self.device)
        self.keep.append(t)
        return t

    def hold(self, *ts):
        self.keep.extend(t for t in ts if t is not None)

    def _emit(self, kind, field, args):
        op = L.Op()
        op.kind = kind
        op.lane = self._lane if field is not None else 0
        if field is not None:
            setattr(op.u, field, args)
        self.ops.append(op)
        self.op_flops.append(0)

    def igemm(self, a, w, out, B, H, W, C1, N, **kw):
        self.hold(a, w, out, kw.get("a2"), kw.get("bias"), kw.get("rowvec"), kw.get("residual"), kw.get("row_stats"), kw.get("colsum"))
        if (kw.get("KH", 1) == 1 and kw.get("stride", 1) == 1 and not kw.get("upsample", 0) and kw.get("rowvec") is None
                and not kw.get("transpose_out", 0)):
            B, H, W = B * H * W, 1, 1
        ar = O.igemm_args(a, w, out, B, H, W, C1, N, dtype=self.dtype, **kw)
        if self._lane == 1:
            ar.split = -1
        if O.autotune_enabled():
            O.tune_igemm(ar, allow_split=self._lane == 0)
        self._emit(L.OP_IGEMM, "igemm", ar)
        if self.prefetch and w.is_cuda:
            prev, self._prev_igemm = self._prev_igemm, self.ops[-1]
            if prev is not None and prev.u.igemm.w != w.data_ptr():
                prev.u.igemm.prefetch = w.data_ptr()
                prev.u.igemm.prefetch_bytes = min(w.numel() * w.element_size(), 48 << 20)
        KH, st, up = kw.get("KH", 1), kw.get("stride", 1), kw.get("upsample", 0)
        Ho, Wo = (tuple(kw["up_hw"]) if kw.get("up_hw") else (2 * H, 2 * W)) if up else ((H + st - 1) // st, (W + st - 1) // st)
        f = 2 * B * Ho * Wo * N * KH * KH * (C1 + kw.get("C2", 0))
        self.flops += f
        self.op_flops[-1] = f

    def igemm_group(self, calls):
        first = len(self.ops)
        for args, kw in calls:
            self.igemm(*args, **kw)
        members = [op.u.igemm for op in self.ops[first:]]
        if self._lane == 0 and len(members) == len(calls):
            O.tune_group(members)

    def groupnorm(self, x, gamma, beta, y, B, HW, C1, x2=None, C2=0, eps=1e-5, silu=False):
        need = L.lib().sr_groupnorm_scratch_floats(B, HW)
        if self._gn_scratch is None or self._gn_scratch.numel() < need:
            self._gn_scratch = self.buf(need, dtype=torch.float32)
        self.hold(x, x2, gamma, beta, y)
        self._emit(L.OP_GROUPNORM, "gn", O.groupnorm_args(x, gamma, beta, y, B, HW, C1, self._gn_scratch, x2, C2, 32, eps, silu))

    def layernorm(self, x, gamma, beta, y, rows, Cc, eps=1e-5):
        self.hold(x, gamma, beta, y)
        a = L._Ln()
        a.x, a.gamma, a.beta, a.y = O._p(x), O._p(gamma), O._p(beta), O._p(y)
        a.rows, a.C, a.dtype, a.eps = rows, Cc, O.DT[self.dtype], eps
        self._emit(L.OP_LAYERNORM, "ln", a)

    def layernorm_gather(self, x, sel, nsel, frame_rows, n_frames, gamma, beta, y, Cc, err_flag=None, eps=1e-5):
        self.hold(x, sel, gamma, beta, y, err_flag)
        a = L._Ln()
        a.x, a.gamma, a.beta, a.y = O._p(x), O._p(gamma), O._p(beta), O._p(y)
        a.rows, a.C, a.dtype, a.eps = nsel * frame_rows, Cc, O.DT[self.dtype], eps
        a.sel, a.err_flag, a.frame_rows, a.n_frames = O._p(sel), O._p(err_flag), frame_rows, n_frames
        self._emit(L.OP_LAYERNORM_GATHER, "ln", a)

    def row_stats(self, x, stats, rows, Cc, eps=1e-5):
        self.hold(x, stats)
        a = L._Ln()
        a.x, a.gamma, a.beta, a.y = O._p(x), None, None, O._p(stats)
        a.rows, a.C, a.dtype, a.eps = rows, Cc, O.DT[x.dtype], eps
        self._emit(L.OP_ROW_STATS, "ln", a)

    def attention(self, q, k, vt, o, B, Bk, Tq, Tk, heads, d, ldt):
        self.hold(q, k, vt, o)
        self._emit(L.OP_ATTENTION, "attn", O.attention_args(q, k, vt, o, B, Bk, Tq, Tk, heads, d, ldt))
        self.flops += 4 * B * heads * Tq * Tk * d
        self.op_flops[-1] = 4 * B * heads * Tq * Tk * d

    def nchw_to_nhwc(self, x, y, B, Cc, HW, Cpad, scale=1.0):
        self.hold(x, y)
        a = L._Cvt()
        a.x, a.y, a.per_batch_scale = O._p(x), O._p(y), None
        a.B, a.C, a.HW, a.Cpad, a.dtype, a.ldc, a.scale = B, Cc, HW, Cpad, O.DT[y.dtype], Cpad, scale
        self._emit(L.OP_NCHW_TO_NHWC, "cvt", a)

    def nhwc_to_nchw(self, x, y, B, Cc, HW, ldc):
        self.hold(x, y)
        a = L._Cvt()
        a.x, a.y, a.per_batch_scale = O._p(x), O._p(y), None
        a.B, a.C, a.HW, a.Cpad, a.dtype, a.ldc, a.scale = B, Cc, HW, ldc, O.DT[x.dtype], ldc, 1.0
        self._emit(L.OP_NHWC_TO_NCHW, "cvt", a)

    def timestep_embedding(self, t, y, B, dim):
        self.hold(t, y)
        a = L._Temb()
        a.t, a.y, a.B, a.dim, a.dtype = O._p(t), O._p(y), B, dim, O.DT[y.dtype]
        self._emit(L.OP_TIMESTEP_EMBED, "temb", a)

    def silu(self, x, y):
        self.hold(x, y)
        a = L._Ew()
        a.x, a.y, a.n, a.dtype = O._p(x), O._p(y), x.numel(), O.DT[x.dtype]
        self._emit(L.OP_SILU, "ew", a)

    def softmax_rows(self, x, rows, cols):
        self.hold(x)
        a = L._Ew()
        a.x, a.y, a.n, a.dtype, a.rows, a.cols = O._p(x), O._p(x), x.numel(), O.DT[x.dtype], rows, cols
        self._emit(L.OP_SOFTMAX_ROWS, "ew", a)

    def add(self, a, b, y, s=1.0):
        self.hold(a, b, y)
        ar = L._Add()
        ar.a, ar.b, ar.y, ar.n, ar.s, ar.dtype = O._p(a), O._p(b), O._p(y), a.numel(), s, O.DT[a.dtype]
        self._emit(L.OP_ADD_SCALED, "add", ar)

    def gather_rows(self, x, sel, y, nsel, row_bytes, n_rows, err_flag=None):
        self.hold(x, sel, y, err_flag)
        a = L._Gather()
        a.x, a.y, a.sel, a.row_bytes, a.nsel, a.n_rows, a.err_flag = O._p(x), O._p(y), O._p(sel), row_bytes, nsel, n_rows, O._p(err_flag)
        self._emit(L.OP_GATHER_ROWS, "gather", a)

    def take(self):
        p = Plan(self.ops, list(self.keep), self.op_flops)
        self.ops = []
        self.op_flops = []
        self._prev_igemm = None
        return p
```

Baseline: 21.84.

## Compute GroupNorm statistics in the producing GEMM epilogue

The fp16 igemm/conv epilogue now accumulates per-group shifted sum and sum-of-squares partials for each output tile and writes one record per (image, chunk, group). A new groupnorm-from-partials path merges these records, either inside the apply kernel or through a small finalize kernel, so GroupNorm no longer needs its own statistics pass over the activation. The plan builder enables this by default when the producer GEMM's tile geometry and group layout qualify. The trade is extra epilogue work, more LDS use and extra barriers in the GEMM, plus added tile-compatibility constraints.

```diff
diff --git a/include/sr_hip.h b/include/sr_hip.h
--- a/include/sr_hip.h
+++ b/include/sr_hip.h
@@ -56,11 +56,15 @@
   int32_t ln_inline;
   float ln_eps;
   int32_t tile_order;
+  float* gn_partials;
+  int32_t gn_cpg;
+  int32_t gn_hw;
 } sr_igemm_args;
 #define SR_IGEMM_SPLIT_COUNTERS 4096
 #define SR_IGEMM_GROUP_MAX 4
 int sr_igemm(const sr_igemm_args* args, void* stream);
 int sr_igemm_group(const sr_igemm_args* const* args, int32_t n, void* stream);
+int32_t sr_igemm_gn_chunks(const sr_igemm_args* args);
 
 typedef struct {
   const void* x; const void* x2;
@@ -69,8 +73,11 @@
   float* partials;
   int32_t B, HW, C1, C2, groups, silu, dtype;
   float eps;
+  float* stats;
+  int32_t stat_chunks;
 } sr_groupnorm_args;
 int sr_groupnorm(const sr_groupnorm_args* args, void* stream);
+int sr_groupnorm_from_partials(const sr_groupnorm_args* args, void* stream);
 int64_t sr_groupnorm_scratch_floats(int32_t B, int32_t HW);
 
 int sr_row_stats(const void* x, float* stats, int32_t rows, int32_t C, float eps, int32_t dtype, void* stream);
diff --git a/stable-renderer_amd/_lib.py b/stable-renderer_amd/_lib.py
--- a/stable-renderer_amd/_lib.py
+++ b/stable-renderer_amd/_lib.py
@@ -21,12 +21,14 @@
                 ("KH", i32), ("stride", i32), ("upsample", i32), ("act", i32), ("transpose_out", i32), ("ldt", i32),
                 ("out_f32", i32), ("dtype", i32), ("scale", f32), ("rowvec_ld", i32), ("workspace", vp),
                 ("workspace_bytes", C.c_int64), ("row_stats", vp), ("colsum", vp), ("tile", i32), ("split", i32), ("pad_br", i32),
-                ("prefetch", vp), ("prefetch_bytes", C.c_int64), ("up_h", i32), ("up_w", i32), ("split_counters", vp), ("group", i32), ("ln_inline", i32), ("ln_eps", f32), ("tile_order", i32)]
+                ("prefetch", vp), ("prefetch_bytes", C.c_int64), ("up_h", i32), ("up_w", i32), ("split_counters", vp), ("group", i32), ("ln_inline", i32), ("ln_eps", f32), ("tile_order", i32),
+                ("gn_partials", vp), ("gn_cpg", i32), ("gn_hw", i32)]
 
 
 class GroupNormArgs(C.Structure):
     _fields_ = [("x", vp), ("x2", vp), ("gamma", vp), ("beta", vp), ("y", vp), ("partials", vp), ("B", i32),
-                ("HW", i32), ("C1", i32), ("C2", i32), ("groups", i32), ("silu", i32), ("dtype", i32), ("eps", f32)]
+                ("HW", i32), ("C1", i32), ("C2", i32), ("groups", i32), ("silu", i32), ("dtype", i32), ("eps", f32),
+                ("stats", vp), ("stat_chunks", i32)]
 
 
 class AttentionArgs(C.Structure):
@@ -102,8 +104,10 @@
     "sr_layernorm_gather": (C.c_int, [vp, vp, i32, i32, i32, vp, vp, vp, vp, i32, f32, i32, vp]),
     "sr_igemm": (C.c_int, [P(IgemmArgs), vp]),
     "sr_igemm_group": (C.c_int, [P(P(IgemmArgs)), i32, vp]),
+    "sr_igemm_gn_chunks": (i32, [P(IgemmArgs)]),
     "sr_groupnorm": (C.c_int, [P(GroupNormArgs), vp]),
     "sr_groupnorm_scratch_floats": (i64, [i32, i32]),
+    "sr_groupnorm_from_partials": (C.c_int, [P(GroupNormArgs), vp]),
     "sr_layernorm": (C.c_int, [vp, vp, vp, vp, i32, i32, f32, i32, vp]),
     "sr_row_stats": (C.c_int, [vp, vp, i32, i32, f32, i32, vp]),
     "sr_attention": (C.c_int, [P(AttentionArgs), vp]),
diff --git a/stable-renderer_amd/csrc/igemm.hip b/stable-renderer_amd/csrc/igemm.hip
--- a/stable-renderer_amd/csrc/igemm.hip
+++ b/stable-renderer_amd/csrc/igemm.hip
@@ -19,7 +19,7 @@
   return *(const float2*)(p.row_stats + 2 * (int64_t)m);
 }
 
-template <typename T, int BM, int BN, int WAVES_M, int WAVES_N, int LDS_AVAIL, bool GEGLU, int VCAP, bool VECPRE>
+template <typename T, int BM, int BN, int WAVES_M, int WAVES_N, int LDS_AVAIL, bool GEGLU, int VCAP, bool VECPRE, bool GN = false>
 __device__ __forceinline__ void epilogue_rows_h(const sr_igemm_args& p, f32x4 (&acc)[BN / WAVES_N / 16][BM / WAVES_M / 16], char* smem, const int M,
                                                 const int rpb, const int m0, const int n0, const int pm0, const int qn0, const int wv,
                                                 const int lane) {
@@ -51,6 +51,11 @@
   const int ncol = (GEGLU ? ((n0 + qn0) >> 1) : (n0 + qn0)) + lc * 8;
   const bool lane_on = lr < RPI && ncol < ldo;
   const int tid = wv * 64 + lane;
+  typedef float gn_f2 __attribute__((ext_vector_type(2)));
+  [[maybe_unused]] gn_f2 gcs[4] = {}, gcq[4] = {}, gcp[4] = {};
+  [[maybe_unused]] float gpv0 = 0.f, gpv1 = 0.f;
+  [[maybe_unused]] const int gcpg = GN ? p.gn_cpg : 1;
+  [[maybe_unused]] const int gg0 = (lc * 8) / gcpg, geb = (gg0 + 1) * gcpg - lc * 8;
 
   float4 vb = make_float4(0.f, 0.f, 0.f, 0.f), vc = make_float4(0.f, 0.f, 0.f, 0.f);
   if constexpr (!VECPRE) {
@@ -142,6 +147,24 @@
         raw = __builtin_bit_cast(uint4, hv);
       }
       *(uint4*)((_Float16*)p.out + oi) = raw;
+      if constexpr (GN) {
+        if (ps == 0 && it == 0) {
+          if (lr == 0) *(uint4*)(wl + lc * 16) = raw;
+          __builtin_amdgcn_s_waitcnt(0xC07F);
+          __builtin_amdgcn_wave_barrier();
+          gpv0 = (float)*(const _Float16*)(wl + gg0 * gcpg * 2);
+          gpv1 = (float)*(const _Float16*)(wl + ((gg0 + 1) * gcpg < OCOLS ? (gg0 + 1) * gcpg : gg0 * gcpg) * 2);
+#pragma unroll
+          for (int k = 0; k < 4; ++k) gcp[k] = gn_f2{2 * k < geb ? gpv0 : gpv1, 2 * k + 1 < geb ? gpv0 : gpv1};
+        }
+        const h16x8 hv = __builtin_bit_cast(h16x8, raw);
+#pragma unroll
+        for (int k = 0; k < 4; ++k) {
+          const gn_f2 d = gn_f2{(float)hv[2 * k], (float)hv[2 * k + 1]} - gcp[k];
+          gcs[k] += d;
+          gcq[k] = d * d + gcq[k];
+        }
+      }
     }
     if constexpr (ROLL) {
 #pragma unroll
@@ -149,9 +172,65 @@
     }
     __builtin_amdgcn_wave_barrier();
   }
-}
-
-template <typename T, int BM, int BN, int WAVES_M, int WAVES_N, int LDS_AVAIL, bool BLOCK_SYNC = true, int VCAP = 256, bool VECPRE = false>
+  if constexpr (GN) {
+    static_assert(!GEGLU, "statistics of a GEGLU output are not built");
+    constexpr int GPW_MAX = WCOLS / 4, NGT_MAX = BN / 4;
+    static_assert(NW * 1024 + NW * GPW_MAX * 4 + WAVES_M * NGT_MAX * 16 <= LDS_ROWS, "statistics fold staging");
+    char* const gbase = smem + (VECPRE ? 0 : VEC_B);
+    float4* const wred = (float4*)gbase;
+    float* const wpiv = (float*)(gbase + NW * 1024);
+    double* const dred = (double*)(gbase + NW * 1024 + NW * GPW_MAX * 4);
+    const int gpw = WCOLS / gcpg, ngt = BN / gcpg;
+    float gs0 = 0.f, gq0 = 0.f, gs1 = 0.f, gq1 = 0.f;
+#pragma unroll
+    for (int e = 0; e < 8; ++e) {
+      if (e < geb) { gs0 += gcs[e >> 1][e & 1]; gq0 += gcq[e >> 1][e & 1]; }
+      else { gs1 += gcs[e >> 1][e & 1]; gq1 += gcq[e >> 1][e & 1]; }
+    }
+    __syncthreads();
+    wred[wv * 64 + lane] = make_float4(gs0, gq0, gs1, gq1);
+    if (lane_on && lr == 0) {
+      wpiv[wv * GPW_MAX + gg0] = gpv0;
+      if (gg0 + 1 < gpw) wpiv[wv * GPW_MAX + gg0 + 1] = gpv1;
+    }
+    __syncthreads();
+    for (int t = tid; t < ngt * WAVES_M; t += NW * 64) {
+      const int fm = t / ngt, gl = t - fm * ngt, fn = gl / gpw, gw = gl - fn * gpw, w = fm * WAVES_N + fn;
+      const int ca = gw * gcpg, lcA = ca >> 3, lcB = (ca + gcpg - 1) >> 3;
+      float2 fv[RPI][3];
+#pragma unroll
+      for (int r = 0; r < RPI; ++r)
+#pragma unroll
+        for (int j = 0; j < 3; ++j) {
+          const int c = lcA + j <= lcB ? lcA + j : lcB;
+          const float4 v = wred[w * 64 + r * CPR + c];
+          const int gg = (c * 8) / gcpg;
+          fv[r][j] = lcA + j > lcB ? make_float2(0.f, 0.f) : gg == gw ? make_float2(v.x, v.y) : gg + 1 == gw ? make_float2(v.z, v.w) : make_float2(0.f, 0.f);
+        }
+      double fs = 0.0, fq = 0.0;
+#pragma unroll
+      for (int r = 0; r < RPI; ++r)
+#pragma unroll
+        for (int j = 0; j < 3; ++j) { fs += (double)fv[r][j].x; fq += (double)fv[r][j].y; }
+      const double d = (double)wpiv[w * GPW_MAX + gw] - (double)wpiv[fn * GPW_MAX + gw], nw = (double)((BM / WAVES_M) * gcpg);
+      dred[t * 2] = fs + nw * d;
+      dred[t * 2 + 1] = fq + 2.0 * d * fs + nw * d * d;
+    }
+    __syncthreads();
+    const int gimg = m0 / p.gn_hw, gchunks = p.gn_hw / BM, gchunk = (m0 - gimg * p.gn_hw) / BM;
+    for (int gl = tid; gl < ngt; gl += NW * 64) {
+      if (n0 + gl * gcpg >= N) continue;
+      double fs = 0.0, fq = 0.0;
+#pragma unroll
+      for (int fm = 0; fm < WAVES_M; ++fm) { fs += dred[(fm * ngt + gl) * 2]; fq += dred[(fm * ngt + gl) * 2 + 1]; }
+      const int fn = gl / gpw, gw = gl - fn * gpw;
+      const int64_t rec = ((int64_t)gimg * gchunks + gchunk) * (N / gcpg) + (n0 / gcpg + gl);
+      *(float4*)(p.gn_partials + rec * 4) = make_float4(wpiv[fn * GPW_MAX + gw], (float)fs, (float)fq, 0.f);
+    }
+  }
+}
+
+template <typename T, int BM, int BN, int WAVES_M, int WAVES_N, int LDS_AVAIL, bool BLOCK_SYNC = true, int VCAP = 256, bool VECPRE = false, bool GN = false>
 __device__ __forceinline__ void epilogue_rows(const sr_igemm_args& p, f32x4 (&acc)[BN / WAVES_N / 16][BM / WAVES_M / 16], char* smem, const int M,
                                               const int rpb, const int m0, const int n0, const int pm0, const int qn0, const int wv,
                                               const int lane) {
@@ -160,7 +239,10 @@
   const float scale = p.scale;
   const int N = p.N;
   const int ldr = p.rowvec_ld ? p.rowvec_ld : N;
-  {
+  if constexpr (GN) {
+    static_assert(sizeof(T) == 2 && BLOCK_SYNC, "GroupNorm statistics come from the fp16 row-major epilogue");
+    epilogue_rows_h<T, BM, BN, WAVES_M, WAVES_N, LDS_AVAIL, false, VCAP, VECPRE, true>(p, acc, smem, M, rpb, m0, n0, pm0, qn0, wv, lane);
+  } else {
     const int ldo = (p.act == 2) ? (N >> 1) : N;
     const bool o32 = p.out_f32 || sizeof(T) == 4;
     const int oes = o32 ? 4 : 2;
@@ -322,7 +404,7 @@
   asm volatile("s_waitcnt vmcnt(0)" ::: "memory");
 }
 
-template <typename T, int BM, int BN, int WAVES_M, int WAVES_N, int STAGES, bool TRANS, bool SPLIT = false, int BKB = 128, int SPREAD = 0, int MINB = 1, bool LNI = false>
+template <typename T, int BM, int BN, int WAVES_M, int WAVES_N, int STAGES, bool TRANS, bool SPLIT = false, int BKB = 128, int SPREAD = 0, int MINB = 1, bool LNI = false, bool GN = false>
 __device__ __forceinline__ void igemm_body(const sr_igemm_args& p, const int M, const int Ho, const int Wo,
                                            const int NT, const int nwg, const int tile0, const int bid, const int nblk) {
   extern __shared__ __attribute__((aligned(16))) char smem_all[];
@@ -657,7 +739,7 @@
     epilogue_rows<T, BM, BN, WAVES_M, WAVES_N, STAGES * STAGE_BYTES, true, (MINB >= 4 ? 128 : 256), VECPRE>(p, acc, smem, M, rpb, m0, n0, pm0, qn0, wv, lane);
     return;
   } else if constexpr (!TRANS) {
-    epilogue_rows<T, BM, BN, WAVES_M, WAVES_N, STAGES * STAGE_BYTES, true, (MINB >= 4 ? 128 : 256), VECPRE>(p, acc, smem, M, rpb, m0, n0, pm0, qn0, wv, lane);
+    epilogue_rows<T, BM, BN, WAVES_M, WAVES_N, STAGES * STAGE_BYTES, true, (MINB >= 4 ? 128 : 256), VECPRE, GN>(p, acc, smem, M, rpb, m0, n0, pm0, qn0, wv, lane);
 #if SR_IGEMM_TRACE
     SR_TS(4);
     asm volatile("s_waitcnt vmcnt(0)" ::: "memory");
@@ -701,10 +783,10 @@
   }
 }
 
-template <typename T, int BM, int BN, int WAVES_M, int WAVES_N, int STAGES, bool TRANS, bool SPLIT = false, int BKB = 128, int SPREAD = 0, int MINB = 1, bool LNI = false>
+template <typename T, int BM, int BN, int WAVES_M, int WAVES_N, int STAGES, bool TRANS, bool SPLIT = false, int BKB = 128, int SPREAD = 0, int MINB = 1, bool LNI = false, bool GN = false>
 __global__ __launch_bounds__(WAVES_M * WAVES_N * 64, MINB) void igemm_kernel(const sr_igemm_args p, const int M, const int Ho, const int Wo,
                                                                         const int NT, const int nwg, const int tile0) {
-  igemm_body<T, BM, BN, WAVES_M, WAVES_N, STAGES, TRANS, SPLIT, BKB, SPREAD, MINB, LNI>(p, M, Ho, Wo, NT, nwg, tile0, blockIdx.x, gridDim.x);
+  igemm_body<T, BM, BN, WAVES_M, WAVES_N, STAGES, TRANS, SPLIT, BKB, SPREAD, MINB, LNI, GN>(p, M, Ho, Wo, NT, nwg, tile0, blockIdx.x, gridDim.x);
 }
 
 struct igemm_group_k {
@@ -757,7 +839,7 @@
   return launch_group_impl<T, BM, BN, WAVES_M, WAVES_N, STAGES, BKB, SPREAD, MINB, false>(as, Ms, Hos, Wos, n, st);
 }
 
-template <typename T, int BM, int BN, int WAVES_M, int WAVES_N, int STAGES, bool TRANS, int BKB, int SPREAD, int MINB, bool LNI>
+template <typename T, int BM, int BN, int WAVES_M, int WAVES_N, int STAGES, bool TRANS, int BKB, int SPREAD, int MINB, bool LNI, bool GN = false>
 int launch_impl(const sr_igemm_args& a, int M, int Ho, int Wo, hipStream_t st) {
   const int Npad = (a.N + 127) / 128 * 128;
   const int MT = (M + BM - 1) / BM, NT = Npad / BN;
@@ -768,7 +850,7 @@
   constexpr int lds_epi = lds_epi_all <= lds_stage ? lds_epi_all : WAVES_M * WAVES_N * 16 * ((BN / WAVES_N) * 4 + 16);
   constexpr int lds = (lds_stage > lds_epi ? lds_stage : lds_epi) + (sizeof(T) == 2 ? 2 * BN * 4 : 0)
                       + WAVES_M * WAVES_N * 256;
-  auto k = igemm_kernel<T, BM, BN, WAVES_M, WAVES_N, STAGES, TRANS, false, BKB, SPREAD, MINB, LNI>;
+  auto k = igemm_kernel<T, BM, BN, WAVES_M, WAVES_N, STAGES, TRANS, false, BKB, SPREAD, MINB, LNI, GN>;
   static bool attr_set = false;
   if (!attr_set) { (void)hipFuncSetAttribute((const void*)k, hipFuncAttributeMaxDynamicSharedMemorySize, lds); attr_set = true; }
   (void)NT;
@@ -861,6 +943,7 @@
   return SR_OK;
 }
 
+template <bool GN = false>
 __global__ __launch_bounds__(512, 1) void conv3p_kernel(const sr_igemm_args p, const int M, const int NT, const int nwg) {
   using T = _Float16;
   extern __shared__ __attribute__((aligned(16))) char smem_all[];
@@ -980,7 +1063,7 @@
   for (int c = 0; c < NC - 1; ++c) chunk(std::false_type{}, c);
   chunk(std::true_type{}, NC - 1);
 
-  epilogue_rows<T, BM, BN, WAVES_M, WAVES_N, LDS_TOTAL>(p, acc, smem, M, rpb, m0, n0, pm0, qn0, wv, lane);
+  epilogue_rows<T, BM, BN, WAVES_M, WAVES_N, LDS_TOTAL, true, 256, false, GN>(p, acc, smem, M, rpb, m0, n0, pm0, qn0, wv, lane);
 }
 
 static bool conv3p_ok(const sr_igemm_args& a, int M) {
@@ -994,12 +1077,13 @@
   return ipt * (Ri + 2) * (a.W + 2) * 80 <= 32768;
 }
 
+template <bool GN = false>
 static int launch_conv3p(const sr_igemm_args& a, int M, hipStream_t st) {
   constexpr int lds = 2 * 32768 + 4 * 320 * 64 + 8 * 256;
   const int NT = a.N / 320, nwg = (M / 256) * NT;
   static bool attr_set = false;
-  if (!attr_set) { (void)hipFuncSetAttribute((const void*)conv3p_kernel, hipFuncAttributeMaxDynamicSharedMemorySize, lds); attr_set = true; }
-  hipLaunchKernelGGL(conv3p_kernel, dim3(nwg), dim3(512), lds, st, a, M, NT, nwg);
+  if (!attr_set) { (void)hipFuncSetAttribute((const void*)conv3p_kernel<GN>, hipFuncAttributeMaxDynamicSharedMemorySize, lds); attr_set = true; }
+  hipLaunchKernelGGL(conv3p_kernel<GN>, dim3(nwg), dim3(512), lds, st, a, M, NT, nwg);
   SR_CHECK_LAUNCH("sr_igemm(conv3p)");
   return SR_OK;
 }
@@ -1023,6 +1107,43 @@
     if (t < best * 0.9) { best = t; bestS = S; }
   }
   return bestS;
+}
+
+static bool gn_tile_geometry(int tile, int* BM, int* BN, int* WCOLS) {
+  switch (tile) {
+    case 5: case 8: *BM = 256; *BN = 320; *WCOLS = 160; return true;
+    case 9: *BM = 128; *BN = 160; *WCOLS = 80; return true;
+    case 10: *BM = 128; *BN = 320; *WCOLS = 80; return true;
+    case 11: *BM = 128; *BN = 128; *WCOLS = 64; return true;
+    case 12: *BM = 256; *BN = 128; *WCOLS = 64; return true;
+    default: return false;
+  }
+}
+static int gn_chunks(const sr_igemm_args& a, int M, int Ho, int Wo) {
+  int BM, BN, WCOLS;
+  if (!gn_tile_geometry(a.tile, &BM, &BN, &WCOLS)) return 0;
+  if (a.dtype != SR_F16 || a.transpose_out || a.out_f32 || a.act == 2 || a.split > 1 || a.group > 1 || a.row_stats || a.ln_inline) return 0;
+  const int cpg = a.gn_cpg, hw = a.gn_hw;
+  if (cpg < 4 || (cpg > 4 && cpg < 8) || a.N % cpg || a.N % 8 || BN % cpg || WCOLS % cpg) return 0;
+  if (hw <= 0 || hw % BM || M % hw || (Ho * Wo > 1 && hw != Ho * Wo)) return 0;
+  if ((a.tile == 5 || a.tile == 10) && a.N % 320) return 0;
+  if (a.tile == 9 && a.N % 160) return 0;
+  if (a.tile == 8 && !conv3p_ok(a, M)) return 0;
+  return hw / BM;
+}
+static int dispatch_gn(const sr_igemm_args& a, int M, int Ho, int Wo, hipStream_t st) {
+  using T = _Float16;
+  if (gn_chunks(a, M, Ho, Wo) == 0)
+    SR_FAIL(SR_ERR_INVALID, "sr_igemm: gn_partials is not built for this call (tile %d, N %d, gn_cpg %d, gn_hw %d, act %d, split %d: see sr_igemm_gn_chunks)",
+            a.tile, a.N, a.gn_cpg, a.gn_hw, a.act, a.split);
+  switch (a.tile) {
+    case 5: return launch_impl<T, 256, 320, 4, 2, 2, false, 128, 2, 1, false, true>(a, M, Ho, Wo, st);
+    case 8: return launch_conv3p<true>(a, M, st);
+    case 9: return launch_impl<T, 128, 160, 4, 2, 2, false, 128, 0, 4, false, true>(a, M, Ho, Wo, st);
+    case 10: return launch_impl<T, 128, 320, 2, 4, 2, false, 64, 0, 4, false, true>(a, M, Ho, Wo, st);
+    case 11: return launch_impl<T, 128, 128, 4, 2, 2, false, 128, 0, 4, false, true>(a, M, Ho, Wo, st);
+    default: return launch_impl<T, 256, 128, 4, 2, 2, false, 64, 0, 4, false, true>(a, M, Ho, Wo, st);
+  }
 }
 
 template <typename T, bool TRANS>
@@ -1159,10 +1280,17 @@
   const int rc = igemm_check(a, &M, &Ho, &Wo);
   if (rc != SR_OK) return rc;
   hipStream_t st = sr_stream(stream);
+  if (a->gn_partials) return dispatch_gn(*a, M, Ho, Wo, st);
   if (a->dtype == SR_F16) {
     return a->transpose_out ? dispatch<_Float16, true>(*a, M, Ho, Wo, st) : dispatch<_Float16, false>(*a, M, Ho, Wo, st);
   }
   return a->transpose_out ? dispatch<float, true>(*a, M, Ho, Wo, st) : dispatch<float, false>(*a, M, Ho, Wo, st);
+}
+
+extern "C" int32_t sr_igemm_gn_chunks(const sr_igemm_args* a) {
+  int M, Ho, Wo;
+  if (igemm_check(a, &M, &Ho, &Wo) != SR_OK) return 0;
+  return gn_chunks(*a, M, Ho, Wo);
 }
 
 template <typename T>
@@ -1191,6 +1319,7 @@
     const int rc = igemm_check(args[i], &M[i], &Ho[i], &Wo[i]);
     if (rc != SR_OK) return rc;
     const sr_igemm_args* a = args[i];
+    if (a->gn_partials) SR_FAIL(SR_ERR_INVALID, "sr_igemm_group: member %d asks for GroupNorm statistics (gn_partials): not built for grouped launches", i);
     one = one && a->dtype == args[0]->dtype && a->tile == args[0]->tile && a->tile != 0 && !a->transpose_out && a->split == -1;
     if (a->tile == 9) one = one && a->N % 160 == 0;
     if (a->tile == 10) one = one && a->N % 320 == 0;
diff --git a/stable-renderer_amd/csrc/norm.hip b/stable-renderer_amd/csrc/norm.hip
--- a/stable-renderer_amd/csrc/norm.hip
+++ b/stable-renderer_amd/csrc/norm.hip
@@ -121,7 +121,28 @@
   }
 }
 
-template <typename T>
+struct gn_moments { double n, mean, m2; };
+__device__ __forceinline__ void gn_merge(gn_moments& a, const gn_moments& b) {
+  if (b.n == 0.0) return;
+  if (a.n == 0.0) { a = b; return; }
+  const double nt = a.n + b.n, d = b.mean - a.mean, w = (double)__builtin_amdgcn_rcpf((float)nt) * b.n;
+  a.mean += d * w;
+  a.m2 += b.m2 + d * d * (a.n * w);
+  a.n = nt;
+}
+__device__ __forceinline__ gn_moments gn_merge_records(const float* __restrict__ rec, int b, int g, int groups, int nchunk, double n, int part, int nparts) {
+  gn_moments m = {0.0, 0.0, 0.0};
+  const float4* r = (const float4*)rec + (int64_t)b * nchunk * groups + g;
+  const double inv_n = 1.0 / n;
+  for (int i = part; i < nchunk; i += nparts) {
+    const float4 v = r[(int64_t)i * groups];
+    const double sm = (double)v.y * inv_n;
+    gn_merge(m, gn_moments{n, (double)v.x + sm, (double)v.z - (double)v.y * sm});
+  }
+  return m;
+}
+
+template <typename T, int SRC = 0>
 __global__ __launch_bounds__(256) void gn_apply_kernel(const T* __restrict__ x1, const T* __restrict__ x2, const float* __restrict__ partials,
                                                        const float* __restrict__ gamma, const float* __restrict__ beta, T* __restrict__ y,
                                                        int HW, int C1, int C2, int groups, int nchunk, float eps, int silu) {
@@ -158,7 +179,26 @@
     pr[i] = VEC{};
     if (tid + i * 256 < total) { pr[i] = *(const VEC*)src_of(tid + i * 256, pc0[i], pq0[i]); pre_n = i + 1; }
   }
-  {
+  if constexpr (SRC == 1) {
+    gn_moments* red = (gn_moments*)(gm + 2 * groups);
+    const int g = tid & 31, part = tid >> 5;
+    const double n = (double)HW * cpg / nchunk;
+    if (g < groups) red[part * groups + g] = gn_merge_records(partials, b, g, groups, nchunk, n, part, 8);
+    __syncthreads();
+    if (tid < groups) {
+      gn_moments m = red[tid];
+      for (int p8 = 1; p8 < 8; ++p8) gn_merge(m, red[p8 * groups + tid]);
+      double var = m.m2 / m.n;
+      if (var < 0.0) var = 0.0;
+      gm[tid] = (float)m.mean;
+      gm[groups + tid] = (float)(1.0 / sqrt(var + (double)eps));
+    }
+  } else if constexpr (SRC == 2) {
+    if (tid < groups) {
+      const float2 st = *(const float2*)(partials + ((int64_t)b * groups + tid) * 2);
+      gm[tid] = st.x; gm[groups + tid] = st.y;
+    }
+  } else {
     float* red = gm + 2 * groups;
     const int g = tid & 31, part = tid >> 5;
     if (g < groups) {
@@ -760,3 +800,48 @@
   if (!sel || nsel < 1 || frame_rows < 1 || n_frames < 1) SR_FAIL(SR_ERR_INVALID, "sr_layernorm_gather: bad selection");
   return layernorm_impl(x, gamma, beta, y, nsel * frame_rows, C, eps, dtype, stream, ln_gather{sel, err_flag, frame_rows, n_frames});
 }
+
+namespace {
+
+__global__ __launch_bounds__(64) void gn_finalize_kernel(const float* __restrict__ rec, float* __restrict__ stats, int HW, int cpg, int groups,
+                                                         int nchunk, float eps) {
+  __shared__ gn_moments red[64];
+  const int g = blockIdx.x, b = blockIdx.y, lane = threadIdx.x;
+  red[lane] = gn_merge_records(rec, b, g, groups, nchunk, (double)HW * cpg / nchunk, lane, 64);
+  __syncthreads();
+  for (int st = 32; st >= 1; st >>= 1) {
+    if (lane < st) { gn_moments m = red[lane]; gn_merge(m, red[lane + st]); red[lane] = m; }
+    __syncthreads();
+  }
+  if (lane == 0) {
+    double var = red[0].m2 / red[0].n;
+    if (var < 0.0) var = 0.0;
+    *(float2*)(stats + ((int64_t)b * groups + g) * 2) = make_float2((float)red[0].mean, (float)(1.0 / sqrt(var + (double)eps)));
+  }
+}
+
+}
+
+extern "C" int sr_groupnorm_from_partials(const sr_groupnorm_args* a, void* stream) {
+  if (!a || !a->x || !a->y || !a->gamma || !a->beta || !a->partials) SR_FAIL(SR_ERR_INVALID, "sr_groupnorm_from_partials: null pointer");
+  if (a->dtype != SR_F16 || a->C2 != 0 || a->x2) SR_FAIL(SR_ERR_INVALID, "sr_groupnorm_from_partials: fp16, one source");
+  const int C = a->C1;
+  if (a->groups <= 0 || a->groups > 32 || C % a->groups || C % 8) SR_FAIL(SR_ERR_INVALID, "sr_groupnorm_from_partials: C=%d groups=%d", C, a->groups);
+  if (a->B <= 0 || a->HW <= 0 || a->stat_chunks <= 0 || a->HW % a->stat_chunks) SR_FAIL(SR_ERR_INVALID, "sr_groupnorm_from_partials: HW=%d stat_chunks=%d", a->HW, a->stat_chunks);
+  const bool merged = a->stat_chunks > 64;
+  if (merged && !a->stats) SR_FAIL(SR_ERR_INVALID, "sr_groupnorm_from_partials: %d chunks per image need the stats scratch", a->stat_chunks);
+  const size_t lds = (size_t)(2 * C + 2 * a->groups) * sizeof(float) + (merged ? 0 : (size_t)8 * a->groups * sizeof(gn_moments));
+  if (lds > 64 * 1024) SR_FAIL(SR_ERR_INVALID, "sr_groupnorm_from_partials: C too large");
+  hipStream_t st = sr_stream(stream);
+  const dim3 grid(sr_cdiv(a->HW, gn_ppc(a->HW, a->B)), a->B);
+  if (merged) {
+    hipLaunchKernelGGL(gn_finalize_kernel, dim3(a->groups, a->B), dim3(64), 0, st, a->partials, a->stats, a->HW, C / a->groups, a->groups, a->stat_chunks, a->eps);
+    hipLaunchKernelGGL((gn_apply_kernel<_Float16, 2>), grid, dim3(256), lds, st, (const _Float16*)a->x, (const _Float16*)nullptr, a->stats, a->gamma, a->beta,
+                       (_Float16*)a->y, a->HW, C, 0, a->groups, a->stat_chunks, a->eps, a->silu);
+  } else {
+    hipLaunchKernelGGL((gn_apply_kernel<_Float16, 1>), grid, dim3(256), lds, st, (const _Float16*)a->x, (const _Float16*)nullptr, a->partials, a->gamma, a->beta,
+                       (_Float16*)a->y, a->HW, C, 0, a->groups, a->stat_chunks, a->eps, a->silu);
+  }
+  SR_CHECK_LAUNCH("sr_groupnorm_from_partials");
+  return SR_OK;
+}
diff --git a/stable-renderer_amd/csrc/plan.hip b/stable-renderer_amd/csrc/plan.hip
--- a/stable-renderer_amd/csrc/plan.hip
+++ b/stable-renderer_amd/csrc/plan.hip
@@ -3,7 +3,7 @@
 static int run_op(const sr_op& op, void* stream) {
   switch (op.kind) {
     case SR_OP_IGEMM: return sr_igemm(&op.u.igemm, stream);
-    case SR_OP_GROUPNORM: return sr_groupnorm(&op.u.gn, stream);
+    case SR_OP_GROUPNORM: return op.u.gn.stat_chunks > 0 ? sr_groupnorm_from_partials(&op.u.gn, stream) : sr_groupnorm(&op.u.gn, stream);
     case SR_OP_ATTENTION: return sr_attention(&op.u.attn, stream);
     case SR_OP_LAYERNORM:
       return sr_layernorm(op.u.ln.x, op.u.ln.gamma, op.u.ln.beta, op.u.ln.y, op.u.ln.rows, op.u.ln.C, op.u.ln.eps, op.u.ln.dtype, stream);
diff --git a/stable-renderer_amd/ops.py b/stable-renderer_amd/ops.py
--- a/stable-renderer_amd/ops.py
+++ b/stable-renderer_amd/ops.py
@@ -96,7 +96,7 @@
 
 def igemm_args(a, w, out, B, H, W, C1, N, KH=1, stride=1, upsample=0, a2=None, C2=0, bias=None, rowvec=None,
                residual=None, act=0, transpose_out=0, ldt=0, out_f32=0, scale=1.0, dtype=None, rowvec_ld=0, tile=0, split=0, row_stats=None, colsum=None,
-               pad_br=0, up_hw=None, ln_inline=False, ln_eps=1e-5, tile_order=0):
+               pad_br=0, up_hw=None, ln_inline=False, ln_eps=1e-5, tile_order=0, gn_partials=None, gn_cpg=0, gn_hw=0):
     ar = L.IgemmArgs()
     ar.a, ar.a2, ar.w, ar.bias, ar.rowvec, ar.residual, ar.out = _p(a), _p(a2), _p(w), _p(bias), _p(rowvec), _p(residual), _p(out)
     ar.zero_page = _p(zero_page(a.device))
@@ -109,6 +109,7 @@
     ar.up_h, ar.up_w = (0, 0) if (up_hw is None or tuple(up_hw) == (2 * H, 2 * W)) else (int(up_hw[0]), int(up_hw[1]))
     ar.row_stats, ar.colsum = _p(row_stats), _p(colsum)
     ar.ln_inline, ar.ln_eps = int(bool(ln_inline)), ln_eps
+    ar.gn_partials, ar.gn_cpg, ar.gn_hw = _p(gn_partials), gn_cpg, gn_hw
     ws = workspace(a.device)
     ar.workspace, ar.workspace_bytes = _p(ws), ws.numel()
     if os.environ.get("SR_SPLIT_FIXUP", "0") == "1":
@@ -377,6 +378,22 @@
     return ar
 
 
+def igemm_gn_chunks(ar):
+    return int(L.lib().sr_igemm_gn_chunks(C.byref(ar)))
+
+
+def groupnorm_from_partials(x, gamma, beta, B, HW, C1, partials, chunks, groups=32, eps=1e-5, silu=False):
+    y = torch.empty(B, HW, C1, dtype=x.dtype, device=x.device)
+    ar = groupnorm_args(x, gamma, beta, y, B, HW, C1, partials, None, 0, groups, eps, silu)
+    stats = torch.empty(B, groups, 2, dtype=torch.float32, device=x.device) if chunks > GN_MERGE_IN_APPLY else None
+    ar.stats, ar.stat_chunks = _p(stats), chunks
+    L.check(L.lib().sr_groupnorm_from_partials(C.byref(ar), stream_ptr()))
+    return y
+
+
+GN_MERGE_IN_APPLY = 64
+
+
 def groupnorm(x, gamma, beta, B, HW, C1, x2=None, C2=0, groups=32, eps=1e-5, silu=False):
     y = torch.empty(B, HW, C1 + C2, dtype=x.dtype, device=x.device)
     partials = torch.empty(L.lib().sr_groupnorm_scratch_floats(B, HW), dtype=torch.float32, device=x.device)
diff --git a/stable-renderer_amd/plan.py b/stable-renderer_amd/plan.py
--- a/stable-renderer_amd/plan.py
+++ b/stable-renderer_amd/plan.py
@@ -140,7 +140,41 @@
         if self._lane == 0 and len(members) == len(calls):
             O.tune_group(members)
 
+    def _gn_from_producer(self, x, B, HW, C1):
+        mode = os.environ.get("SR_GN_PRODUCER_STATS", "1")
+        if mode == "0" or self.dtype != torch.float16 or C1 % 32:
+            return None
+        cpg = C1 // 32
+        GB = next((g for g in (1, 2, 4, 8) if (g * cpg) % 8 == 0), 0)
+        if mode != "all" and GB and -(-HW // (1024 // (GB * cpg // 8))) <= 16:
+            return None
+        idx = next((i for i in reversed(range(len(self.ops))) if self.ops[i].kind == L.OP_IGEMM and self.ops[i].u.igemm.out == x.data_ptr()), None)
+        if idx is None or self.ops[idx].lane != 0 or self.ops[idx].u.igemm.N != C1:
+            return None
+        if any(self.ops[j].kind == L.OP_IGEMM and self.ops[j].u.igemm.group > 1 and j + self.ops[j].u.igemm.group > idx
+               for j in range(max(0, idx - O.GROUP_MAX + 1), idx + 1)):
+            return None
+        ar = self.ops[idx].u.igemm
+        ar.gn_cpg, ar.gn_hw = cpg, HW
+        chunks = O.igemm_gn_chunks(ar)
+        if chunks <= 0 or (mode != "all" and chunks > O.GN_MERGE_IN_APPLY):
+            ar.gn_cpg, ar.gn_hw = 0, 0
+            return None
+        rec = self.buf(B * chunks * 32 * 4, dtype=torch.float32)
+        ar.gn_partials = rec.data_ptr()
+        return rec, chunks
+
     def groupnorm(self, x, gamma, beta, y, B, HW, C1, x2=None, C2=0, eps=1e-5, silu=False):
+        prod = self._gn_from_producer(x, B, HW, C1) if x2 is None and C2 == 0 else None
+        if prod is not None:
+            rec, chunks = prod
+            self.hold(x, gamma, beta, y)
+            ar = O.groupnorm_args(x, gamma, beta, y, B, HW, C1, rec, None, 0, 32, eps, silu)
+            ar.stat_chunks = chunks
+            if chunks > O.GN_MERGE_IN_APPLY:
+                ar.stats = self.buf(B, 32, 2, dtype=torch.float32).data_ptr()
+            self._emit(L.OP_GROUPNORM, "gn", ar)
+            return
         need = L.lib().sr_groupnorm_scratch_floats(B, HW)
         if self._gn_scratch is None or self._gn_scratch.numel() < need:
             self._gn_scratch = self.buf(need, dtype=torch.float32)
```

Result: no change. 21.81 (-0.2%).
